# underdoc-wang/STC-GNN

Hardware: NVIDIA B200
Metric: train samples/s (fwd+bwd), SF-shape STC cell stack (higher is better)
Workload: dtype f32

## Files before the change

### include/stc_b200.h

```cpp
#ifndef STC_B200_H_
#define STC_B200_H_

#include <stddef.h>
#include <stdint.h>

#ifdef __cplusplus
extern "C" {
#endif

#define STC_ABI_VERSION 6

typedef enum {
  STC_OK = 0,
  STC_ERR_BAD_ARG = -1,
  STC_ERR_UNSUPPORTED = -2,
  STC_ERR_WORKSPACE = -3,
  STC_ERR_CUDA = -4,
  STC_ERR_ARCH = -5
} StcStatus;

enum { STC_ACT_NONE = 0, STC_ACT_RELU = 1 };
enum { STC_SUPPORT_DENSE = 0, STC_SUPPORT_CSR = 1 };

typedef struct {
  int32_t B;
  int32_t N;
  int32_t C;
  int32_t Din;
  int32_t h;
  int32_t Ks;
  int32_t Kc;
  int32_t act;
  int32_t has_bias;
} StcDims;

typedef struct {
  int32_t kind;
  int64_t nnz;
  const float* vals;
  const int32_t* rowptr;
  const int32_t* col;
  const float* t_vals;
  const int32_t* t_rowptr;
  const int32_t* t_col;
} StcSupport;

int stc_abi_version(void);
const char* stc_last_error(void);

size_t stc_cell_saved_bytes(const StcDims* d);
size_t stc_cell_bwd_scratch_bytes(const StcDims* d);

int stc_cell_fwd(const StcDims* d, const StcSupport* gs, const float* gc,
                 const float* xt, int64_t xt_batch_stride, const float* h_prev,
                 const float* Wg, const float* bg, const float* Wc, const float* bc,
                 float* h_out, void* saved, size_t saved_bytes, void* stream);

enum { STC_STAGE_GATES = 0, STC_STAGE_CANDI = 1 };
enum { STC_SAVED_U = 0, STC_SAVED_R, STC_SAVED_C, STC_SAVED_YR, STC_SAVED_YX, STC_SAVED_YH, STC_SAVED_Q,
       STC_SAVED_PG, STC_SAVED_PC, STC_SAVED_REGIONS };
int stc_cell_saved_layout(const StcDims* d, int64_t* offsets_floats, int32_t n_offsets);
int stc_cell_fwd_stage(const StcDims* d, int32_t stage, const float* gc,
                       const float* xt, int64_t xt_batch_stride, const float* h_prev,
                       const float* Wg, const float* bg, const float* Wc, const float* bc,
                       float* h_out, void* saved, size_t saved_bytes, void* stream);

int stc_cell_bwd(const StcDims* d, const StcSupport* gs, const float* gc,
                 const float* xt, int64_t xt_batch_stride, const float* h_prev,
                 const float* Wg, const float* Wc, const float* d_h_out,
                 float* d_xt, float* d_h_prev,
                 float* dWg, float* dbg, float* dWc, float* dbc, float* dGs, float* dGc,
                 int32_t accumulate_params, const void* saved, size_t saved_bytes,
                 void* scratch, size_t scratch_bytes, void* stream);

int stc_cell_fwd_x(const StcDims* d, const StcSupport* gs, const float* gc,
                   const float* xt, int64_t xt_batch_stride, const float* h_prev,
                   const float* Wg, const float* bg, const float* Wc, const float* bc,
                   float* h_out, void* saved, size_t saved_bytes, const float* yx_terms, void* stream);
int stc_cell_bwd_x(const StcDims* d, const StcSupport* gs, const float* gc,
                   const float* xt, int64_t xt_batch_stride, const float* h_prev,
                   const float* Wg, const float* Wc, const float* d_h_out,
                   float* d_xt, float* d_h_prev,
                   float* dWg, float* dbg, float* dWc, float* dbc, float* dGs, float* dGc,
                   int32_t accumulate_params, const void* saved, size_t saved_bytes,
                   void* scratch, size_t scratch_bytes, const float* yx_terms, float* dyx_terms_out, void* stream);
int stc_support_outer(int32_t N, int32_t B, int32_t width, const float* a, int64_t a_batch_stride, const float* b,
                      float coef, float* dGs, void* stream);
int stc_support_apply_edge_grad(const StcSupport* gs, int32_t N, int32_t B, int32_t width,
                                const float* x, int64_t x_batch_stride, const float* z, int64_t z_batch_stride,
                                float* y, float alpha, float beta, const float* a, int64_t a_batch_stride, float coef,
                                float* dvals, void* stream);
int stc_support_apply_rows_edge_grad(const StcSupport* gs, int32_t N, int32_t B, int32_t width,
                                     const float* x, int64_t x_batch_stride, const float* z, int64_t z_batch_stride,
                                     float* y, float alpha, float beta, const float* a, int64_t a_batch_stride,
                                     float coef, float* dvals, const int32_t* rows, int32_t n_rows, void* stream);

int stc_pair_scores_csr(const StcSupport* gs, int32_t N, int64_t width, const float* u, const float* v,
                        float* scores, void* stream);
int stc_pair_scores_csr_rows(const StcSupport* gs, int32_t N, int64_t width, int64_t ld, const float* u, const float* v,
                             float* scores, const int32_t* rows, int32_t n_rows, void* stream);
int stc_edge_softmax_fwd(const StcSupport* gs, int32_t N, const float* scores, float* p, void* stream);
int stc_edge_softmax_bwd(const StcSupport* gs, int32_t N, const float* scores, const float* p, const float* dp,
                         float* dscores, void* stream);

size_t stc_pair_topk_workspace_bytes(int32_t N, int64_t width, int32_t k);
int stc_pair_topk(int32_t N, int64_t width, const float* u, const float* v, int32_t k,
                  int32_t* cols, float* scores, void* ws, size_t ws_bytes, void* stream);

enum { STC_SCRATCH_DYR = 0, STC_SCRATCH_DYX, STC_SCRATCH_DYH, STC_SCRATCH_REGIONS };
int stc_cell_bwd_scratch_layout(const StcDims* d, int64_t* offsets_floats, int32_t n_offsets);
int stc_cell_bwd_stage(const StcDims* d, int32_t stage, const float* gc,
                       const float* xt, int64_t xt_batch_stride, const float* h_prev,
                       const float* Wg, const float* Wc, const float* d_h_out,
                       float* d_xt, float* d_h_prev,
                       float* dWg, float* dbg, float* dWc, float* dbc, float* dGc,
                       int32_t accumulate_params, const void* saved, size_t saved_bytes,
                       void* scratch, size_t scratch_bytes, void* stream);

int stc_support_apply(const StcSupport* gs, int32_t N, int32_t B, int32_t width, int32_t transpose,
                      const float* x, int64_t x_batch_stride, const float* z, int64_t z_batch_stride,
                      float* y, float alpha, float beta, void* stream);

int stc_support_apply_rows(const StcSupport* gs, int32_t N, int32_t B, int32_t width, int32_t transpose,
                           const float* x, int64_t x_batch_stride, const float* z, int64_t z_batch_stride,
                           float* y, float alpha, float beta, const int32_t* rows, int32_t n_rows, void* stream);

int stc_halo_pack(const float* x_ext, int64_t x_batch_stride, int32_t width, int32_t B, const int32_t* idx,
                  int32_t n_rows, float* send, void* stream);
int stc_halo_unpack(const float* recv, int32_t width, int32_t B, int32_t row0, int32_t n_rows, float* x_ext,
                    int64_t x_batch_stride, void* stream);

int stc_tf32x3_gemm(const float* a, const float* b, float* d, int32_t M, int32_t N, int32_t K, void* stream);

int stc_concurrency_set(int32_t mode);

int stc_last_launch_count(void);

int stc_timing_enable(int32_t on);
int stc_timing_collect(double* ms_by_kind, int64_t* launches_by_kind, double* alg_bytes_by_kind, int32_t n_kinds);
const char* stc_kernel_kind_name(int32_t kind);

int stc_debug_trace_set(void* dev_buf, int64_t n_slots);

#ifdef __cplusplus
}
#endif
#endif
```

### stc_gnn_b200/_lib.py

```python
import ctypes
import os
from ctypes import POINTER, Structure, c_char_p, c_float, c_int, c_int32, c_int64, c_size_t, c_void_p

HERE = os.path.dirname(os.path.abspath(__file__))
LIB_PATH = os.path.join(HERE, "libstc_b200.so")

ABI_VERSION = 6
ACT_NONE, ACT_RELU = 0, 1
SUPPORT_DENSE, SUPPORT_CSR = 0, 1

EXPORTED = (
    "stc_abi_version", "stc_last_error", "stc_cell_saved_bytes", "stc_cell_bwd_scratch_bytes",
    "stc_cell_fwd", "stc_cell_bwd", "stc_support_apply", "stc_last_launch_count",
    "stc_timing_enable", "stc_timing_collect", "stc_kernel_kind_name", "stc_tf32x3_gemm",
    "stc_cell_saved_layout", "stc_cell_fwd_stage", "stc_debug_trace_set",
    "stc_cell_bwd_scratch_layout", "stc_cell_bwd_stage",
    "stc_support_apply_rows", "stc_halo_pack", "stc_halo_unpack", "stc_concurrency_set",
    "stc_cell_fwd_x", "stc_cell_bwd_x", "stc_support_outer", "stc_support_apply_edge_grad",
    "stc_support_apply_rows_edge_grad", "stc_pair_scores_csr", "stc_edge_softmax_fwd", "stc_edge_softmax_bwd",
    "stc_pair_scores_csr_rows", "stc_pair_topk_workspace_bytes", "stc_pair_topk",
)
STAGE_GATES, STAGE_CANDI = 0, 1
SAVED_REGIONS = ("u", "r", "c", "Yr", "Yx", "Yh", "Q", "Pg", "Pc")
SCRATCH_REGIONS = ("dYr", "dYx", "dYh")


class StcDims(Structure):
    _fields_ = [(n, c_int32) for n in ("B", "N", "C", "Din", "h", "Ks", "Kc", "act", "has_bias")]


class StcSupport(Structure):
    _fields_ = [("kind", c_int32), ("nnz", c_int64), ("vals", c_void_p), ("rowptr", c_void_p), ("col", c_void_p),
                ("t_vals", c_void_p), ("t_rowptr", c_void_p), ("t_col", c_void_p)]


_lib = None


def load(build_if_missing: bool = True):
    global _lib
    if _lib is not None:
        return _lib
    if build_if_missing:
        from .build import build
        build()
    if not os.path.exists(LIB_PATH):
        raise RuntimeError(f"{LIB_PATH} is missing: run `python -m stc_gnn_b200.build` (no CPU fallback exists)")
    lib = ctypes.CDLL(LIB_PATH)
    lib.stc_abi_version.restype = c_int
    lib.stc_last_error.restype = c_char_p
    lib.stc_last_launch_count.restype = c_int
    lib.stc_cell_saved_bytes.restype = c_size_t
    lib.stc_cell_saved_bytes.argtypes = [POINTER(StcDims)]
    lib.stc_cell_bwd_scratch_bytes.restype = c_size_t
    lib.stc_cell_bwd_scratch_bytes.argtypes = [POINTER(StcDims)]
    lib.stc_cell_fwd.restype = c_int
    lib.stc_cell_fwd.argtypes = [POINTER(StcDims), POINTER(StcSupport), c_void_p, c_void_p, c_int64, c_void_p,
                                 c_void_p, c_void_p, c_void_p, c_void_p, c_void_p, c_void_p, c_size_t, c_void_p]
    lib.stc_cell_fwd_x.restype = c_int
    lib.stc_cell_fwd_x.argtypes = lib.stc_cell_fwd.argtypes[:-1] + [c_void_p, c_void_p]
    lib.stc_support_outer.restype = c_int
    lib.stc_support_outer.argtypes = [c_int32, c_int32, c_int32, c_void_p, c_int64, c_void_p, c_float, c_void_p, c_void_p]
    lib.stc_support_apply_edge_grad.restype = c_int
    lib.stc_support_apply_edge_grad.argtypes = [POINTER(StcSupport), c_int32, c_int32, c_int32, c_void_p, c_int64,
                                                c_void_p, c_int64, c_void_p, c_float, c_float, c_void_p, c_int64,
                                                c_float, c_void_p, c_void_p]
    lib.stc_support_apply_rows_edge_grad.restype = c_int
    lib.stc_support_apply_rows_edge_grad.argtypes = lib.stc_support_apply_edge_grad.argtypes[:-1] + [c_void_p, c_int32,
                                                                                                    c_void_p]
    lib.stc_pair_scores_csr.restype = c_int
    lib.stc_pair_scores_csr.argtypes = [POINTER(StcSupport), c_int32, c_int64, c_void_p, c_void_p, c_void_p, c_void_p]
    lib.stc_pair_scores_csr_rows.restype = c_int
    lib.stc_pair_scores_csr_rows.argtypes = [POINTER(StcSupport), c_int32, c_int64, c_int64, c_void_p, c_void_p,
                                             c_void_p, c_void_p, c_int32, c_void_p]
    lib.stc_pair_topk_workspace_bytes.restype = c_size_t
    lib.stc_pair_topk_workspace_bytes.argtypes = [c_int32, c_int64, c_int32]
    lib.stc_pair_topk.restype = c_int
    lib.stc_pair_topk.argtypes = [c_int32, c_int64, c_void_p, c_void_p, c_int32, c_void_p, c_void_p, c_void_p, c_size_t,
                                  c_void_p]
    lib.stc_edge_softmax_fwd.restype = c_int
    lib.stc_edge_softmax_fwd.argtypes = [POINTER(StcSupport), c_int32, c_void_p, c_void_p, c_void_p]
    lib.stc_edge_softmax_bwd.restype = c_int
    lib.stc_edge_softmax_bwd.argtypes = [POINTER(StcSupport), c_int32, c_void_p, c_void_p, c_void_p, c_void_p, c_void_p]
    lib.stc_cell_saved_layout.restype = c_int
    lib.stc_cell_saved_layout.argtypes = [POINTER(StcDims), POINTER(c_int64), c_int32]
    lib.stc_cell_fwd_stage.restype = c_int
    lib.stc_cell_fwd_stage.argtypes = [POINTER(StcDims), c_int32, c_void_p, c_void_p, c_int64, c_void_p, c_void_p,
                                       c_void_p, c_void_p, c_void_p, c_void_p, c_void_p, c_size_t, c_void_p]
    lib.stc_cell_bwd.restype = c_int
    lib.stc_cell_bwd.argtypes = [POINTER(StcDims), POINTER(StcSupport), c_void_p, c_void_p, c_int64, c_void_p,
                                 c_void_p, c_void_p, c_void_p, c_void_p, c_void_p, c_void_p, c_void_p, c_void_p,
                                 c_void_p, c_void_p, c_void_p, c_int32, c_void_p, c_size_t, c_void_p, c_size_t,
                                 c_void_p]
    lib.stc_cell_bwd_x.restype = c_int
    lib.stc_cell_bwd_x.argtypes = lib.stc_cell_bwd.argtypes[:-1] + [c_void_p, c_void_p, c_void_p]
    lib.stc_cell_bwd_scratch_layout.restype = c_int
    lib.stc_cell_bwd_scratch_layout.argtypes = [POINTER(StcDims), POINTER(c_int64), c_int32]
    lib.stc_cell_bwd_stage.restype = c_int
    lib.stc_cell_bwd_stage.argtypes = [POINTER(StcDims), c_int32, c_void_p, c_void_p, c_int64, c_void_p,
                                       c_void_p, c_void_p, c_void_p, c_void_p, c_void_p, c_void_p, c_void_p, c_void_p,
                                       c_void_p, c_void_p, c_int32, c_void_p, c_size_t, c_void_p, c_size_t, c_void_p]
    lib.stc_support_apply.restype = c_int
    lib.stc_support_apply.argtypes = [POINTER(StcSupport), c_int32, c_int32, c_int32, c_int32, c_void_p, c_int64,
                                      c_void_p, c_int64, c_void_p, c_float, c_float, c_void_p]
    lib.stc_support_apply_rows.restype = c_int
    lib.stc_support_apply_rows.argtypes = [POINTER(StcSupport), c_int32, c_int32, c_int32, c_int32, c_void_p, c_int64,
                                           c_void_p, c_int64, c_void_p, c_float, c_float, c_void_p, c_int32, c_void_p]
    lib.stc_halo_pack.restype = c_int
    lib.stc_halo_pack.argtypes = [c_void_p, c_int64, c_int32, c_int32, c_void_p, c_int32, c_void_p, c_void_p]
    lib.stc_halo_unpack.restype = c_int
    lib.stc_halo_unpack.argtypes = [c_void_p, c_int32, c_int32, c_int32, c_int32, c_void_p, c_int64, c_void_p]
    lib.stc_concurrency_set.restype = c_int
    lib.stc_concurrency_set.argtypes = [c_int32]
    lib.stc_tf32x3_gemm.restype = c_int
    lib.stc_tf32x3_gemm.argtypes = [c_void_p, c_void_p, c_void_p, c_int32, c_int32, c_int32, c_void_p]
    lib.stc_timing_enable.restype = c_int
    lib.stc_timing_enable.argtypes = [c_int32]
    lib.stc_timing_collect.restype = c_int
    lib.stc_timing_collect.argtypes = [POINTER(ctypes.c_double), POINTER(c_int64), POINTER(ctypes.c_double), c_int32]
    lib.stc_debug_trace_set.restype = c_int
    lib.stc_debug_trace_set.argtypes = [c_void_p, c_int64]
    lib.stc_kernel_kind_name.restype = c_char_p
    lib.stc_kernel_kind_name.argtypes = [c_int32]
    if lib.stc_abi_version() != ABI_VERSION:
        raise RuntimeError(f"libstc_b200.so ABI {lib.stc_abi_version()} != binding ABI {ABI_VERSION}: rebuild")
    _lib = lib
    return lib


def saved_layout(dims: StcDims) -> dict:
    lib = load()
    offs = (c_int64 * len(SAVED_REGIONS))()
    check(lib.stc_cell_saved_layout(dims, offs, len(SAVED_REGIONS)), "stc_cell_saved_layout")
    return {n: int(offs[i]) for i, n in enumerate(SAVED_REGIONS)}


def scratch_layout(dims: StcDims) -> dict:
    lib = load()
    offs = (c_int64 * len(SCRATCH_REGIONS))()
    check(lib.stc_cell_bwd_scratch_layout(dims, offs, len(SCRATCH_REGIONS)), "stc_cell_bwd_scratch_layout")
    return {n: int(offs[i]) for i, n in enumerate(SCRATCH_REGIONS)}


def check(status: int, what: str) -> None:
    if status != 0:
        msg = _lib.stc_last_error().decode("utf-8", "replace") if _lib is not None else ""
        raise RuntimeError(f"{what} failed (status {status}): {msg}")


def last_launch_count() -> int:
    return int(load().stc_last_launch_count())


LAUNCHES = 0


def note_launches() -> None:
    global LAUNCHES
    LAUNCHES += int(_lib.stc_last_launch_count())


def set_concurrency(mode: int) -> None:
    check(load().stc_concurrency_set(int(mode)), "stc_concurrency_set")


def timing_enable(on: bool) -> None:
    load().stc_timing_enable(1 if on else 0)


def timing_collect():
    lib = load()
    n = 32
    ms = (ctypes.c_double * n)()
    cnt = (c_int64 * n)()
    by = (ctypes.c_double * n)()
    kinds = lib.stc_timing_collect(ms, cnt, by, n)
    return {lib.stc_kernel_kind_name(k).decode(): (ms[k], int(cnt[k]), by[k]) for k in range(kinds) if cnt[k]}
```

### stc_gnn_b200/cell.py

```python
from __future__ import annotations

import os

import torch
from torch import nn

from . import _lib
from .support import CsrSupport, dense_struct

INPLACE_LEAF_GRADS = os.environ.get("STC_INPLACE_GRADS", "1") != "0"

_ACT_CODES = {None: _lib.ACT_NONE, nn.ReLU: _lib.ACT_RELU}
_ACT_NAMES = {_lib.ACT_NONE: None, _lib.ACT_RELU: "relu"}


def _activation_code(activation) -> int:
    if activation in _ACT_CODES:
        return _ACT_CODES[activation]
    if isinstance(activation, str):
        return {"none": _lib.ACT_NONE, "relu": _lib.ACT_RELU}[activation]
    raise NotImplementedError(f"activation {activation!r} is not implemented in the B200 cell (None or nn.ReLU)")


class GraphConvParams(nn.Module):

    def __init__(self, Ks: int, Kc: int, input_dim: int, hidden_dim: int, use_bias: bool = True):
        super().__init__()
        self.Ks, self.Kc, self.input_dim, self.hidden_dim, self.use_bias = Ks, Kc, input_dim, hidden_dim, use_bias
        self.W = nn.Parameter(torch.empty(input_dim * Ks * Kc, hidden_dim), requires_grad=True)
        nn.init.xavier_normal_(self.W)
        if use_bias:
            self.b = nn.Parameter(torch.empty(hidden_dim), requires_grad=True)
            nn.init.constant_(self.b, val=0.0)


def _dims(B, N, C, Din, h, Ks, Kc, act, has_bias) -> _lib.StcDims:
    return _lib.StcDims(B, N, C, Din, h, Ks, Kc, act, 1 if has_bias else 0)


_SIZES = {}


def _buffer_floats(lib, dims: _lib.StcDims, key):
    hit = _SIZES.get(key)
    if hit is None:
        if len(_SIZES) > 256:
            _SIZES.clear()
        hit = _SIZES[key] = (lib.stc_cell_saved_bytes(dims) // 4, lib.stc_cell_bwd_scratch_bytes(dims) // 4)
    return hit


def _ptr(t):
    return t.data_ptr() if t is not None else None


class _CellFunction(torch.autograd.Function):

    @staticmethod
    def forward(ctx, Gs, Gc, Xt, H, Wg, bg, Wc, bc, Yx, Ev, cfg):
        lib = _lib.load()
        Ks, Kc, act = cfg
        B, N, C, Din = Xt.shape
        h = H.shape[-1]
        for name, t in (("Gc", Gc), ("Xt", Xt), ("Ht_1", H), ("gates.W", Wg), ("candi.W", Wc)):
            if not t.is_cuda or t.dtype != torch.float32:
                raise RuntimeError(f"STC_Cell (B200): {name} must be a float32 CUDA tensor, got {t.dtype} on {t.device}; "
                                   "there is no CPU fallback")
        if H.shape != (B, N, C, h):
            raise RuntimeError(f"Ht_1 shape {tuple(H.shape)} does not match Xt {tuple(Xt.shape)}")
        rows = (Din + h) * Ks * Kc
        if Wg.shape != (rows, 2 * h) or Wc.shape != (rows, h) or Gc.shape != (C, C):
            raise RuntimeError(f"shape mismatch: gates.W {tuple(Wg.shape)} (want {(rows, 2 * h)}), candi.W "
                               f"{tuple(Wc.shape)} (want {(rows, h)}), Gc {tuple(Gc.shape)} (want {(C, C)})")
        for name, b_, n_ in (("gates.b", bg, 2 * h), ("candi.b", bc, h)):
            if b_ is not None and (b_.shape != (n_,) or not b_.is_cuda or b_.dtype != torch.float32):
                raise RuntimeError(f"{name} must be a float32 CUDA tensor of shape ({n_},)")
        if (bg is None) != (bc is None):
            raise RuntimeError("gates.b and candi.b must both be present or both absent")
        csr = isinstance(Gs, CsrSupport)
        if csr:
            if Gs.N != N:
                raise RuntimeError(f"CSR support has {Gs.N} nodes, Xt has {N}")
            if Ev is not None and Ev is not Gs.vals:
                raise RuntimeError("edge values passed to the cell must be the CsrSupport's own `vals`")
            if Gs.learnable:
                Gs.sync_t_vals()
            gs_struct = Gs.struct()
        else:
            if not Gs.is_cuda or Gs.dtype != torch.float32 or Gs.shape != (N, N):
                raise RuntimeError(f"Gs must be a float32 CUDA [N,N] tensor or a CsrSupport, got {tuple(Gs.shape)} {Gs.dtype}")
            gs_keep = Gs.contiguous()
            gs_struct = dense_struct(gs_keep)
        Gc_c, H_c, Wg_c, Wc_c = Gc.contiguous(), H.contiguous(), Wg.contiguous(), Wc.contiguous()
        bg_c = bg.contiguous() if bg is not None else None
        bc_c = bc.contiguous() if bc is not None else None
        Xt_c = Xt if (B == 0 or Xt[0].is_contiguous()) else Xt.contiguous()
        xbs = Xt_c.stride(0) if B > 1 else N * C * Din
        dims = _dims(B, N, C, Din, h, Ks, Kc, act, bg is not None)
        ctx.size_key = (B, N, C, Din, h, Ks, Kc, act, bg is not None)
        saved = torch.empty(_buffer_floats(lib, dims, ctx.size_key)[0], dtype=torch.float32, device=Xt.device)
        Hn = torch.empty((B, N, C, h), dtype=torch.float32, device=Xt.device)
        stream = torch.cuda.current_stream().cuda_stream
        Yx_c = None
        if Yx is not None and Ks > 1:
            if Yx.shape != (Ks - 1, B, N, C, Din) or not Yx.is_cuda or Yx.dtype != torch.float32:
                raise RuntimeError(f"hoisted Xt-side terms must be a float32 CUDA tensor of shape {(Ks - 1, B, N, C, Din)}, "
                                   f"got {tuple(Yx.shape)}")
            Yx_c = Yx.contiguous()
        if B == 0:
            status = 0
        elif Yx_c is not None:
            status = lib.stc_cell_fwd_x(dims, gs_struct, Gc_c.data_ptr(), Xt_c.data_ptr(), xbs, H_c.data_ptr(),
                                        Wg_c.data_ptr(), _ptr(bg_c), Wc_c.data_ptr(), _ptr(bc_c), Hn.data_ptr(),
                                        saved.data_ptr(), saved.numel() * 4, Yx_c.data_ptr(), stream)
        else:
            status = lib.stc_cell_fwd(dims, gs_struct, Gc_c.data_ptr(), Xt_c.data_ptr(), xbs, H_c.data_ptr(),
                                      Wg_c.data_ptr(), _ptr(bg_c), Wc_c.data_ptr(), _ptr(bc_c), Hn.data_ptr(),
                                      saved.data_ptr(), saved.numel() * 4, stream)
        _lib.check(status, "stc_cell_fwd")
        _lib.note_launches()
        ctx.hoisted = Yx_c is not None
        ctx.cfg, ctx.dims_tuple, ctx.xbs, ctx.csr = cfg, (B, N, C, Din, h), xbs, csr
        ctx.gs_obj = Gs if csr else None
        ctx.has_bias = bg is not None
        ctx.sinks = {}
        if INPLACE_LEAF_GRADS:
            for i, t in ((0, None if csr else Gs), (1, Gc), (4, Wg), (5, bg), (6, Wc), (7, bc), (9, Ev)):
                if t is not None and ctx.needs_input_grad[i] and t.is_leaf and t.is_contiguous():
                    ctx.sinks[i] = t
        ctx.has_ev = Ev is not None
        ctx.save_for_backward(*( [] if csr else [gs_keep] ), Gc_c, Xt_c, H_c, Wg_c, Wc_c, saved,
                              *([Yx_c] if Yx_c is not None else []), *([Ev] if Ev is not None else []))
        return Hn

    @staticmethod
    @torch.autograd.function.once_differentiable
    def backward(ctx, dHn):
        lib = _lib.load()
        Ks, Kc, act = ctx.cfg
        B, N, C, Din, h = ctx.dims_tuple
        sv = list(ctx.saved_tensors)
        if ctx.has_ev:
            sv.pop()
        Yx = sv.pop() if ctx.hoisted else None
        if ctx.csr:
            Gs = ctx.gs_obj
            Gc, Xt, H, Wg, Wc, saved = sv
            gs_struct = Gs.struct()
        else:
            Gs, Gc, Xt, H, Wg, Wc, saved = sv
            gs_struct = dense_struct(Gs)
        need = ctx.needs_input_grad
        dev = dHn.device
        dHn = dHn.contiguous()
        L, P = Din + h, Ks * Kc
        dims = _dims(B, N, C, Din, h, Ks, Kc, act, ctx.has_bias)
        new = lambda *shape: torch.empty(shape, dtype=torch.float32, device=dev)
        if ctx.hoisted and need[2]:
            raise RuntimeError("hoisted Xt-side terms: the gradient w.r.t. Xt is folded by the caller (stack.py hoists only "
                               "when the input sequence needs no gradient)")
        dXt = new(B, N, C, Din) if need[2] else None
        dH = new(B, N, C, h)
        dYx = torch.empty_like(Yx) if ctx.hoisted else None
        returned = [None] * 11

        def target(i, shape, wanted=True):
            if not wanted:
                return None
            leaf = ctx.sinks.get(i)
            if leaf is not None and need[i]:
                if leaf.grad is None:
                    leaf.grad = torch.zeros(shape, dtype=torch.float32, device=dev)
                if leaf.grad.is_contiguous() and leaf.grad.dtype == torch.float32 and leaf.grad.shape == torch.Size(shape):
                    return leaf.grad
            buf = torch.zeros(shape, dtype=torch.float32, device=dev)
            returned[i] = buf
            return buf

        dWg, dWc = target(4, (P * L, 2 * h)), target(6, (P * L, h))
        dbg, dbc = target(5, (2 * h,), ctx.has_bias), target(7, (h,), ctx.has_bias)
        dGs = target(9, (Gs.nnz,), need[9]) if ctx.csr else target(0, (N, N), need[0])
        dGc = target(1, (C, C), need[1])
        returned[2], returned[3], returned[8] = dXt, dH, dYx
        if B == 0:
            if dYx is not None:
                dYx.zero_()
            return tuple(returned)
        scratch = torch.empty(_buffer_floats(lib, dims, ctx.size_key)[1], dtype=torch.float32, device=dev)
        common = (dims, gs_struct, Gc.data_ptr(), Xt.data_ptr(), ctx.xbs, H.data_ptr(), Wg.data_ptr(),
                  Wc.data_ptr(), dHn.data_ptr(), _ptr(dXt), dH.data_ptr(), dWg.data_ptr(), _ptr(dbg),
                  dWc.data_ptr(), _ptr(dbc), _ptr(dGs), _ptr(dGc), 1, saved.data_ptr(),
                  saved.numel() * 4, scratch.data_ptr(), scratch.numel() * 4)
        stream = torch.cuda.current_stream().cuda_stream
        if ctx.hoisted:
            status = lib.stc_cell_bwd_x(*common, Yx.data_ptr(), dYx.data_ptr(), stream)
        else:
            status = lib.stc_cell_bwd(*common, stream)
        _lib.check(status, "stc_cell_bwd")
        _lib.note_launches()
        for i in (0, 1, 4, 5, 6, 7, 8, 9):
            if not need[i]:
                returned[i] = None
        return tuple(returned)


def stc_cell_forward(Gs, Gc, Xt, Ht_1, Wg, bg, Wc, bc, Ks: int, Kc: int, activation=None) -> torch.Tensor:
    return _CellFunction.apply(Gs, Gc, Xt, Ht_1, Wg, bg, Wc, bc, None, _edge_values(Gs),
                               (int(Ks), int(Kc), _activation_code(activation)))


def _edge_values(Gs):
    return Gs.vals if isinstance(Gs, CsrSupport) and Gs.learnable else None


class STC_Cell(nn.Module):

    def __init__(self, num_nodes: int, num_categories: int, Ks: int, Kc: int, input_dim: int, hidden_dim: int,
                 use_bias=True, activation=None):
        super().__init__()
        self.num_nodes = num_nodes
        self.num_categories = num_categories
        self.hidden_dim = hidden_dim
        self.input_dim = input_dim
        self.Ks, self.Kc = Ks, Kc
        self._act = _activation_code(activation)
        self.gates = GraphConvParams(Ks, Kc, input_dim + hidden_dim, hidden_dim * 2, use_bias)
        self.candi = GraphConvParams(Ks, Kc, input_dim + hidden_dim, hidden_dim, use_bias)

    def init_hidden(self, batch_size: int):
        weight = next(self.parameters()).data
        return weight.new_zeros(batch_size, self.num_nodes, self.num_categories, self.hidden_dim)

    def forward(self, Gs, Gc: torch.Tensor, Xt: torch.Tensor, Ht_1: torch.Tensor, _Yx: torch.Tensor = None):
        assert len(Xt.shape) == len(Ht_1.shape) == 4, 'STC-cell must take in 4D tensor as input [Xt, Ht-1]'
        if isinstance(Gs, torch.Tensor) and Gs.layout != torch.strided:
            Gs = _csr_cache(Gs)
        if hasattr(Gs, "fwd") and hasattr(Gs, "hop_ext"):
            from .halo import partitioned_cell_forward
            return partitioned_cell_forward(Gs, Gc, Xt, Ht_1, self.gates.W, getattr(self.gates, "b", None), self.candi.W,
                                            getattr(self.candi, "b", None), self.Ks, self.Kc, _ACT_NAMES[self._act],
                                            reduce_params=getattr(Gs, "reduce_per_cell", True))
        return _CellFunction.apply(Gs, Gc, Xt, Ht_1, self.gates.W, getattr(self.gates, "b", None), self.candi.W,
                                   getattr(self.candi, "b", None), _Yx, _edge_values(Gs), (self.Ks, self.Kc, self._act))


_CSR_CACHE = {}


def _csr_cache(G: torch.Tensor) -> CsrSupport:
    if G.requires_grad:
        raise RuntimeError("STC_Cell (B200): a torch sparse Gs is a constant support and gets no gradient; for learned "
                           "edge weights on a fixed pattern pass CsrSupport(rowptr, col, vals_requiring_grad, N) "
                           "(or a dense [N,N] tensor when the whole dGs is needed)")
    if G.layout == torch.sparse_csr:
        vals, idx = G.values(), G.col_indices()
    else:
        vals, idx = G._values(), G._indices()
    key = (vals.data_ptr(), vals._version, idx.data_ptr(), idx._version, int(vals.numel()), tuple(G.shape), G.layout,
           vals.dtype)
    hit = _CSR_CACHE.get(key)
    if hit is None:
        if len(_CSR_CACHE) > 8:
            _CSR_CACHE.clear()
        hit = _CSR_CACHE[key] = (CsrSupport.from_torch_sparse(G), G)
    return hit[0]
```

### stc_gnn_b200/csrc/stc_api.cu

```cuda
#include "stc_common.cuh"

#include <stdlib.h>
#include <string.h>

#include <atomic>
#include <mutex>
#include <vector>

namespace stc {

static thread_local char g_err[512] = "";
static thread_local int g_launches = 0;

void set_error(const char* fmt, ...) {
  va_list ap;
  va_start(ap, fmt);
  vsnprintf(g_err, sizeof(g_err), fmt, ap);
  va_end(ap);
}
void count_launch(int n) { g_launches += n; }
void reset_launch_count() { g_launches = 0; }

struct TimedLaunch {
  int kind;
// ... 238 lines not shown
  a.Hout = phase == 0 ? 2 * d.h : d.h;
  a.x0 = xt;
  a.x0_bs = xt_bs;
  a.yx = ws + w.Yx;
  a.W = W;
  a.Q = Q;
  a.opt = conv_opt_flags();
  const bool wide_bwd = !(a.opt & OPT_WIDE_DX_FFMA) && conv_big_bwd_shape_ok(a.C, a.Din, a.h, a.Ks, a.Kc, a.Hout);
  a.dpre_ld = (conv_tc_eligible(a) || wide_bwd) ? a.Kc * a.Hout : a.Hout;
  conv_trace_target(&a.trace, &a.trace_tiles);
  if (a.trace) a.trace += (size_t)phase * a.trace_tiles * TRACE_SLOTS;
  return a;
}

}

using namespace stc;

extern "C" {

int stc_timing_enable(int32_t on) {
  g_timing.store(on != 0);
  return STC_OK;
}

int stc_timing_collect(double* ms, int64_t* launches, double* bytes, int32_t n_kinds) {
  std::lock_guard<std::mutex> lk(g_tmu);
  for (auto& t : g_timed) {
    float m = 0.f;
    if (cudaEventSynchronize(t.e1) == cudaSuccess && cudaEventElapsedTime(&m, t.e0, t.e1) == cudaSuccess &&
        t.kind < n_kinds) {
      if (ms) ms[t.kind] += m;
      if (launches) launches[t.kind] += 1;
      if (bytes) bytes[t.kind] += t.bytes;
    }
    g_event_pool.push_back(t.e0);
    g_event_pool.push_back(t.e1);
  }
  g_timed.clear();
  return KK_COUNT;
}

const char* stc_kernel_kind_name(int32_t kind) {
  static const char* names[KK_COUNT] = {"support_dense", "support_csr", "support_outer", "cheby_small",
                                        "conv_fwd",      "conv_bwd_dx", "conv_bwd_dw", "tc_conv_fwd", "tc_conv_bwd_dx", "tc_conv_bwd_dw",
                                        "tc_support", "tc_gemm_test", "tc_outer", "tc_support_big", "support_csr_grad",
                                        "pair_scores_csr", "edge_softmax", "pair_topk"};
  return (kind >= 0 && kind < KK_COUNT) ? names[kind] : "?";
}

int stc_debug_trace_set(void* dev_buf, int64_t n_slots) {
  std::lock_guard<std::mutex> lk(g_tmu);
  g_trace_buf = (long long*)dev_buf;
  g_trace_tiles = dev_buf ? (int)(n_slots / (2 * TRACE_SLOTS)) : 0;
  return STC_OK;
}

int stc_concurrency_set(int32_t mode) {
  if (mode < -1 || mode > 1) {
    set_error("stc_concurrency_set: mode %d (use -1 = by problem size, 0 = one stream, 1 = always fork)", mode);
    return STC_ERR_BAD_ARG;
  }
  g_concurrency.store(mode, std::memory_order_relaxed);
  return STC_OK;
}

int stc_abi_version(void) { return STC_ABI_VERSION; }
const char* stc_last_error(void) { return g_err; }
int stc_last_launch_count(void) { return g_launches; }

size_t stc_cell_saved_bytes(const StcDims* d) {
  if (check_dims(d) != STC_OK) return 0;
  return make_layout(*d).saved_total * sizeof(float);
}
size_t stc_cell_bwd_scratch_bytes(const StcDims* d) {
  if (check_dims(d) != STC_OK) return 0;
  return make_layout(*d).scratch_total * sizeof(float);
}

int stc_support_apply(const StcSupport* gs, int32_t N, int32_t B, int32_t width, int32_t transpose,
                      const float* x, int64_t x_batch_stride, const float* z, int64_t z_batch_stride, float* y,
                      float alpha, float beta, void* stream) {
  reset_launch_count();
  if (!gs || !x || !y) {
    set_error("stc_support_apply: NULL argument");
    return STC_ERR_BAD_ARG;
  }
  STC_TRY(check_arch());
  return launch_support_apply(*gs, N, B, width, transpose != 0, x, x_batch_stride, z, z_batch_stride, y, alpha,
                              beta, nullptr, 0.f, (cudaStream_t)stream);
}

int stc_support_apply_rows(const StcSupport* gs, int32_t N, int32_t B, int32_t width, int32_t transpose, const float* x,
                           int64_t x_batch_stride, const float* z, int64_t z_batch_stride, float* y, float alpha,
                           float beta, const int32_t* rows, int32_t n_rows, void* stream) {
  reset_launch_count();
  if (!gs || !x || !y || !rows) {
    set_error("stc_support_apply_rows: NULL argument");
    return STC_ERR_BAD_ARG;
  }
  if (n_rows < 0 || n_rows > N) {
    set_error("stc_support_apply_rows: n_rows %d outside [0, N = %d]", n_rows, N);
    return STC_ERR_BAD_ARG;
  }
  STC_TRY(check_arch());
  return launch_support_apply(*gs, N, B, width, transpose != 0, x, x_batch_stride, z, z_batch_stride, y, alpha, beta,
                              nullptr, 0.f, (cudaStream_t)stream, rows, n_rows);
}

int stc_halo_pack(const float* x_ext, int64_t x_batch_stride, int32_t width, int32_t B, const int32_t* idx, int32_t n_rows,
                  float* send, void* stream) {
  reset_launch_count();
  if (n_rows > 0 && (!x_ext || !idx || !send)) {
    set_error("stc_halo_pack: NULL argument");
    return STC_ERR_BAD_ARG;
  }
  STC_TRY(check_arch());
  return launch_halo_rows(true, const_cast<float*>(x_ext), x_batch_stride, width, B, idx, 0, n_rows, send, (cudaStream_t)stream);
}

int stc_halo_unpack(const float* recv, int32_t width, int32_t B, int32_t row0, int32_t n_rows, float* x_ext,
                    int64_t x_batch_stride, void* stream) {
  reset_launch_count();
  if (n_rows > 0 && (!x_ext || !recv)) {
    set_error("stc_halo_unpack: NULL argument");
    return STC_ERR_BAD_ARG;
  }
  STC_TRY(check_arch());
  return launch_halo_rows(false, x_ext, x_batch_stride, width, B, nullptr, row0, n_rows, const_cast<float*>(recv), (cudaStream_t)stream);
}

int stc_tf32x3_gemm(const float* a, const float* b, float* d, int32_t M, int32_t N, int32_t K, void* stream) {
  reset_launch_count();
  if (!a || !b || !d) {
    set_error("stc_tf32x3_gemm: NULL argument");
    return STC_ERR_BAD_ARG;
  }
  STC_TRY(check_arch());
  return launch_tf32x3_gemm(a, b, d, M, N, K, (cudaStream_t)stream);
}

struct FwdCtx {
  const StcDims& d;
  const WsLayout& w;
  const StcSupport* gs;
  const float* gc;
  const float* xt;
  int64_t xt_bs;
  const float* h_prev;
  float* ws;
  cudaStream_t st;
  Lanes* lanes = nullptr;
  const float* yx_pre = nullptr;
};

static int fwd_terms_xh(const FwdCtx& f) {
  const StcDims& d = f.d;
  const WsLayout& w = f.w;
  float* ws = f.ws;
  const size_t Rh = w.R * d.h, Rx = w.R * d.Din;
  const int CD = d.C * d.Din, CH = d.C * d.h;
  const long long nbs_h = (long long)d.N * CH;
  cudaStream_t sx = f.st;
  if (f.lanes && f.lanes->active() && d.Ks > 1 && !f.yx_pre) {
    STC_TRY(f.lanes->fork(0));
    sx = f.lanes->stream(0);
  }
  for (int k = 1; k < d.Ks && !f.yx_pre; ++k) {
    const float alpha = k == 1 ? 1.f : 2.f, beta = k == 1 ? 0.f : -1.f;
    const float* xin = k == 1 ? f.xt : ws + w.Yx + (size_t)(k - 2) * Rx;
    const int64_t xin_bs = k == 1 ? f.xt_bs : (int64_t)d.N * CD;
    const float* xz = k == 1 ? nullptr : (k == 2 ? f.xt : ws + w.Yx + (size_t)(k - 3) * Rx);
    const int64_t xz_bs = k == 2 ? f.xt_bs : (int64_t)d.N * CD;
    STC_TRY(launch_support_apply(*f.gs, d.N, d.B, CD, true, xin, xin_bs, xz, xz_bs, ws + w.Yx + (size_t)(k - 1) * Rx,
                                 alpha, beta, nullptr, 0.f, sx));
  }
  for (int k = 1; k < d.Ks; ++k) {
    const float alpha = k == 1 ? 1.f : 2.f, beta = k == 1 ? 0.f : -1.f;
    const float* hin = k == 1 ? f.h_prev : ws + w.Yh + (size_t)(k - 2) * Rh;
    const float* hz = k == 1 ? nullptr : (k == 2 ? f.h_prev : ws + w.Yh + (size_t)(k - 3) * Rh);
    STC_TRY(launch_support_apply(*f.gs, d.N, d.B, CH, true, hin, nbs_h, hz, nbs_h, ws + w.Yh + (size_t)(k - 1) * Rh,
                                 alpha, beta, nullptr, 0.f, f.st));
  }
  if (f.lanes) STC_TRY(f.lanes->join(0));
  return STC_OK;
}

static int fwd_gates(const FwdCtx& f, const float* Wg, const float* bg) {
  const StcDims& d = f.d;
  const WsLayout& w = f.w;
  float* ws = f.ws;
  if (d.Kc > 1) STC_TRY(launch_cheby_small(f.gc, d.C, d.Kc, ws + w.Q, f.st));
  ConvArgs a = base_args(d, f.xt, f.xt_bs, Wg, ws + w.Q, ws, w, 0);
  if (f.yx_pre) a.yx = f.yx_pre;
  a.h0 = f.h_prev;
  a.yh = ws + w.Yh;
  a.bias = d.has_bias ? bg : nullptr;
  a.Hprev = f.h_prev;
  a.u = ws + w.u;
  a.r = ws + w.r;
  a.rH = ws + w.Yr;
  a.Psave = ws + w.Pg;
  a.Wimg = (w.Wimg_c > w.Wimg_g) ? ws + w.Wimg_g : nullptr;
  return launch_conv_fwd(a, f.st);
}

static int fwd_terms_rh(const FwdCtx& f) {
  const StcDims& d = f.d;
  const WsLayout& w = f.w;
  float* ws = f.ws;
  const size_t Rh = w.R * d.h;
  const int CH = d.C * d.h;
  const long long nbs_h = (long long)d.N * CH;
  for (int k = 1; k < d.Ks; ++k) {
    const float alpha = k == 1 ? 1.f : 2.f, beta = k == 1 ? 0.f : -1.f;
    const float* in = ws + w.Yr + (size_t)(k - 1) * Rh;
    const float* z = k == 1 ? nullptr : ws + w.Yr + (size_t)(k - 2) * Rh;
    STC_TRY(launch_support_apply(*f.gs, d.N, d.B, CH, true, in, nbs_h, z, nbs_h, ws + w.Yr + (size_t)k * Rh, alpha, beta,
                                 nullptr, 0.f, f.st));
  }
  return STC_OK;
}

static int fwd_candi(const FwdCtx& f, const float* Wc, const float* bc, float* h_out) {
  const StcDims& d = f.d;
  const WsLayout& w = f.w;
  float* ws = f.ws;
  const size_t Rh = w.R * d.h;
  ConvArgs a = base_args(d, f.xt, f.xt_bs, Wc, ws + w.Q, ws, w, 1);
  if (f.yx_pre) a.yx = f.yx_pre;
  a.h0 = ws + w.Yr;
  a.yh = ws + w.Yr + Rh;
  a.bias = d.has_bias ? bc : nullptr;
  a.Hprev = f.h_prev;
  a.u = ws + w.u;
  a.c = ws + w.c;
  a.Hnew = h_out;
  a.Psave = ws + w.Pc;
  a.Wimg = (w.saved_total > w.Wimg_c) ? ws + w.Wimg_c : nullptr;
  return launch_conv_fwd(a, f.st);
}

static int check_fwd_args(const StcDims* dp, const float* gc, const float* xt, const float* h_prev, const float* Wg,
                          const float* bg, const float* Wc, const float* bc, float* h_out, void* wsv, size_t ws_bytes,
                          const char* who) {
  STC_TRY(check_dims(dp));
  if (!gc || !xt || !h_prev || !Wg || !Wc || !h_out || !wsv) {
    set_error("%s: NULL argument", who);
    return STC_ERR_BAD_ARG;
  }
  if (dp->has_bias && (!bg || !bc)) {
    set_error("%s: has_bias set but bias pointer is NULL", who);
    return STC_ERR_BAD_ARG;
  }
  const WsLayout w = make_layout(*dp);
  if (ws_bytes < w.saved_total * sizeof(float)) {
    set_error("saved buffer too small: %zu < %zu bytes", ws_bytes, w.saved_total * sizeof(float));
    return STC_ERR_WORKSPACE;
  }
  return STC_OK;
}

static int cell_fwd_impl(const StcDims* dp, const StcSupport* gs, const float* gc, const float* xt,
                         int64_t xt_batch_stride, const float* h_prev, const float* Wg, const float* bg, const float* Wc,
                         const float* bc, float* h_out, void* wsv, size_t ws_bytes, const float* yx_terms, void* stream,
                         const char* who) {
  reset_launch_count();
  STC_TRY(check_fwd_args(dp, gc, xt, h_prev, Wg, bg, Wc, bc, h_out, wsv, ws_bytes, who));
  if (!gs) {
    set_error("%s: NULL support", who);
    return STC_ERR_BAD_ARG;
  }
  const StcDims& d = *dp;
  if (d.B == 0) return STC_OK;
  STC_TRY(check_arch());
  const WsLayout w = make_layout(d);
  Lanes lanes((cudaStream_t)stream, d);
  FwdCtx f{d, w, gs, gc, xt, xt_batch_stride, h_prev, (float*)wsv, (cudaStream_t)stream};
  f.lanes = &lanes;
  f.yx_pre = d.Ks > 1 ? yx_terms : nullptr;
  STC_TRY(fwd_terms_xh(f));
  STC_TRY(fwd_gates(f, Wg, bg));
  STC_TRY(fwd_terms_rh(f));
  STC_TRY(fwd_candi(f, Wc, bc, h_out));
  return STC_OK;
}

int stc_cell_fwd(const StcDims* dp, const StcSupport* gs, const float* gc, const float* xt,
                 int64_t xt_batch_stride, const float* h_prev, const float* Wg, const float* bg, const float* Wc,
                 const float* bc, float* h_out, void* wsv, size_t ws_bytes, void* stream) {
  return cell_fwd_impl(dp, gs, gc, xt, xt_batch_stride, h_prev, Wg, bg, Wc, bc, h_out, wsv, ws_bytes, nullptr, stream,
                       "stc_cell_fwd");
}

int stc_cell_fwd_x(const StcDims* dp, const StcSupport* gs, const float* gc, const float* xt,
                   int64_t xt_batch_stride, const float* h_prev, const float* Wg, const float* bg, const float* Wc,
                   const float* bc, float* h_out, void* wsv, size_t ws_bytes, const float* yx_terms, void* stream) {
  return cell_fwd_impl(dp, gs, gc, xt, xt_batch_stride, h_prev, Wg, bg, Wc, bc, h_out, wsv, ws_bytes, yx_terms, stream,
                       "stc_cell_fwd_x");
}

int stc_cell_saved_layout(const StcDims* dp, int64_t* offsets, int32_t n_offsets) {
  STC_TRY(check_dims(dp));
  if (!offsets || n_offsets < STC_SAVED_REGIONS) {
    set_error("stc_cell_saved_layout: need room for %d offsets", (int)STC_SAVED_REGIONS);
    return STC_ERR_BAD_ARG;
  }
  const WsLayout w = make_layout(*dp);
  const size_t v[STC_SAVED_REGIONS] = {w.u, w.r, w.c, w.Yr, w.Yx, w.Yh, w.Q, w.Pg, w.Pc};
  for (int i = 0; i < STC_SAVED_REGIONS; ++i) offsets[i] = (int64_t)v[i];
  return STC_OK;
}

int stc_cell_fwd_stage(const StcDims* dp, int32_t stage, const float* gc, const float* xt, int64_t xt_batch_stride,
                       const float* h_prev, const float* Wg, const float* bg, const float* Wc, const float* bc,
                       float* h_out, void* wsv, size_t ws_bytes, void* stream) {
  reset_launch_count();
  STC_TRY(check_fwd_args(dp, gc, xt, h_prev, Wg, bg, Wc, bc, h_out, wsv, ws_bytes, "stc_cell_fwd_stage"));
  if (stage != STC_STAGE_GATES && stage != STC_STAGE_CANDI) {
    set_error("stc_cell_fwd_stage: bad stage %d", stage);
    return STC_ERR_BAD_ARG;
  }
  const StcDims& d = *dp;
  if (d.B == 0) return STC_OK;
  STC_TRY(check_arch());
  const WsLayout w = make_layout(d);
  const FwdCtx f{d, w, nullptr, gc, xt, xt_batch_stride, h_prev, (float*)wsv, (cudaStream_t)stream};
  return stage == STC_STAGE_GATES ? fwd_gates(f, Wg, bg) : fwd_candi(f, Wc, bc, h_out);
}

static int adjoint_chain(const StcDims& d, const StcSupport& gs, int width, const float* y0, int64_t y0_bs,
                         const float* yk , float* ybar0, float* ybark ,
                         float* dGs, cudaStream_t st, Lanes* lanes = nullptr, int outer_lane = 1) {
  const size_t Rw = (size_t)d.B * d.N * width;
  const int64_t nbs = (int64_t)d.N * width;
  for (int k = d.Ks - 1; k >= 1; --k) {
    const float coef = k >= 2 ? 2.f : 1.f;
    float* yb_k = ybark + (size_t)(k - 1) * Rw;
    float* yb_km1 = k == 1 ? ybar0 : ybark + (size_t)(k - 2) * Rw;
    float* axpy = nullptr;
    if (k >= 2) axpy = k == 2 ? ybar0 : ybark + (size_t)(k - 3) * Rw;
    if (dGs && gs.kind == STC_SUPPORT_CSR) {
      const float* yprev = k == 1 ? y0 : yk + (size_t)(k - 2) * Rw;
      const int64_t yprev_bs = k == 1 ? y0_bs : nbs;
      STC_TRY(launch_support_csr_edge_grad(gs, d.N, d.B, width, yb_k, nbs, yb_km1, nbs, yb_km1, coef, 1.f, axpy, -1.f,
                                           yprev, yprev_bs, coef, dGs, st));
      continue;
    }
    if (dGs) {
      const float* yprev = k == 1 ? y0 : yk + (size_t)(k - 2) * Rw;
      const int64_t yprev_bs = k == 1 ? y0_bs : nbs;
      cudaStream_t so = st;
      if (lanes && lanes->active()) {
        STC_TRY(lanes->fork_from(st, outer_lane));
        so = lanes->stream(outer_lane);
      }
      STC_TRY(launch_support_outer(d.N, d.B, width, yprev, yprev_bs, yb_k, coef, dGs, so));
    }
    STC_TRY(launch_support_apply(gs, d.N, d.B, width, false, yb_k, nbs, yb_km1, nbs, yb_km1, coef, 1.f, axpy, -1.f,
                                 st));
  }
  return STC_OK;
}

struct BwdCtx {
  const StcDims& d;
  const WsLayout& w;
  const float* gc;
  const float* xt;
  int64_t xt_bs;
  const float* h_prev;
  const float* d_h_out;
  float* d_xt;
  float* d_h_prev;
  float* dGc;
  float* sv;
  float* sc;
  cudaStream_t st;
  Lanes* lanes = nullptr;
  const float* yx_pre = nullptr;
  float* dyx_out = nullptr;
  bool want_dGc() const { return dGc != nullptr && d.Kc > 1; }
  float* dYx0() const { return d_xt ? d_xt : sc + w.dYx0; }
};

static int check_bwd_args(const StcDims* dp, const float* gc, const float* xt, const float* h_prev, const float* Wg,
                          const float* Wc, const float* d_h_out, float* d_h_prev, float* dWg, float* dbg, float* dWc,
                          float* dbc, const void* savedv, size_t saved_bytes, void* scratchv, size_t scratch_bytes,
                          const char* who) {
  STC_TRY(check_dims(dp));
  const StcDims& d = *dp;
  if (!gc || !xt || !h_prev || !Wg || !Wc || !d_h_out || !d_h_prev || !dWg || !dWc || !savedv || !scratchv) {
    set_error("%s: NULL argument", who);
    return STC_ERR_BAD_ARG;
  }
  if (d.has_bias && (!dbg || !dbc)) {
    set_error("%s: has_bias set but a bias-gradient pointer is NULL", who);
    return STC_ERR_BAD_ARG;
  }
  const WsLayout w = make_layout(d);
  if (saved_bytes < w.saved_total * sizeof(float) || scratch_bytes < w.scratch_total * sizeof(float)) {
    set_error("buffers too small: saved %zu (need %zu), scratch %zu (need %zu) bytes", saved_bytes,
              w.saved_total * sizeof(float), scratch_bytes, w.scratch_total * sizeof(float));
    return STC_ERR_WORKSPACE;
  }
  return STC_OK;
}

static int bwd_begin(const BwdCtx& b, float* dWg, float* dbg, float* dWc, float* dbc, float* dGs, size_t dGs_floats,
                     int accumulate_params) {
  const StcDims& d = b.d;
  const int L = d.Din + d.h, P = d.Ks * d.Kc;
  if (!accumulate_params) {
    STC_CUDA_OK(cudaMemsetAsync(dWg, 0, sizeof(float) * P * L * 2 * d.h, b.st));
    STC_CUDA_OK(cudaMemsetAsync(dWc, 0, sizeof(float) * P * L * d.h, b.st));
    if (d.has_bias) {
      STC_CUDA_OK(cudaMemsetAsync(dbg, 0, sizeof(float) * 2 * d.h, b.st));
      STC_CUDA_OK(cudaMemsetAsync(dbc, 0, sizeof(float) * d.h, b.st));
    }
    if (dGs && dGs_floats) STC_CUDA_OK(cudaMemsetAsync(dGs, 0, sizeof(float) * dGs_floats, b.st));
    if (b.dGc) STC_CUDA_OK(cudaMemsetAsync(b.dGc, 0, sizeof(float) * d.C * d.C, b.st));
  }
  if (d.B > 0 && b.want_dGc()) STC_CUDA_OK(cudaMemsetAsync(b.sc + b.w.dQ, 0, sizeof(float) * d.Kc * d.C * d.C, b.st));
  return STC_OK;
}

static int launch_dw_beside(const BwdCtx& b, const ConvArgs& a) {
  if (b.lanes && b.lanes->active()) {
    STC_TRY(b.lanes->fork(0));
    return launch_conv_bwd_dw(a, b.lanes->stream(0));
  }
  return launch_conv_bwd_dw(a, b.st);
}

static int bwd_candi(const BwdCtx& b, const float* Wc, float* dWc, float* dbc) {
  const StcDims& d = b.d;
  const WsLayout& w = b.w;
  const size_t Rh = w.R * d.h;
  ConvArgs a = base_args(d, b.xt, b.xt_bs, Wc, b.sv + w.Q, b.sv, w, 1);
  if (b.yx_pre) a.yx = b.yx_pre;
  a.h0 = b.sv + w.Yr;
  a.yh = b.sv + w.Yr + Rh;
  a.Hprev = b.h_prev;
  a.u = b.sv + w.u;
  a.c = b.sv + w.c;
  a.dHn = b.d_h_out;
  a.dpre = b.sc + w.dpre;
  a.dbias = d.has_bias ? dbc : nullptr;
  a.dYx0 = b.dYx0();
  a.dYx = b.dyx_out ? b.dyx_out : b.sc + w.dYx;
  a.accum_x = 0;
  a.dYh0 = b.sc + w.dYr;
  a.dYh = b.sc + w.dYr + Rh;
  a.dQ = b.want_dGc() ? b.sc + w.dQ : nullptr;
  a.dW = dWc;
  a.Psave = b.sv + w.Pc;
  a.Wimg = (w.saved_total > w.Wimg_c && w.scratch_total > w.Wimg_dx) ? b.sc + w.Wimg_dx : nullptr;
  STC_TRY(launch_conv_bwd_dx(a, b.st));
  return launch_dw_beside(b, a);
}

static int bwd_gates(const BwdCtx& b, const float* Wg, float* dWg, float* dbg) {
  const StcDims& d = b.d;
  const WsLayout& w = b.w;
  ConvArgs a = base_args(d, b.xt, b.xt_bs, Wg, b.sv + w.Q, b.sv, w, 0);
  if (b.yx_pre) a.yx = b.yx_pre;
  a.h0 = b.h_prev;
  a.yh = b.sv + w.Yh;
  a.Hprev = b.h_prev;
  a.u = b.sv + w.u;
  a.r = b.sv + w.r;
  a.c = b.sv + w.c;
  a.dHn = b.d_h_out;
  a.drH = b.sc + w.dYr;
  a.dpre = b.sc + w.dpre;
  a.dbias = d.has_bias ? dbg : nullptr;
  a.dYx0 = b.dYx0();
  a.dYx = b.dyx_out ? b.dyx_out : b.sc + w.dYx;
  a.accum_x = 1;
  a.dYh0 = b.d_h_prev;
  a.dYh = b.sc + w.dYh;
  a.dQ = b.want_dGc() ? b.sc + w.dQ : nullptr;
  a.dW = dWg;
  a.Psave = b.sv + w.Pg;
  a.Wimg = (w.Wimg_c > w.Wimg_g && w.scratch_total > w.Wimg_dx) ? b.sc + w.Wimg_dx : nullptr;
  if (b.lanes) STC_TRY(b.lanes->join(0));
  STC_TRY(launch_conv_bwd_dx(a, b.st));
  STC_TRY(launch_dw_beside(b, a));
  if (b.want_dGc()) STC_TRY(launch_cheby_small_bwd(b.gc, b.sv + w.Q, b.sc + w.dQ, d.C, d.Kc, b.dGc, b.st));
  return STC_OK;
}

static int cell_bwd_impl(const StcDims* dp, const StcSupport* gs, const float* gc, const float* xt,
                         int64_t xt_batch_stride, const float* h_prev, const float* Wg, const float* Wc,
                         const float* d_h_out, float* d_xt, float* d_h_prev, float* dWg, float* dbg, float* dWc, float* dbc,
                         float* dGs, float* dGc, int32_t accumulate_params, const void* savedv, size_t saved_bytes,
                         void* scratchv, size_t scratch_bytes, const float* yx_terms, float* dyx_terms_out, void* stream,
                         const char* who) {
  reset_launch_count();
  STC_TRY(check_bwd_args(dp, gc, xt, h_prev, Wg, Wc, d_h_out, d_h_prev, dWg, dbg, dWc, dbc, savedv, saved_bytes, scratchv,
                         scratch_bytes, who));
  const StcDims& d = *dp;
  if (!gs) {
    set_error("%s: NULL argument", who);
    return STC_ERR_BAD_ARG;
  }
  if (dGs && gs->kind == STC_SUPPORT_CSR && (!gs->rowptr || !gs->col || !gs->vals || gs->nnz < 0)) {
    set_error("%s: the edge-value gradient of a CSR support needs its rowptr/col/vals and nnz", who);
    return STC_ERR_BAD_ARG;
  }
  if (d.Ks > 1 && ((yx_terms != nullptr) != (dyx_terms_out != nullptr))) {
    set_error("%s: yx_terms and dyx_terms_out go together (the caller that supplied the Xt-side terms folds their adjoints)", who);
    return STC_ERR_BAD_ARG;
  }
  const WsLayout w = make_layout(d);
  STC_TRY(check_arch());
  cudaStream_t st = (cudaStream_t)stream;
  Lanes lanes(st, d);
  BwdCtx b{d, w, gc, xt, xt_batch_stride, h_prev, d_h_out, d_xt, d_h_prev, dGc,
           const_cast<float*>((const float*)savedv), (float*)scratchv, st};
  b.lanes = &lanes;
  const bool hoisted = d.Ks > 1 && yx_terms != nullptr;
  if (hoisted) {
    b.yx_pre = yx_terms;
    b.dyx_out = dyx_terms_out;
  }
  const size_t dGs_floats = gs->kind == STC_SUPPORT_CSR ? (size_t)gs->nnz : (size_t)d.N * d.N;
  STC_TRY(bwd_begin(b, dWg, dbg, dWc, dbc, dGs, dGs_floats, accumulate_params));
  if (d.B == 0) return STC_OK;
  const size_t Rh = w.R * d.h;
  const int CD = d.C * d.Din, CH = d.C * d.h;

  STC_TRY(bwd_candi(b, Wc, dWc, dbc));
  STC_TRY(adjoint_chain(d, *gs, CH, b.sv + w.Yr, (int64_t)d.N * CH, b.sv + w.Yr + Rh, b.sc + w.dYr, b.sc + w.dYr + Rh,
                        dGs, st, &lanes, 1));
  STC_TRY(bwd_gates(b, Wg, dWg, dbg));
  if (!hoisted) {
    cudaStream_t sx = st;
    if (lanes.active() && d.Ks > 1) {
      STC_TRY(lanes.fork(2));
      sx = lanes.stream(2);
    }
    STC_TRY(adjoint_chain(d, *gs, CD, xt, xt_batch_stride, b.sv + w.Yx, b.dYx0(), b.sc + w.dYx, dGs, sx, &lanes, 1));
  }
  STC_TRY(adjoint_chain(d, *gs, CH, h_prev, (int64_t)d.N * CH, b.sv + w.Yh, d_h_prev, b.sc + w.dYh, dGs, st, &lanes, 1));
  return lanes.join_all();
}

int stc_cell_bwd(const StcDims* dp, const StcSupport* gs, const float* gc, const float* xt,
                 int64_t xt_batch_stride, const float* h_prev, const float* Wg, const float* Wc,
                 const float* d_h_out, float* d_xt, float* d_h_prev, float* dWg, float* dbg, float* dWc, float* dbc,
                 float* dGs, float* dGc, int32_t accumulate_params, const void* savedv, size_t saved_bytes,
                 void* scratchv, size_t scratch_bytes, void* stream) {
  return cell_bwd_impl(dp, gs, gc, xt, xt_batch_stride, h_prev, Wg, Wc, d_h_out, d_xt, d_h_prev, dWg, dbg, dWc, dbc, dGs, dGc,
                       accumulate_params, savedv, saved_bytes, scratchv, scratch_bytes, nullptr, nullptr, stream,
                       "stc_cell_bwd");
}

int stc_cell_bwd_x(const StcDims* dp, const StcSupport* gs, const float* gc, const float* xt,
                   int64_t xt_batch_stride, const float* h_prev, const float* Wg, const float* Wc,
                   const float* d_h_out, float* d_xt, float* d_h_prev, float* dWg, float* dbg, float* dWc, float* dbc,
                   float* dGs, float* dGc, int32_t accumulate_params, const void* savedv, size_t saved_bytes,
                   void* scratchv, size_t scratch_bytes, const float* yx_terms, float* dyx_terms_out, void* stream) {
  return cell_bwd_impl(dp, gs, gc, xt, xt_batch_stride, h_prev, Wg, Wc, d_h_out, d_xt, d_h_prev, dWg, dbg, dWc, dbc, dGs, dGc,
                       accumulate_params, savedv, saved_bytes, scratchv, scratch_bytes, yx_terms, dyx_terms_out, stream,
                       "stc_cell_bwd_x");
}

int stc_support_outer(int32_t N, int32_t B, int32_t width, const float* a, int64_t a_batch_stride, const float* b,
                      float coef, float* dGs, void* stream) {
  reset_launch_count();
  if (!a || !b || !dGs) {
    set_error("stc_support_outer: NULL argument");
    return STC_ERR_BAD_ARG;
  }
  STC_TRY(check_arch());
  return launch_support_outer(N, B, width, a, a_batch_stride, b, coef, dGs, (cudaStream_t)stream);
}

int stc_support_apply_edge_grad(const StcSupport* gs, int32_t N, int32_t B, int32_t width, const float* x,
                                int64_t x_batch_stride, const float* z, int64_t z_batch_stride, float* y, float alpha,
                                float beta, const float* a, int64_t a_batch_stride, float coef, float* dvals,
                                void* stream) {
  reset_launch_count();
  if (!gs || !x || !y || !a || !dvals) {
    set_error("stc_support_apply_edge_grad: NULL argument");
    return STC_ERR_BAD_ARG;
  }
  if (gs->kind != STC_SUPPORT_CSR) {
    set_error("stc_support_apply_edge_grad: CSR supports only (a dense support's gradient is stc_support_outer)");
    return STC_ERR_UNSUPPORTED;
  }
  STC_TRY(check_arch());
  return launch_support_csr_edge_grad(*gs, N, B, width, x, x_batch_stride, z, z_batch_stride, y, alpha, beta, nullptr,
                                      0.f, a, a_batch_stride, coef, dvals, (cudaStream_t)stream);
}

int stc_support_apply_rows_edge_grad(const StcSupport* gs, int32_t N, int32_t B, int32_t width, const float* x,
                                     int64_t x_batch_stride, const float* z, int64_t z_batch_stride, float* y,
                                     float alpha, float beta, const float* a, int64_t a_batch_stride, float coef,
                                     float* dvals, const int32_t* rows, int32_t n_rows, void* stream) {
  reset_launch_count();
  if (!gs || !x || !y || !a || !dvals || !rows) {
    set_error("stc_support_apply_rows_edge_grad: NULL argument");
    return STC_ERR_BAD_ARG;
  }
  if (gs->kind != STC_SUPPORT_CSR) {
    set_error("stc_support_apply_rows_edge_grad: CSR supports only");
    return STC_ERR_UNSUPPORTED;
  }
  if (n_rows < 0 || n_rows > N) {
    set_error("stc_support_apply_rows_edge_grad: n_rows %d outside [0, N = %d]", n_rows, N);
    return STC_ERR_BAD_ARG;
  }
  STC_TRY(check_arch());
  return launch_support_csr_edge_grad(*gs, N, B, width, x, x_batch_stride, z, z_batch_stride, y, alpha, beta, nullptr,
                                      0.f, a, a_batch_stride, coef, dvals, (cudaStream_t)stream, rows, n_rows);
}

static int check_pattern(const StcSupport* gs, int32_t N, const char* who) {
  if (!gs) {
    set_error("%s: NULL pattern", who);
    return STC_ERR_BAD_ARG;
  }
  if (gs->kind != STC_SUPPORT_CSR) {
    set_error("%s: the pattern must be a CSR support (kind %d)", who, gs->kind);
    return STC_ERR_UNSUPPORTED;
  }
  if (!gs->rowptr || !gs->col || gs->nnz < 0) {
    set_error("%s: the pattern needs rowptr / col and nnz >= 0", who);
    return STC_ERR_BAD_ARG;
  }
  if (N <= 0) {
    set_error("%s: N = %d must be positive", who, N);
    return STC_ERR_BAD_ARG;
  }
  return STC_OK;
}

int stc_pair_scores_csr(const StcSupport* gs, int32_t N, int64_t width, const float* u, const float* v, float* scores,
                        void* stream) {
  reset_launch_count();
  STC_TRY(check_pattern(gs, N, "stc_pair_scores_csr"));
  if (!u || !v || !scores) {
    set_error("stc_pair_scores_csr: NULL argument");
    return STC_ERR_BAD_ARG;
  }
  if (width <= 0) {
    set_error("stc_pair_scores_csr: width = %lld must be positive", (long long)width);
    return STC_ERR_BAD_ARG;
  }
  STC_TRY(check_arch());
  return launch_pair_scores_csr(gs->rowptr, gs->col, gs->nnz, N, width, u, v, scores, (cudaStream_t)stream);
}

int stc_pair_scores_csr_rows(const StcSupport* gs, int32_t N, int64_t width, int64_t ld, const float* u, const float* v,
                             float* scores, const int32_t* rows, int32_t n_rows, void* stream) {
  reset_launch_count();
  STC_TRY(check_pattern(gs, N, "stc_pair_scores_csr_rows"));
  if (!u || !v || !scores || !rows) {
    set_error("stc_pair_scores_csr_rows: NULL argument");
    return STC_ERR_BAD_ARG;
  }
  if (width <= 0) {
    set_error("stc_pair_scores_csr_rows: width = %lld must be positive", (long long)width);
    return STC_ERR_BAD_ARG;
  }
  if (ld < width) {
    set_error("stc_pair_scores_csr_rows: row stride ld = %lld is smaller than width = %lld", (long long)ld,
              (long long)width);
    return STC_ERR_BAD_ARG;
  }
  if (n_rows < 0 || n_rows > N) {
    set_error("stc_pair_scores_csr_rows: n_rows %d outside [0, N = %d]", n_rows, N);
    return STC_ERR_BAD_ARG;
  }
  STC_TRY(check_arch());
  return launch_pair_scores_csr_rows(gs->rowptr, gs->col, gs->nnz, N, width, ld, u, v, scores, rows, n_rows,
                                     (cudaStream_t)stream);
}

int stc_edge_softmax_fwd(const StcSupport* gs, int32_t N, const float* scores, float* p, void* stream) {
  reset_launch_count();
  STC_TRY(check_pattern(gs, N, "stc_edge_softmax_fwd"));
  if (!scores || !p) {
    set_error("stc_edge_softmax_fwd: NULL argument");
    return STC_ERR_BAD_ARG;
  }
  STC_TRY(check_arch());
  return launch_edge_softmax(false, gs->rowptr, gs->nnz, N, scores, nullptr, nullptr, p, (cudaStream_t)stream);
}

int stc_edge_softmax_bwd(const StcSupport* gs, int32_t N, const float* scores, const float* p, const float* dp,
                         float* dscores, void* stream) {
  reset_launch_count();
  STC_TRY(check_pattern(gs, N, "stc_edge_softmax_bwd"));
  if (!scores || !p || !dp || !dscores) {
    set_error("stc_edge_softmax_bwd: NULL argument");
    return STC_ERR_BAD_ARG;
  }
  STC_TRY(check_arch());
  return launch_edge_softmax(true, gs->rowptr, gs->nnz, N, scores, p, dp, dscores, (cudaStream_t)stream);
}

static int check_topk_shape(int32_t N, int64_t width, int32_t k, const char* who) {
  if (N <= 0 || width <= 0 || width % 4 != 0 || width > (1 << 28)) {
    set_error("%s: N = %d must be positive and width = %lld a positive multiple of 4 (at most 2^28)", who, N,
              (long long)width);
    return STC_ERR_BAD_ARG;
  }
  if (k > 32) {
    set_error("%s: k = %d: at most 32 columns a row are kept on chip", who, k);
    return STC_ERR_UNSUPPORTED;
  }
  if (k < 1 || k > N) {
    set_error("%s: k = %d outside [1, N = %d]", who, k, N);
    return STC_ERR_BAD_ARG;
  }
  return STC_OK;
// ... 72 lines not shown
```

### stc_gnn_b200/csrc/stc_common.cuh

```cuda
#pragma once
#include <cuda_runtime.h>
#include <stdint.h>
#include <stdio.h>
#include <stdarg.h>

#include "../../include/stc_b200.h"

namespace stc {

void set_error(const char* fmt, ...);
void count_launch(int n = 1);
void reset_launch_count();

#define STC_CUDA_OK(expr)                                                                   \
  do {                                                                                      \
    cudaError_t _e = (expr);                                                                \
    if (_e != cudaSuccess) {                                                                \
      stc::set_error("%s failed: %s (%s:%d)", #expr, cudaGetErrorString(_e), __FILE__, __LINE__); \
      return STC_ERR_CUDA;                                                                  \
    }                                                                                       \
  } while (0)

#define STC_LAUNCH_OK(name)                                                                 \
  do {                                                                                      \
    cudaError_t _e = cudaGetLastError();                                                    \
    if (_e != cudaSuccess) {                                                                \
      stc::set_error("launch of %s failed: %s (%s:%d)", name, cudaGetErrorString(_e), __FILE__, __LINE__); \
      return STC_ERR_CUDA;                                                                  \
    }                                                                                       \
    stc::count_launch();                                                                    \
  } while (0)

#define STC_TRY(expr)            \
  do {                           \
    int _s = (expr);             \
    if (_s != STC_OK) return _s; \
  } while (0)

enum KernelKind {
  KK_SUPPORT_DENSE = 0, KK_SUPPORT_CSR, KK_SUPPORT_OUTER, KK_CHEBY_SMALL, KK_CONV_FWD, KK_CONV_BWD_DX,
  KK_CONV_BWD_DW, KK_TC_CONV_FWD, KK_TC_CONV_BWD_DX, KK_TC_CONV_BWD_DW, KK_TC_SUPPORT, KK_TC_GEMM_TEST, KK_TC_OUTER, KK_TC_SUPPORT_BIG,
  KK_SUPPORT_CSR_GRAD, KK_PAIR_SCORES_CSR, KK_EDGE_SOFTMAX, KK_PAIR_TOPK, KK_COUNT
};
struct ScopedKernelTimer {
  ScopedKernelTimer(int kind, cudaStream_t st, double alg_bytes);
  ~ScopedKernelTimer();
  cudaEvent_t e0, e1;
  int kind;
  double bytes;
  cudaStream_t st;
};

static inline size_t round_up(size_t x, size_t m) { return (x + m - 1) / m * m; }
static inline int ceil_div(long long a, long long b) { return (int)((a + b - 1) / b); }

struct FastDiv {
  uint32_t d, M, s;
};
static inline FastDiv make_fastdiv(uint32_t d) {
  FastDiv f;
  f.d = d ? d : 1;
  f.s = 0;
  while ((2u << f.s) <= f.d && f.s < 31) ++f.s;
  f.M = (uint32_t)(((((uint64_t)1) << (32 + f.s)) - 1) / f.d);
  return f;
}
#ifdef __CUDACC__
__device__ __forceinline__ uint32_t fast_div(uint32_t n, const FastDiv f) {
  if (f.d == 1) return n;
  uint32_t q = __umulhi(n, f.M) >> f.s;
  if (n - q * f.d >= f.d) ++q;
  return q;
}
#endif

int device_sm_count();
int check_arch();

struct WsLayout {
  size_t R;
  size_t u, r, c, Yr, Yx, Yh, Q, Pg, Pc, Wimg_g, Wimg_c, saved_total;
  size_t dpre, dYx0, dYx, dYh, dYr, dQ, Wimg_dx, scratch_total;
};
WsLayout make_layout(const StcDims& d);

int launch_support_apply(const StcSupport& gs, int N, int B, int width, bool transpose, const float* x,
                         int64_t x_bs, const float* z, int64_t z_bs, float* y, float alpha, float beta,
                         float* axpy_out, float axpy_coef, cudaStream_t st, const int32_t* row_list = nullptr,
                         int n_list = 0);
int launch_halo_rows(bool pack, float* x_ext, long long x_bs, int W, int B, const int32_t* idx, int row0, int n_rows,
                     float* buf, cudaStream_t st);

int try_launch_support_tc(const float* G, int N, int B, int width, bool transpose, const float* x, int64_t x_bs,
                          const float* z, int64_t z_bs, float* y, float alpha, float beta, cudaStream_t st,
                          bool* handled);
int try_launch_support_tc_big(const float* G, int N, int B, int width, bool transpose, const float* x, int64_t x_bs,
                              const float* z, int64_t z_bs, float* y, float alpha, float beta, cudaStream_t st,
                              bool* handled);
int try_launch_outer_tc(int N, int B, int width, const float* a, int64_t a_bs, const float* bmat, float coef, float* dG,
                        cudaStream_t st, bool* handled);

int launch_support_csr_edge_grad(const StcSupport& gs, int N, int B, int width, const float* x, int64_t x_bs,
                                 const float* z, int64_t z_bs, float* y, float alpha, float beta, float* axpy_out,
                                 float axpy_coef, const float* a, int64_t a_bs, float coef, float* dvals,
                                 cudaStream_t st, const int32_t* row_list = nullptr, int n_list = 0);

int launch_support_outer(int N, int B, int width, const float* a, int64_t a_bs, const float* bmat, float coef,
                         float* dG, cudaStream_t st);

int launch_pair_scores_csr(const int32_t* rowptr, const int32_t* col, long long nnz, int N, long long width,
                           const float* u, const float* v, float* scores, cudaStream_t st);
int launch_pair_scores_csr_rows(const int32_t* rowptr, const int32_t* col, long long nnz, int N, long long width,
                                long long ld, const float* u, const float* v, float* scores, const int32_t* rows,
                                int n_rows, cudaStream_t st);
int launch_edge_softmax(bool bwd, const int32_t* rowptr, long long nnz, int N, const float* s, const float* p,
                        const float* dp, float* out, cudaStream_t st);
size_t pair_topk_ws_bytes(int N, int k);
int launch_pair_topk(int N, int width, const float* u, const float* v, int k, int32_t* cols, float* scores, void* ws,
                     cudaStream_t st);

int launch_cheby_small(const float* G, int C, int K, float* Q, cudaStream_t st);
int launch_cheby_small_bwd(const float* G, const float* Q, float* dQ, int C, int K, float* dG, cudaStream_t st);

struct ConvArgs {
  int B, N, C, Din, h, Ks, Kc, Hout, act, phase;
  const float* x0;
  long long x0_bs;
  const float* yx;
  const float* h0;
  const float* yh;
  const float* W;
  const float* bias;
  const float* Q;
  const float* Hprev;
  float* u;
  float* r;
  float* rH;
  float* c;
  float* Hnew;
  float* Psave;
  float* Wimg;
  const float* dHn;
  const float* drH;
  float* dpre;
  int dpre_ld;
  float* dbias;
  float* dYx0;
  float* dYx;
  int accum_x;
  float* dYh0;
  float* dYh;
  float* dQ;
  float* dW;
  int opt;
  long long* trace;
  int trace_tiles;
};
enum { OPT_L2_PREFETCH = 1, OPT_GENERIC_EPILOGUE = 4 ,
       OPT_SMEM_A = 8 ,
       OPT_WIDE_DX_FFMA = 32  };
constexpr int TRACE_SLOTS = 16;
int conv_opt_flags();
void conv_trace_target(long long** buf, int* tiles);
int launch_tf32x3_gemm(const float* A, const float* Bm, float* D, int M, int N, int K, cudaStream_t st);
int launch_conv_fwd(const ConvArgs& a, cudaStream_t st);
bool conv_big_shape_ok(int C, int Din, int h, int Ks, int Kc, int Hout);
size_t conv_big_img_floats(int C, int Din, int h, int Ks, int Kc, int Hout);
int try_launch_conv_fwd_big(const ConvArgs& a, cudaStream_t st, bool* handled);
size_t conv_big_dx_img_floats(int C, int Din, int h, int Ks, int Kc, int Hout);
int try_launch_conv_bwd_dx_big(const ConvArgs& a, cudaStream_t st, bool* handled);
bool conv_big_bwd_shape_ok(int C, int Din, int h, int Ks, int Kc, int Hout);
int try_launch_conv_bwd_dw_big(const ConvArgs& a, cudaStream_t st, bool* handled);
bool conv_tc_eligible(const ConvArgs& a);
bool conv_tc_dw_shape_ok(const ConvArgs& a);
int launch_conv_bwd_dx(const ConvArgs& a, cudaStream_t st);
int launch_conv_bwd_dw(const ConvArgs& a, cudaStream_t st);

}
```

### stc_gnn_b200/csrc/stc_conv.cu

```cuda
#include "stc_conv_common.cuh"

namespace stc {

template <int NI>
__device__ __forceinline__ void tile_gemm(float (&acc)[NI][4][4], const float* __restrict__ A, int lda,
                                          const float* __restrict__ Bm, int ldb, int K, int RG, int CG) {
  const int items = RG * CG;
#pragma unroll
  for (int i = 0; i < NI; ++i) {
    const int it = threadIdx.x + i * CV_THREADS;
    if (it >= items) break;
    const int rg = it / CG, cg = it - rg * CG;
    const float* ap = A + rg * 4 * lda;
    const float* bp = Bm + cg * 4;
#pragma unroll 4
    for (int k = 0; k < K; ++k) {
      float a0 = ap[k], a1 = ap[lda + k], a2 = ap[2 * lda + k], a3 = ap[3 * lda + k];
      float4 b = *reinterpret_cast<const float4*>(bp + k * ldb);
      acc[i][0][0] = fmaf(a0, b.x, acc[i][0][0]); acc[i][0][1] = fmaf(a0, b.y, acc[i][0][1]);
      acc[i][0][2] = fmaf(a0, b.z, acc[i][0][2]); acc[i][0][3] = fmaf(a0, b.w, acc[i][0][3]);
      acc[i][1][0] = fmaf(a1, b.x, acc[i][1][0]); acc[i][1][1] = fmaf(a1, b.y, acc[i][1][1]);
      acc[i][1][2] = fmaf(a1, b.z, acc[i][1][2]); acc[i][1][3] = fmaf(a1, b.w, acc[i][1][3]);
      acc[i][2][0] = fmaf(a2, b.x, acc[i][2][0]); acc[i][2][1] = fmaf(a2, b.y, acc[i][2][1]);
      acc[i][2][2] = fmaf(a2, b.z, acc[i][2][2]); acc[i][2][3] = fmaf(a2, b.w, acc[i][2][3]);
// ... 118 lines not shown
    }
    target = (t.npt / 2) * a.C;
    if (target < a.C) target = a.C;
  }
}


int launch_conv_fwd(const ConvArgs& a, cudaStream_t st) {
  bool handled = false;
  STC_TRY(try_launch_conv_fwd_tc(a, st, &handled));
  if (handled) return STC_OK;
  STC_TRY(try_launch_conv_fwd_big(a, st, &handled));
  if (handled) return STC_OK;
  ConvTile t; size_t smem; int ni;
  STC_TRY(pick_rows_fwd(a, &t, &smem, &ni));
  long long total_nodes = (long long)a.B * a.N;
  int grid = ceil_div(total_nodes, t.npt);
  const double R = (double)total_nodes * a.C;
  ScopedKernelTimer _t(KK_CONV_FWD, st,
                       4.0 * R * (a.Ks * t.L + (a.phase == 0 ? 3 * a.h : 4 * a.h)) + 4.0 * a.Ks * a.Kc * t.L * a.Hout);
  switch (ni) {
    case 1: STC_TRY(set_smem(conv_fwd_kernel<1>, smem)); conv_fwd_kernel<1><<<grid, CV_THREADS, smem, st>>>(a, t); break;
    case 2: STC_TRY(set_smem(conv_fwd_kernel<2>, smem)); conv_fwd_kernel<2><<<grid, CV_THREADS, smem, st>>>(a, t); break;
    default: STC_TRY(set_smem(conv_fwd_kernel<4>, smem)); conv_fwd_kernel<4><<<grid, CV_THREADS, smem, st>>>(a, t); break;
  }
  STC_LAUNCH_OK("conv_fwd_kernel");
  return STC_OK;
}

template <int NI>
__global__ void __launch_bounds__(CV_THREADS)
conv_bwd_dx_kernel(const ConvArgs a, const ConvTile t, const int DP) {
  extern __shared__ __align__(16) float smem[];
  const int C = a.C, L = t.L, LP = t.LP, LP4 = t.LP4, Hout = a.Hout, h = a.h, Din = a.Din;
  const bool mixed = a.Kc > 1;
  const bool want_dQ = mixed && a.dQ != nullptr;
  float* Ds = smem;
  float* WsT = Ds + (size_t)t.rowsP * DP;
  float* DY = WsT + (size_t)Hout * LP4;
  float* DF = DY + (size_t)t.rowsP * LP;
  float* Fin = DF + (mixed ? (size_t)t.rowsP * LP : 0);
  float* Qs = Fin + (want_dQ ? (size_t)t.rowsP * LP : 0);

  const long long total_nodes = (long long)a.B * a.N;
  const long long g0 = (long long)blockIdx.x * t.npt;
  const int nodes_valid = (int)min((long long)t.npt, total_nodes - g0);
  const int rows_valid = nodes_valid * C;
  const long long row0 = g0 * C;
  const long long R = total_nodes * C;
  const FeatSrc fs = feat_src(a);
  const int RG = t.rowsP / 4, CGL = LP4 / 4;

  for (int i = threadIdx.x; i < (a.Kc - 1) * C * C; i += blockDim.x) Qs[i] = a.Q[C * C + i];

  for (int idx = threadIdx.x; idx < t.rowsP * h; idx += blockDim.x) {
    const int row = idx / h, j = idx - row * h;
    const long long o = (row0 + row) * h + j;
    if (row < rows_valid) {
      const float dhn = a.dHn[o], uu = a.u[o], cc = a.c[o];
      if (a.phase == 1) {
        float g = dhn * uu * (1.f - cc * cc);
        if (a.act == STC_ACT_RELU && !(cc > 0.f)) g = 0.f;
        Ds[row * DP + j] = g;
        a.dpre[(row0 + row) * a.dpre_ld + j] = g;
      } else {
        const float hp = a.Hprev[o], rr = a.r[o], drh = a.drH[o];
        float gu = dhn * (cc - hp) * uu * (1.f - uu);
        float gr = drh * hp * rr * (1.f - rr);
        if (a.act == STC_ACT_RELU) {
          if (!(uu > 0.5f)) gu = 0.f;
          if (!(rr > 0.5f)) gr = 0.f;
        }
        Ds[row * DP + j] = gu;
        Ds[row * DP + h + j] = gr;
        a.dpre[(row0 + row) * a.dpre_ld + j] = gu;
        a.dpre[(row0 + row) * a.dpre_ld + h + j] = gr;
        a.dYh0[o] = dhn * (1.f - uu) + drh * rr;
      }
    } else {
      Ds[row * DP + j] = 0.f;
      if (a.phase == 0) Ds[row * DP + h + j] = 0.f;
    }
  }
  __syncthreads();
  if (a.dbias) {
    for (int j = threadIdx.x; j < Hout; j += blockDim.x) {
      float s = 0.f;
      for (int row = 0; row < rows_valid; ++row) s += Ds[row * DP + j];
      atomicAdd(&a.dbias[j], s);
    }
  }

  for (int k = 0; k < a.Ks; ++k) {
    __syncthreads();
    for (int idx = threadIdx.x; idx < t.rowsP * LP; idx += blockDim.x) DY[idx] = 0.f;
    if (want_dQ) load_feat_tile(fs, k, g0, nodes_valid, t.rowsP, Fin, LP);
    for (int c = 0; c < a.Kc; ++c) {
      __syncthreads();
      const float* Wblk = a.W + (size_t)(k * a.Kc + c) * L * Hout;
      for (int idx = threadIdx.x; idx < Hout * LP4; idx += blockDim.x) {
        int j = idx / LP4, l = idx - j * LP4;
        WsT[idx] = (l < L) ? Wblk[l * Hout + j] : 0.f;
      }
      __syncthreads();
      float acc[NI][4][4];
#pragma unroll
      for (int i = 0; i < NI; ++i)
#pragma unroll
        for (int x = 0; x < 4; ++x)
#pragma unroll
          for (int y = 0; y < 4; ++y) acc[i][x][y] = 0.f;
      tile_gemm<NI>(acc, Ds, DP, WsT, LP4, Hout, RG, CGL);
      float* dst = (c == 0) ? DY : DF;
      const int items = RG * CGL;
#pragma unroll
      for (int i = 0; i < NI; ++i) {
        const int it = threadIdx.x + i * CV_THREADS;
        if (it >= items) break;
        const int rg = it / CGL, lg = it - rg * CGL;
#pragma unroll
        for (int x = 0; x < 4; ++x)
#pragma unroll
          for (int y = 0; y < 4; ++y) {
            const int l = lg * 4 + y;
            if (l < L) {
              float* p = dst + (rg * 4 + x) * LP + l;
              if (c == 0) *p += acc[i][x][y]; else *p = acc[i][x][y];
            }
          }
      }
      if (c > 0) {
        __syncthreads();
        const float* Qc = Qs + (size_t)(c - 1) * C * C;
        unmix_add_tile(DF, DY, Qc, rows_valid, C, L, LP);
        if (want_dQ) {
          for (int pr = threadIdx.x; pr < C * C; pr += blockDim.x) {
            const int cp = pr / C, d = pr - cp * C;
            float s = 0.f;
            for (int node = 0; node < nodes_valid; ++node) {
              const float* y = Fin + (node * C + cp) * LP;
              const float* f = DF + (node * C + d) * LP;
              for (int l = 0; l < L; ++l) s = fmaf(y[l], f[l], s);
            }
            atomicAdd(&a.dQ[(size_t)c * C * C + pr], s);
          }
        }
      }
    }
    __syncthreads();
    {
      float* dx = (k == 0) ? a.dYx0 : a.dYx + (size_t)(k - 1) * R * Din;
      if (dx) {
        dx += row0 * Din;
        for (int idx = threadIdx.x; idx < rows_valid * Din; idx += blockDim.x) {
          int row = idx / Din, l = idx - row * Din;
          float v = DY[row * LP + l];
          dx[idx] = a.accum_x ? dx[idx] + v : v;
        }
      }
      float* dh = (k == 0) ? a.dYh0 : a.dYh + (size_t)(k - 1) * R * h;
      dh += row0 * h;
      const bool add_direct = (k == 0 && a.phase == 0);
      for (int idx = threadIdx.x; idx < rows_valid * h; idx += blockDim.x) {
        int row = idx / h, l = idx - row * h;
        float v = DY[row * LP + Din + l];
        dh[idx] = add_direct ? dh[idx] + v : v;
      }
    }
  }
}

static size_t conv_dx_smem(const ConvArgs& a, const ConvTile& t, int DP) {
  const bool mixed = a.Kc > 1;
  const bool want_dQ = mixed && a.dQ != nullptr;
  size_t f = (size_t)t.rowsP * DP + (size_t)a.Hout * t.LP4 + (size_t)t.rowsP * t.LP * (1 + (mixed ? 1 : 0) + (want_dQ ? 1 : 0)) +
             (size_t)(mixed ? (a.Kc - 1) : 0) * a.C * a.C;
  return f * sizeof(float);
}

int launch_conv_bwd_dx(const ConvArgs& a, cudaStream_t st) {
  {
    bool handled = false;
    STC_TRY(try_launch_conv_bwd_dx_tc(a, st, &handled));
    if (handled) return STC_OK;
    STC_TRY(try_launch_conv_bwd_dx_big(a, st, &handled));
    if (handled) return STC_OK;
  }
  const int L = a.Din + a.h;
  const int CGL = ((L + 3) & ~3) / 4;
  const int HoutP = (a.Hout + 3) & ~3;
  const int DP = HoutP | 1;
  int target = 4 * CV_THREADS * 2 / CGL;
  if (target > 128) target = 128;
  if (target < 4) target = 4;
  ConvTile t; size_t smem; int ni;
  for (;;) {
    t = make_tile(a, target);
    smem = conv_dx_smem(a, t, DP);
    ni = ceil_div((t.rowsP / 4) * CGL, CV_THREADS);
    if (smem <= 200 * 1024 && ni <= CV_MAX_NI) break;
    if (t.npt == 1) {
      set_error("conv backward tile does not fit: C=%d Din=%d h=%d Hout=%d needs %zu B smem, %d items/thread", a.C,
                a.Din, a.h, a.Hout, smem, ni);
      return STC_ERR_UNSUPPORTED;
    }
    target = (t.npt / 2) * a.C;
    if (target < a.C) target = a.C;
  }
  long long total_nodes = (long long)a.B * a.N;
  int grid = ceil_div(total_nodes, t.npt);
  const double R = (double)total_nodes * a.C;
  ScopedKernelTimer _t(KK_CONV_BWD_DX, st,
                       4.0 * R * ((a.phase == 0 ? 7 * a.h + a.Ks * a.Din : 3 * a.h) + a.Hout + a.Ks * L +
                                  ((a.dQ && a.Kc > 1) ? a.Ks * L : 0)) + 4.0 * a.Ks * a.Kc * L * a.Hout);
  switch (ni) {
    case 1: STC_TRY(set_smem(conv_bwd_dx_kernel<1>, smem)); conv_bwd_dx_kernel<1><<<grid, CV_THREADS, smem, st>>>(a, t, DP); break;
    case 2: STC_TRY(set_smem(conv_bwd_dx_kernel<2>, smem)); conv_bwd_dx_kernel<2><<<grid, CV_THREADS, smem, st>>>(a, t, DP); break;
    default: STC_TRY(set_smem(conv_bwd_dx_kernel<4>, smem)); conv_bwd_dx_kernel<4><<<grid, CV_THREADS, smem, st>>>(a, t, DP); break;
  }
  STC_LAUNCH_OK("conv_bwd_dx_kernel");
  return STC_OK;
}

constexpr int DW_SLAB = 64;

template <int NI>
__global__ void __launch_bounds__(CV_THREADS)
conv_bwd_dw_kernel(const ConvArgs a, const ConvTile t, const int tiles_per_cta) {
  extern __shared__ __align__(16) float smem[];
  const int C = a.C, L = t.L, LP4 = t.LP4, Hout = a.Hout;
  const int blk = blockIdx.y, k = blk / a.Kc, c = blk - k * a.Kc;
  const int col0 = blockIdx.z * DW_SLAB;
  const int ncol = min(DW_SLAB, Hout - col0);
  const int SP = (ncol + 3) & ~3;
  float* Fin = smem;
  float* Fmx = Fin + (size_t)t.rowsP * LP4;
  float* Dsm = Fmx + (c > 0 ? (size_t)t.rowsP * LP4 : 0);
  float* Qs = Dsm + (size_t)t.rowsP * DW_SLAB;
  const FeatSrc fs = feat_src(a);
  const long long total_nodes = (long long)a.B * a.N;
  const long long ntiles = (total_nodes + t.npt - 1) / t.npt;

  if (c > 0)
    for (int i = threadIdx.x; i < C * C; i += blockDim.x) Qs[i] = a.Q[(size_t)c * C * C + i];

  const int LG = LP4 / 4, CG = SP / 4, IT = LG * CG;
  int G = 1, g = 0, item0 = threadIdx.x;
  bool active = true;
  if (IT < CV_THREADS) {
    G = CV_THREADS / IT;
    g = threadIdx.x / IT;
    item0 = threadIdx.x - g * IT;
    active = g < G;
  }
  float acc[NI][4][4];
#pragma unroll
  for (int i = 0; i < NI; ++i)
#pragma unroll
    for (int x = 0; x < 4; ++x)
#pragma unroll
      for (int y = 0; y < 4; ++y) acc[i][x][y] = 0.f;

  for (int idx = threadIdx.x; idx < t.rowsP * LP4 * (c > 0 ? 2 : 1); idx += blockDim.x) Fin[idx] = 0.f;

  const long long tile_lo = (long long)blockIdx.x * tiles_per_cta;
  const long long tile_hi = min(ntiles, tile_lo + tiles_per_cta);
  for (long long tile = tile_lo; tile < tile_hi; ++tile) {
    const long long g0 = tile * t.npt;
    const int nodes_valid = (int)min((long long)t.npt, total_nodes - g0);
    const int rows_valid = nodes_valid * C;
    const long long row0 = g0 * C;
    __syncthreads();
    load_feat_tile(fs, k, g0, nodes_valid, rows_valid, Fin, LP4);
    for (int idx = threadIdx.x; idx < rows_valid * SP; idx += blockDim.x) {
      int row = idx / SP, j = idx - row * SP;
      Dsm[row * SP + j] = (j < ncol) ? a.dpre[(row0 + row) * a.dpre_ld + col0 + j] : 0.f;
    }
    __syncthreads();
    const float* F = Fin;
    if (c > 0) {
      mix_tile(Fin, Fmx, Qs, rows_valid, C, L, LP4);
      F = Fmx;
      __syncthreads();
    }
    if (active) {
#pragma unroll
      for (int i = 0; i < NI; ++i) {
        const int it = item0 + i * CV_THREADS;
        if (it >= IT) break;
        const int lg = it / CG, cg = it - lg * CG;
        for (int row = g; row < rows_valid; row += G) {
          float4 f = *reinterpret_cast<const float4*>(F + row * LP4 + lg * 4);
          float4 d = *reinterpret_cast<const float4*>(Dsm + row * SP + cg * 4);
          acc[i][0][0] = fmaf(f.x, d.x, acc[i][0][0]); acc[i][0][1] = fmaf(f.x, d.y, acc[i][0][1]);
          acc[i][0][2] = fmaf(f.x, d.z, acc[i][0][2]); acc[i][0][3] = fmaf(f.x, d.w, acc[i][0][3]);
          acc[i][1][0] = fmaf(f.y, d.x, acc[i][1][0]); acc[i][1][1] = fmaf(f.y, d.y, acc[i][1][1]);
          acc[i][1][2] = fmaf(f.y, d.z, acc[i][1][2]); acc[i][1][3] = fmaf(f.y, d.w, acc[i][1][3]);
          acc[i][2][0] = fmaf(f.z, d.x, acc[i][2][0]); acc[i][2][1] = fmaf(f.z, d.y, acc[i][2][1]);
          acc[i][2][2] = fmaf(f.z, d.z, acc[i][2][2]); acc[i][2][3] = fmaf(f.z, d.w, acc[i][2][3]);
          acc[i][3][0] = fmaf(f.w, d.x, acc[i][3][0]); acc[i][3][1] = fmaf(f.w, d.y, acc[i][3][1]);
          acc[i][3][2] = fmaf(f.w, d.z, acc[i][3][2]); acc[i][3][3] = fmaf(f.w, d.w, acc[i][3][3]);
        }
      }
    }
  }
  if (active) {
    float* dWblk = a.dW + (size_t)blk * L * Hout;
#pragma unroll
    for (int i = 0; i < NI; ++i) {
      const int it = item0 + i * CV_THREADS;
      if (it >= IT) break;
      const int lg = it / CG, cg = it - lg * CG;
#pragma unroll
      for (int x = 0; x < 4; ++x) {
        const int l = lg * 4 + x;
        if (l >= L) continue;
#pragma unroll
        for (int y = 0; y < 4; ++y) {
          const int j = cg * 4 + y;
// ... 60 lines not shown
```

### stc_gnn_b200/csrc/stc_conv_tc_big.cu

```cuda
#include "stc_conv_common.cuh"
#include "stc_tc.cuh"

#include <stdlib.h>
#include <string.h>

namespace stc {

using namespace tc;

constexpr int BG_STAGES = 3;
constexpr int BG_THREADS = 512;
constexpr int BG_FWD_THREADS = BG_THREADS + 32;
constexpr int BG_ACOL = 384;

struct BigPlan {
  int npt, Dp, KBL;
  int nchk;
  int nch;
  int ntiles;
  int PS;
  int x_vec;
  uint32_t stage_bytes;
  uint32_t off_b, off_pm, off_q, off_bias, off_bar, smem_bytes;
  int land;
// ... 555 lines not shown
      for (int t_ = 0; t_ < my_tiles; ++t_) {
        for (int k = 0; k < a.Ks; ++k, ++terms) {
          for (int kc = 0; kc < p.nkc; ++kc, ++g) {
            const int buf = (int)(g & 1u), st = (int)(g % (uint32_t)p.stages);
            if (kc == 0 && terms > 0) mbar_wait(acc_empty, (terms - 1u) & 1u);
            mbar_wait(&a_full[buf], (g >> 1) & 1u);
            mbar_wait(&b_full[st], (g / (uint32_t)p.stages) & 1u);
            fence_after_sync();
            const uint32_t a_hi0 = tmem_base + (uint32_t)(BG_ACOL + 64 * buf);
            const uint64_t dBh = make_smem_desc_sw128(smem_u32(Bring + (size_t)st * p.stage_bytes));
            const uint64_t dBl = dBh + (uint64_t)(((uint32_t)Nb * ATOM_ROW_BYTES) >> 4);
#pragma unroll
            for (int ks = 0; ks < 4; ++ks) {
              const uint64_t ko = (uint64_t)(ks * 2);
              const uint32_t ah = a_hi0 + (uint32_t)(ks * 8), al = ah + 32u;
              const uint32_t d_main = tmem_base + (uint32_t)((ks & 1) * Nb);
              mma_tf32_atmem(d_small, al, dBh + ko, idesc, (kc > 0 || ks > 0) ? 1u : 0u);
              mma_tf32_atmem(d_main, ah, dBh + ko, idesc, (kc > 0 || ks >= 2) ? 1u : 0u);
              mma_tf32_atmem(d_small, ah, dBl + ko, idesc, 1u);
            }
            mma_commit(&a_free[buf]);
            mma_commit(&b_free[st]);
            if (kc == p.nkc - 1) mma_commit(acc_full);
            const uint32_t t = g + (uint32_t)(p.stages - 1);
            if (t < total_chunks) {
              const uint32_t ts = t % (uint32_t)p.stages, tu = t / (uint32_t)p.stages;
              if (tu >= 1u) mbar_wait(&b_free[ts], (tu - 1u) & 1u);
              mbar_arrive_expect_tx(&b_full[ts], p.stage_bytes);
              bulk_g2s(Bring + (size_t)ts * p.stage_bytes, img_of(t), p.stage_bytes, &b_full[ts]);
            }
          }
        }
      }
    }
    __syncwarp();
  } else {
  uint32_t g = 0;
  uint32_t acc_phase = 0;
  for (int tile = blockIdx.x; tile < p.ntiles; tile += gridDim.x) {
    const long long g0 = (long long)tile * p.npt;
    const int nodes_valid = (int)min((long long)p.npt, total_nodes - g0);
    const int rows_valid = nodes_valid * C;
    const long long row0 = g0 * C;
    const bool valid = erow < rows_valid;
    const long long gr = row0 + erow;
    const int cpr = h >> 2;
    for (int it = tid; it < 128 * cpr; it += BG_THREADS) {
      const int row = it / cpr, j = (it - row * cpr) << 2;
      float4 g0v = make_float4(0.f, 0.f, 0.f, 0.f), g1v = g0v;
      if (row < rows_valid) {
        const long long o = (row0 + row) * h + j;
        const float4 dhn = *reinterpret_cast<const float4*>(a.dHn + o);
        const float4 uu = *reinterpret_cast<const float4*>(a.u + o);
        const float4 cc = *reinterpret_cast<const float4*>(a.c + o);
        if (a.phase == 1) {
          g0v = make_float4(dhn.x * uu.x * (1.f - cc.x * cc.x), dhn.y * uu.y * (1.f - cc.y * cc.y),
                            dhn.z * uu.z * (1.f - cc.z * cc.z), dhn.w * uu.w * (1.f - cc.w * cc.w));
          if (a.act == STC_ACT_RELU) {
            if (!(cc.x > 0.f)) g0v.x = 0.f;
            if (!(cc.y > 0.f)) g0v.y = 0.f;
            if (!(cc.z > 0.f)) g0v.z = 0.f;
            if (!(cc.w > 0.f)) g0v.w = 0.f;
          }
          *reinterpret_cast<float4*>(a.dpre + (row0 + row) * a.dpre_ld + j) = g0v;
        } else {
          const float4 hp = *reinterpret_cast<const float4*>(a.Hprev + o);
          const float4 rr = *reinterpret_cast<const float4*>(a.r + o);
          const float4 drh = *reinterpret_cast<const float4*>(a.drH + o);
          g0v = make_float4(dhn.x * (cc.x - hp.x) * uu.x * (1.f - uu.x), dhn.y * (cc.y - hp.y) * uu.y * (1.f - uu.y),
                            dhn.z * (cc.z - hp.z) * uu.z * (1.f - uu.z), dhn.w * (cc.w - hp.w) * uu.w * (1.f - uu.w));
          g1v = make_float4(drh.x * hp.x * rr.x * (1.f - rr.x), drh.y * hp.y * rr.y * (1.f - rr.y),
                            drh.z * hp.z * rr.z * (1.f - rr.z), drh.w * hp.w * rr.w * (1.f - rr.w));
          if (a.act == STC_ACT_RELU) {
            if (!(uu.x > 0.5f)) g0v.x = 0.f;
            if (!(uu.y > 0.5f)) g0v.y = 0.f;
            if (!(uu.z > 0.5f)) g0v.z = 0.f;
            if (!(uu.w > 0.5f)) g0v.w = 0.f;
            if (!(rr.x > 0.5f)) g1v.x = 0.f;
            if (!(rr.y > 0.5f)) g1v.y = 0.f;
            if (!(rr.z > 0.5f)) g1v.z = 0.f;
            if (!(rr.w > 0.5f)) g1v.w = 0.f;
          }
          *reinterpret_cast<float4*>(a.dpre + (row0 + row) * a.dpre_ld + j) = g0v;
          *reinterpret_cast<float4*>(a.dpre + (row0 + row) * a.dpre_ld + h + j) = g1v;
          *reinterpret_cast<float4*>(a.dYh0 + o) =
              make_float4(dhn.x * (1.f - uu.x) + drh.x * rr.x, dhn.y * (1.f - uu.y) + drh.y * rr.y,
                          dhn.z * (1.f - uu.z) + drh.z * rr.z, dhn.w * (1.f - uu.w) + drh.w * rr.w);
        }
      }
      *reinterpret_cast<float4*>(Dsm + row * DP + j) = g0v;
      if (a.phase == 0) *reinterpret_cast<float4*>(Dsm + row * DP + h + j) = g1v;
    }
    bg_producer_sync();
    if (a.dbias && tid < Hout) {
      float sacc = 0.f;
      for (int row = 0; row < rows_valid; ++row) sacc += Dsm[row * DP + tid];
      db_acc += sacc;
    }
    if (want_dQ && (C & 7) == 0) {
      const int nblk = C >> 3;
      for (int item = tid; item < C * nblk; item += BG_THREADS) {
        const int cp = item / nblk, dblk = item - cp * nblk;
        float sacc[8];
#pragma unroll
        for (int j = 0; j < 8; ++j) sacc[j] = 0.f;
        for (int node = 0; node < nodes_valid; ++node) {
          const float* pp = a.Psave + (row0 + node * C + cp) * (long long)Hout;
          const float* dd = Dsm + (node * C + dblk) * DP;
          for (int o = 0; o < Hout; o += 4) {
            const float4 x = *reinterpret_cast<const float4*>(pp + o);
#pragma unroll
            for (int j = 0; j < 8; ++j) {
              const float4 y = *reinterpret_cast<const float4*>(dd + (size_t)(j * nblk) * DP + o);
              sacc[j] = fmaf(x.x, y.x, sacc[j]); sacc[j] = fmaf(x.y, y.y, sacc[j]);
              sacc[j] = fmaf(x.z, y.z, sacc[j]); sacc[j] = fmaf(x.w, y.w, sacc[j]);
            }
          }
        }
#pragma unroll
        for (int j = 0; j < 8; ++j) dQacc[cp * C + dblk + j * nblk] += sacc[j];
      }
    } else if (want_dQ) {
      for (int pr = tid; pr < C * C; pr += BG_THREADS) {
        const int cp = pr / C, d = pr - cp * C;
        float sacc = 0.f;
        for (int node = 0; node < nodes_valid; ++node) {
          const float* pp = a.Psave + (row0 + node * C + cp) * (long long)Hout;
          const float* dd = Dsm + (node * C + d) * DP;
          for (int o = 0; o < Hout; o += 4) {
            const float4 x = *reinterpret_cast<const float4*>(pp + o);
            const float4 y = *reinterpret_cast<const float4*>(dd + o);
            sacc = fmaf(x.x, y.x, sacc); sacc = fmaf(x.y, y.y, sacc); sacc = fmaf(x.z, y.z, sacc); sacc = fmaf(x.w, y.w, sacc);
          }
        }
        dQacc[pr] += sacc;
      }
    }
    auto reload_ok = [&](int k_, int kc_) {
      return k_ > 0 && kc_ < p.nkc && (32 * kc_ + 8 * qtr) >= Hout && valid && a.dpre_ld >= 2 * Hout;
    };
    float4 nx0 = make_float4(0.f, 0.f, 0.f, 0.f), nx1 = nx0;
    for (int k = 0; k < a.Ks; ++k) {
      float4 prev[4][2];
#pragma unroll
      for (int gi = 0; gi < 4; ++gi) {
        prev[gi][0] = prev[gi][1] = make_float4(0.f, 0.f, 0.f, 0.f);
        const int c0 = 8 * qtr + 32 * gi;
        if (c0 < Nb && valid) {
          if (c0 < h) {
            if (k == 0 && a.phase == 0) {
              const float4* src = reinterpret_cast<const float4*>(a.dYh0 + gr * h + c0);
              prev[gi][0] = src[0];
              prev[gi][1] = src[1];
            }
          } else {
            const int xi = c0 - h;
            if (xi < Din && xvec && a.accum_x) {
              const float* src = (k == 0 ? a.dYx0 : a.dYx + (size_t)(k - 1) * R * Din) + gr * Din + xi;
              prev[gi][0] = *reinterpret_cast<const float4*>(src);
              if (xi + 4 < Din) prev[gi][1] = *reinterpret_cast<const float4*>(src + 4);
            }
          }
        }
      }
      if (reload_ok(k, 0)) {
        const float4* dp = reinterpret_cast<const float4*>(a.dpre + gr * a.dpre_ld + 8 * qtr);
        nx0 = dp[0];
        nx1 = dp[1];
      }
      for (int kc = 0; kc < p.nkc; ++kc, ++g) {
        const int kk0 = 32 * kc + 8 * qtr;
        float av[8];
        if (kk0 < Hout) {
          const float4 x0 = *reinterpret_cast<const float4*>(Dsm + erow * DP + kk0);
          const float4 x1 = *reinterpret_cast<const float4*>(Dsm + erow * DP + kk0 + 4);
          av[0] = x0.x; av[1] = x0.y; av[2] = x0.z; av[3] = x0.w; av[4] = x1.x; av[5] = x1.y; av[6] = x1.z; av[7] = x1.w;
        } else if (k > 0 && valid && a.dpre_ld >= 2 * Hout) {
          av[0] = nx0.x; av[1] = nx0.y; av[2] = nx0.z; av[3] = nx0.w; av[4] = nx1.x; av[5] = nx1.y; av[6] = nx1.z; av[7] = nx1.w;
        } else {
          const float* spm = Dsm + (enode * C) * DP + (kk0 - Hout);
#pragma unroll
          for (int i = 0; i < 8; ++i) av[i] = 0.f;
          if (valid) {
#pragma unroll 4
            for (int d = 0; d < C; ++d) {
              const float w = qrow[d];
              const float4 x0 = *reinterpret_cast<const float4*>(spm + d * DP);
              const float4 x1 = *reinterpret_cast<const float4*>(spm + d * DP + 4);
              av[0] = fmaf(w, x0.x, av[0]); av[1] = fmaf(w, x0.y, av[1]); av[2] = fmaf(w, x0.z, av[2]); av[3] = fmaf(w, x0.w, av[3]);
              av[4] = fmaf(w, x1.x, av[4]); av[5] = fmaf(w, x1.y, av[5]); av[6] = fmaf(w, x1.z, av[6]); av[7] = fmaf(w, x1.w, av[7]);
            }
          }
        }
        if (reload_ok(k, kc + 1)) {
          const float4* dp = reinterpret_cast<const float4*>(a.dpre + gr * a.dpre_ld + kk0 + 32);
          nx0 = dp[0];
          nx1 = dp[1];
        }
        if (k == 0 && kk0 >= Hout && valid && a.dpre_ld >= 2 * Hout) {
          float4* dp = reinterpret_cast<float4*>(a.dpre + gr * a.dpre_ld + kk0);
          dp[0] = make_float4(av[0], av[1], av[2], av[3]);
          dp[1] = make_float4(av[4], av[5], av[6], av[7]);
        }
        const int buf = (int)(g & 1u);
        const uint32_t ua = g >> 1;
        if (ua >= 1u) {
          mbar_wait(&a_free[buf], (ua - 1u) & 1u);
          fence_after_sync();
        }
        {
          const uint32_t tA = tl + (uint32_t)(BG_ACOL + 64 * buf + 8 * qtr);
          float hi[8], lo[8];
#pragma unroll
          for (int i = 0; i < 8; ++i) split_tf32(av[i], hi[i], lo[i]);
          tmem_st8(tA, hi);
          tmem_st8(tA + 32u, lo);
        }
        tmem_st_wait();
        fence_before_sync();
        __syncwarp();
        if (lane == 0) mbar_arrive(&a_full[buf]);
      }
      mbar_wait(acc_full, acc_phase);
      acc_phase ^= 1u;
      fence_after_sync();
#pragma unroll
      for (int gi = 0; gi < 4; ++gi) {
        const int c0 = 8 * qtr + 32 * gi;
        if (c0 >= Nb) break;
        float v[8];
        {
          uint32_t t0[8], t1[8], t2[8];
          tmem_ld8_async(tl + (uint32_t)(2 * Nb + c0), t2);
          tmem_ld8_async(tl + (uint32_t)c0, t0);
          tmem_ld8_async(tl + (uint32_t)(Nb + c0), t1);
          tmem_ld_wait();
          tmem_ld_pin8(t0); tmem_ld_pin8(t1); tmem_ld_pin8(t2);
#pragma unroll
          for (int i = 0; i < 8; ++i) v[i] = (__uint_as_float(t2[i]) + __uint_as_float(t0[i])) + __uint_as_float(t1[i]);
        }
        if (!valid) continue;
        const float4 p0 = prev[gi][0], p1 = prev[gi][1];
        if (c0 < h) {
          float* dst = (k == 0 ? a.dYh0 : a.dYh + (size_t)(k - 1) * R * h) + gr * h + c0;
          reinterpret_cast<float4*>(dst)[0] = make_float4(v[0] + p0.x, v[1] + p0.y, v[2] + p0.z, v[3] + p0.w);
          reinterpret_cast<float4*>(dst)[1] = make_float4(v[4] + p1.x, v[5] + p1.y, v[6] + p1.z, v[7] + p1.w);
        } else {
          const int xi = c0 - h;
          if (xi >= Din) continue;
          float* dst = (k == 0 ? a.dYx0 : a.dYx + (size_t)(k - 1) * R * Din) + gr * Din + xi;
          if (xvec) {
            reinterpret_cast<float4*>(dst)[0] = make_float4(v[0] + p0.x, v[1] + p0.y, v[2] + p0.z, v[3] + p0.w);
            if (xi + 4 < Din) reinterpret_cast<float4*>(dst)[1] = make_float4(v[4] + p1.x, v[5] + p1.y, v[6] + p1.z, v[7] + p1.w);
          } else {
#pragma unroll
            for (int i = 0; i < 8; ++i)
              if (xi + i < Din) dst[i] = a.accum_x ? dst[i] + v[i] : v[i];
          }
        }
      }
      fence_before_sync();
      __syncwarp();
      if (lane == 0) mbar_arrive(acc_empty);
      bg_producer_sync();
    }
  }
  if (a.dbias && tid < Hout) atomicAdd(&a.dbias[tid], db_acc);
  if (want_dQ)
    for (int i = tid; i < C * C; i += BG_THREADS) atomicAdd(&a.dQ[C * C + i], dQacc[i]);
  }
  __syncthreads();
  if (warp == 0) tmem_dealloc(tmem_base, 512u);
}

static bool big_dx_shape_ok(const ConvArgs& a) {
  if (!conv_big_shape_ok(a.C, a.Din, a.h, a.Ks, a.Kc, a.Hout)) return false;
  const int KBLp = (a.h + ((a.Din + 7) & ~7) + 15) & ~15;
  if (KBLp > 128) return false;
  const size_t smem = (size_t)2 * 2 * KBLp * ATOM_ROW_BYTES + (size_t)(128 + a.C) * (a.Hout + 4) * sizeof(float) +
                      2 * (size_t)a.C * a.C * sizeof(float) + 2048;
  return smem <= 220 * 1024;
}

size_t conv_big_dx_img_floats(int C, int Din, int h, int Ks, int Kc, int Hout) {
  ConvArgs a;
  memset(&a, 0, sizeof(a));
  a.C = C; a.Din = Din; a.h = h; a.Ks = Ks; a.Kc = Kc; a.Hout = Hout;
  if (!big_dx_shape_ok(a)) return 0;
  const int KBLp = (h + ((Din + 7) & ~7) + 15) & ~15;
  return (size_t)Ks * (2 * Hout / 32) * 2 * KBLp * (ATOM_ROW_BYTES / sizeof(float));
}

int try_launch_conv_bwd_dx_big(const ConvArgs& a, cudaStream_t st, bool* handled) {
  *handled = false;
  if (a.Wimg == nullptr || !big_dx_shape_ok(a) || (a.opt & OPT_WIDE_DX_FFMA)) return STC_OK;
  if (!aligned16g(a.dHn) || !aligned16g(a.u) || !aligned16g(a.c) || !aligned16g(a.Hprev) || !aligned16g(a.dpre) ||
      !aligned16g(a.dYh0) || !aligned16g(a.dYh) || !aligned16g(a.Psave) || (a.dpre_ld % 4) != 0 ||
      (a.phase == 0 && (!aligned16g(a.r) || !aligned16g(a.drH))) || ((reinterpret_cast<uintptr_t>(a.Wimg) & 127) != 0)) {
    set_error("tcgen05 wide-state backward needs 16-byte aligned gradient / workspace tensors");
    return STC_ERR_BAD_ARG;
  }
  BigDxPlan p;
  p.npt = 128 / a.C;
  p.Dp = (a.Din + 7) & ~7;
  p.KBL = a.h + p.Dp;
  p.KBLp = (p.KBL + 15) & ~15;
  p.nkc = 2 * a.Hout / 32;
  p.DP = a.Hout + 4;
  p.x_vec = (a.Din % 4 == 0) && aligned16g(a.dYx0) && aligned16g(a.dYx);
  const long long total_nodes = (long long)a.B * a.N;
  p.ntiles = ceil_div(total_nodes, p.npt);
  p.stage_bytes = (uint32_t)(2 * p.KBLp * ATOM_ROW_BYTES);
  const size_t rest = round_up((size_t)(128 + a.C) * p.DP * sizeof(float), 16) +
                      2 * round_up((size_t)a.C * a.C * sizeof(float), 16) + 8 * (2 * BG_STAGES + 3) + 16;
  p.stages = ((size_t)BG_STAGES * p.stage_bytes + rest <= 226 * 1024) ? BG_STAGES : 2;
  size_t o = 0;
  p.off_b = (uint32_t)o; o += (size_t)p.stages * p.stage_bytes;
  p.off_ds = (uint32_t)o; o += round_up((size_t)(128 + a.C) * p.DP * sizeof(float), 16);
  p.off_q = (uint32_t)o; o += round_up((size_t)a.C * a.C * sizeof(float), 16);
  p.off_qacc = (uint32_t)o; o += round_up((size_t)a.C * a.C * sizeof(float), 16);
  p.off_bar = (uint32_t)o; o += 8 * (2 * BG_STAGES + 6) + 16;
  p.smem_bytes = (uint32_t)o;
  if (p.smem_bytes > 226 * 1024) return STC_OK;
  {
    const long long items = (long long)a.Ks * p.nkc * p.KBLp * 8;
    tc_big_dx_prep_kernel<<<(int)min((items + 255) / 256, (long long)1024), 256, 0, st>>>(
        a.W, reinterpret_cast<uint8_t*>(a.Wimg), a.Din, a.h, a.Ks, a.Kc, a.Hout, p.KBL, p.KBLp, p.nkc);
    STC_LAUNCH_OK("tc_big_dx_prep_kernel");
  }
  STC_TRY(set_smem(tc_conv_bwd_dx_big_kernel, p.smem_bytes));
  int grid = device_sm_count();
  if (grid > p.ntiles) grid = p.ntiles;
  const int L = a.Din + a.h;
  const double R = (double)total_nodes * a.C;
  ScopedKernelTimer _t(KK_TC_CONV_BWD_DX, st,
                       4.0 * R * ((a.phase == 0 ? 6 * a.h + a.Ks * a.Din : 3 * a.h) + a.Hout + a.Ks * L +
                                  (a.dQ ? a.Hout : 0)) + 4.0 * a.Ks * a.Kc * L * a.Hout);
  tc_conv_bwd_dx_big_kernel<<<grid, BG_FWD_THREADS, p.smem_bytes, st>>>(a, p, reinterpret_cast<const uint8_t*>(a.Wimg));
  STC_LAUNCH_OK("tc_conv_bwd_dx_big_kernel");
  *handled = true;
  return STC_OK;
}

constexpr int BG_DW_CR = 32;
constexpr int BG_DW_DRAIN = 4;

struct BigDwPlan {
  int Dp, KBL, N1, NH;
  int nsplit;
  long long rows_per;
  int x_vec;
  uint32_t img_bytes;
  uint32_t off_img, off_bar, smem_bytes;
};

__global__ void __launch_bounds__(BG_THREADS, 1)
tc_conv_bwd_dw_big_kernel(const ConvArgs a, const BigDwPlan p) {
  extern __shared__ __align__(1024) uint8_t smem[];
  if ((smem_u32(smem) & 1023u) != 0u) __trap();
  const int tid = threadIdx.x, warp = tid >> 5, lane = tid & 31;
  const int C = a.C, h = a.h, Din = a.Din, Hout = a.Hout, L = a.Din + a.h;
  constexpr uint32_t IMG1 = 4u * BG_DW_CR * ATOM_ROW_BYTES;
  uint8_t* img = smem + p.off_img;
  uint64_t* img_free = reinterpret_cast<uint64_t*>(smem + p.off_bar);
  uint64_t* acc_full = img_free + 2;
  uint32_t* tmem_slot = reinterpret_cast<uint32_t*>(acc_full + 1);
  if (tid == 0) {
    mbar_init(&img_free[0], 1);
    mbar_init(&img_free[1], 1);
    mbar_init(acc_full, 1);
    mbar_fence_init();
  }
  if (warp == 0) tmem_alloc(tmem_slot, 512u);
  fence_before_sync();
  __syncthreads();
  fence_after_sync();
  const int warp_u = uniform_warp_index();
  const uint32_t tmem_base = uniform_u32(*tmem_slot);
  const uint32_t idesc = make_idesc_tf32_mn(128, 128);
  const uint32_t d_small = tmem_base + 256u;
  const long long total_nodes = (long long)a.B * a.N;
  const long long R = total_nodes * C;

  const int T = a.Ks * p.NH;
  const int tile = (int)blockIdx.x % T, split = (int)blockIdx.x / T;
  const int k = tile / p.NH, nh = tile - k * p.NH;
  const long long rbeg = (long long)split * p.rows_per;
  const long long rend = min(R, rbeg + p.rows_per);
  const int nchunks = rbeg < rend ? (int)((rend - rbeg + BG_DW_CR - 1) / BG_DW_CR) : 0;

  const int cq = tid & 31, r0 = tid >> 5;
  const int m0 = 4 * cq;
  const uint32_t soff0 = (uint32_t)(m0 >> 5) * (BG_DW_CR * ATOM_ROW_BYTES);
  int apart = 2;
  int aoff = 0;
  if (m0 < h) { apart = 0; aoff = m0; }
  else if (m0 - h < Din) { apart = 1; aoff = m0 - h; }
  const int anvalid = apart == 1 ? min(4, Din - aoff) : 4;
  const bool avec = apart == 0 || (apart == 1 && p.x_vec && anvalid == 4);
  const int bn = nh * 128 + m0;
  const bool blive = bn < p.N1;
  const float* hsrc = (k == 0 ? a.h0 : a.yh + (size_t)(k - 1) * R * h);
  const float* xsrc = (k == 0 ? a.x0 : a.yx + (size_t)(k - 1) * R * Din);

  auto fetch = [&](int ch, float4 (&fa)[2], float4 (&fb)[2]) {
#pragma unroll
    for (int i = 0; i < 2; ++i) {
      const long long row = rbeg + (long long)ch * BG_DW_CR + r0 + 16 * i;
      fa[i] = fb[i] = make_float4(0.f, 0.f, 0.f, 0.f);
      if (row >= rend) continue;
      if (apart == 0) {
        fa[i] = *reinterpret_cast<const float4*>(hsrc + row * h + aoff);
      } else if (apart == 1) {
        const float* xs;
        if (k == 0) {
          const long long rows_per_sample = (long long)a.N * C;
          const long long b = row / rows_per_sample;
          xs = xsrc + b * a.x0_bs + (row - b * rows_per_sample) * Din + aoff;
        } else {
          xs = xsrc + row * Din + aoff;
        }
        if (avec) {
          fa[i] = *reinterpret_cast<const float4*>(xs);
        } else {
          fa[i].x = xs[0];
          if (anvalid > 1) fa[i].y = xs[1];
          if (anvalid > 2) fa[i].z = xs[2];
          if (anvalid > 3) fa[i].w = xs[3];
        }
      }
      if (blive) fb[i] = *reinterpret_cast<const float4*>(a.dpre + row * a.dpre_ld + bn);
    }
  };

  const int sp = warp & 3, qtr = warp >> 2;
  const int mrow = sp * 32 + lane;
  const uint32_t tl = tmem_base + ((uint32_t)(sp * 32) << 16);
  float acc[4][8];
#pragma unroll
  for (int i = 0; i < 4; ++i)
#pragma unroll
    for (int j = 0; j < 8; ++j) acc[i][j] = 0.f;
  uint32_t acc_phase = 0;
  auto drain = [&]() {
    mbar_wait(acc_full, acc_phase);
    acc_phase ^= 1u;
    fence_after_sync();
#pragma unroll
    for (int i = 0; i < 4; ++i) {
      uint32_t t0[8], t1[8], t2[8];
      const uint32_t c0 = (uint32_t)(32 * qtr + 8 * i);
      tmem_ld8_async(tl + 256u + c0, t2);
      tmem_ld8_async(tl + c0, t0);
      tmem_ld8_async(tl + 128u + c0, t1);
      tmem_ld_wait();
      tmem_ld_pin8(t0); tmem_ld_pin8(t1); tmem_ld_pin8(t2);
#pragma unroll
      for (int j = 0; j < 8; ++j)
        acc[i][j] += (__uint_as_float(t2[j]) + __uint_as_float(t0[j])) + __uint_as_float(t1[j]);
    }
    fence_before_sync();
    __syncthreads();
// ... 118 lines not shown
```

### stc_gnn_b200/csrc/stc_conv_tc_bwd.cu

```cuda
#include "stc_conv_common.cuh"
#include "stc_tc.cuh"

namespace stc {

using namespace tc;

constexpr int DX_APM = 3;

struct TcDxPlan {
  int npt, Dp, KBL;
  int N1;
  int Npad;
  int Kdd;
  int KA;
  int nmain;
  int tmem_cols, ntiles;
  int DP;
  int PW;
  int x_vec;
  uint32_t off_a, off_b, off_ds, off_dh, off_ps, off_q, off_acc, off_bar, smem_bytes;
};

struct DxIn {
  float4 dhn, uu, cc, hp, rr, drh;
};
__device__ __forceinline__ void dx_load(const ConvArgs& a, long long o, DxIn& in) {
  in.dhn = *reinterpret_cast<const float4*>(a.dHn + o);
  in.uu = *reinterpret_cast<const float4*>(a.u + o);
  in.cc = *reinterpret_cast<const float4*>(a.c + o);
  if (a.phase == 0) {
    in.hp = *reinterpret_cast<const float4*>(a.Hprev + o);
    in.rr = *reinterpret_cast<const float4*>(a.r + o);
    in.drh = *reinterpret_cast<const float4*>(a.drH + o);
  }
}
__device__ __forceinline__ void dx_adjoint(const ConvArgs& a, const DxIn& in, float4& g0v, float4& g1v, float4& dir) {
  const float4 dhn = in.dhn, uu = in.uu, cc = in.cc;
  if (a.phase == 1) {
    g0v = make_float4(dhn.x * uu.x * (1.f - cc.x * cc.x), dhn.y * uu.y * (1.f - cc.y * cc.y),
                      dhn.z * uu.z * (1.f - cc.z * cc.z), dhn.w * uu.w * (1.f - cc.w * cc.w));
    if (a.act == STC_ACT_RELU) {
      if (!(cc.x > 0.f)) g0v.x = 0.f;
      if (!(cc.y > 0.f)) g0v.y = 0.f;
      if (!(cc.z > 0.f)) g0v.z = 0.f;
      if (!(cc.w > 0.f)) g0v.w = 0.f;
    }
  } else {
    const float4 hp = in.hp, rr = in.rr, drh = in.drh;
    g0v = make_float4(dhn.x * (cc.x - hp.x) * uu.x * (1.f - uu.x), dhn.y * (cc.y - hp.y) * uu.y * (1.f - uu.y),
                      dhn.z * (cc.z - hp.z) * uu.z * (1.f - uu.z), dhn.w * (cc.w - hp.w) * uu.w * (1.f - uu.w));
    g1v = make_float4(drh.x * hp.x * rr.x * (1.f - rr.x), drh.y * hp.y * rr.y * (1.f - rr.y),
                      drh.z * hp.z * rr.z * (1.f - rr.z), drh.w * hp.w * rr.w * (1.f - rr.w));
    if (a.act == STC_ACT_RELU) {
      if (!(uu.x > 0.5f)) g0v.x = 0.f;
      if (!(uu.y > 0.5f)) g0v.y = 0.f;
      if (!(uu.z > 0.5f)) g0v.z = 0.f;
      if (!(uu.w > 0.5f)) g0v.w = 0.f;
      if (!(rr.x > 0.5f)) g1v.x = 0.f;
      if (!(rr.y > 0.5f)) g1v.y = 0.f;
      if (!(rr.z > 0.5f)) g1v.z = 0.f;
      if (!(rr.w > 0.5f)) g1v.w = 0.f;
    }
    dir = make_float4(dhn.x * (1.f - uu.x) + drh.x * rr.x, dhn.y * (1.f - uu.y) + drh.y * rr.y,
                      dhn.z * (1.f - uu.z) + drh.z * rr.z, dhn.w * (1.f - uu.w) + drh.w * rr.w);
  }
}

__device__ __forceinline__ void dx_prefetch_tile(const ConvArgs& a, const TcDxPlan& p, int tile, bool want_dQ) {
  const long long total_nodes = (long long)a.B * a.N;
  const long long g0 = (long long)tile * p.npt;
  const int nv = (int)min((long long)p.npt, total_nodes - g0);
  const long long row0 = g0 * a.C;
  const uint32_t hb = (uint32_t)(nv * a.C * a.h * 4);
  l2_prefetch(a.dHn + row0 * a.h, hb);
  l2_prefetch(a.u + row0 * a.h, hb);
  l2_prefetch(a.c + row0 * a.h, hb);
  if (a.phase == 0) {
    l2_prefetch(a.Hprev + row0 * a.h, hb);
    l2_prefetch(a.r + row0 * a.h, hb);
    l2_prefetch(a.drH + row0 * a.h, hb);
  }
  if (want_dQ) l2_prefetch(a.Psave + row0 * p.PW, (uint32_t)(nv * a.C * p.PW * 4));
  if (a.accum_x && p.x_vec) {
    const uint32_t xb = (uint32_t)(nv * a.C * a.Din * 4);
    const long long R = total_nodes * a.C;
    if (a.dYx0) l2_prefetch(a.dYx0 + row0 * a.Din, xb);
    if (a.dYx)
      for (int k = 1; k < a.Ks; ++k) l2_prefetch(a.dYx + (size_t)(k - 1) * R * a.Din + row0 * a.Din, xb);
  }
}

template <bool FAST, bool AT>
__global__ void __launch_bounds__(CV_THREADS, 2)
tc_conv_bwd_dx_kernel(const ConvArgs a, const TcDxPlan p) {
  extern __shared__ __align__(1024) uint8_t smem[];
  if ((smem_u32(smem) & 1023u) != 0u) __trap();
  const int tid = threadIdx.x, warp = tid >> 5, lane = tid & 31;
  const int C = a.C, L = a.Din + a.h, h = a.h, Din = a.Din, Hout = a.Hout, DP = p.DP;
  const bool want_dQ = a.dQ != nullptr && a.Kc > 1;
  const uint32_t atomA = 128 * ATOM_ROW_BYTES;
  const uint32_t atomB = (uint32_t)p.Npad * ATOM_ROW_BYTES;
  uint8_t* A_hi = smem + p.off_a;
  uint8_t* A_lo = A_hi + atomA;
  uint8_t* B_hi = smem + p.off_b;
  uint8_t* B_lo = B_hi + (AT ? (size_t)atomB : (size_t)p.KA * atomB);
  const size_t bstride = AT ? 2 * (size_t)atomB : (size_t)atomB;
  float* Dsm = reinterpret_cast<float*>(smem + p.off_ds);
  float* Dh = reinterpret_cast<float*>(smem + p.off_dh);
  float* Psm = reinterpret_cast<float*>(smem + p.off_ps);
  float* Qs = reinterpret_cast<float*>(smem + p.off_q);
  float* dQacc = reinterpret_cast<float*>(smem + p.off_acc);
  uint64_t* mma_bar = reinterpret_cast<uint64_t*>(smem + p.off_bar);
  uint64_t* load_bar = mma_bar + 1;
  uint32_t* tmem_slot = reinterpret_cast<uint32_t*>(mma_bar + 2);

  if (tid == 0) {
    mbar_init(mma_bar, 1);
    mbar_init(load_bar, 1);
    mbar_fence_init();
  }
  if (warp == 0) tmem_alloc(tmem_slot, (uint32_t)p.tmem_cols);
  for (int i = tid; i < (a.Kc - 1) * C * C; i += CV_THREADS) {
    Qs[i] = a.Q[C * C + i];
    dQacc[i] = 0.f;
  }
  for (int ja = 0; ja < p.KA; ++ja) {
    uint8_t* bh = B_hi + (size_t)ja * bstride;
    uint8_t* bl = B_lo + (size_t)ja * bstride;
    for (int it = tid; it < p.Npad * 8; it += CV_THREADS) {
      const int n = it >> 3, qq = it & 7;
      const int k = n / p.KBL, kb = n - k * p.KBL;
      const int l = kb < h ? Din + kb : (kb - h < Din ? kb - h : -1);
      float v[4];
#pragma unroll
      for (int i = 0; i < 4; ++i) {
        const int kk = ja * ATOM_K + qq * 4 + i;
        const int c = kk / Hout, o = kk - c * Hout;
        v[i] = (n < p.N1 && l >= 0 && kk < p.Kdd) ? a.W[((size_t)(k * a.Kc + c) * L + l) * Hout + o] : 0.f;
      }
      store_split4(bh, bl, atom_chunk_offset(n, qq), make_float4(v[0], v[1], v[2], v[3]));
    }
  }
  fence_async_smem();
  fence_before_sync();
  __syncthreads();
  fence_after_sync();
  const int warp_u = uniform_warp_index();
  const uint32_t tmem_base = uniform_u32(*tmem_slot);
  const uint32_t idesc = make_idesc_tf32(128, p.Npad), idesc2 = make_idesc_tf32(128, 2 * p.Npad);
  const uint32_t d_small = tmem_base + (uint32_t)(p.nmain * p.Npad);
  const uint64_t dA_hi = make_smem_desc_sw128(smem_u32(A_hi)), dA_lo = make_smem_desc_sw128(smem_u32(A_lo));
  const uint64_t dB_hi = make_smem_desc_sw128(smem_u32(B_hi)), dB_lo = make_smem_desc_sw128(smem_u32(B_lo));
  const long long total_nodes = (long long)a.B * a.N;
  const long long R = total_nodes * C;

  const int q = tid & 7, r0 = tid >> 3;
  uint32_t aoff[4];
  int rnode[4], rcat[4];
#pragma unroll
  for (int i = 0; i < 4; ++i) {
    aoff[i] = atom_chunk_offset(r0 + 32 * i, q);
    rnode[i] = (r0 + 32 * i) / C;
    rcat[i] = (r0 + 32 * i) - rnode[i] * C;
  }
  const int lane_base = (warp & 3) * 32, half = warp >> 2;
  const int erow = lane_base + lane;
  const uint32_t tl = tmem_base + ((uint32_t)lane_base << 16);
  const bool db_fast = a.dbias != nullptr && (CV_THREADS % (h >> 2)) == 0;
  float4 dbs0 = make_float4(0.f, 0.f, 0.f, 0.f), dbs1 = dbs0;
  float db_acc = 0.f;
  const int db_groups = CV_THREADS / Hout, db_col = tid % Hout, db_grp = tid / Hout;
  constexpr int DQ_C = 5;
  const int dq_chunks = Hout >> 2;
  const bool dq_fast = want_dQ && a.Kc == 2 && C <= DQ_C && p.npt * dq_chunks <= CV_THREADS;
  const int dq_node = tid / dq_chunks, dq_oc = (tid - dq_node * dq_chunks) << 2;
  float dq[DQ_C * DQ_C];
#pragma unroll
  for (int i = 0; i < DQ_C * DQ_C; ++i) dq[i] = 0.f;
  uint32_t mma_phase = 0, load_phase = 0;
  bool mma_pending = false;
  const bool tracing = a.trace != nullptr && blockIdx.x == 0 && tid == 0;
  int trace_it = 0;

  for (int tile = blockIdx.x; tile < p.ntiles; tile += gridDim.x) {
    const long long g0 = (long long)tile * p.npt;
    const int nodes_valid = (int)min((long long)p.npt, total_nodes - g0);
    const int rows_valid = nodes_valid * C;
    const long long row0 = g0 * C;
    if (warp_u == 1 && elect_one_sync()) {
      if (want_dQ) {
        const uint32_t bytes = (uint32_t)(rows_valid * p.PW * 4);
        mbar_arrive_expect_tx(load_bar, bytes);
        bulk_g2s(Psm, a.Psave + row0 * p.PW, bytes, load_bar);
      }
      if ((a.opt & OPT_L2_PREFETCH) && tile + (int)gridDim.x < p.ntiles) dx_prefetch_tile(a, p, tile + gridDim.x, want_dQ);
    }
    STC_TRACE(0);
    const int cpr = h >> 2;
    auto emit_item = [&](int row, int j, const float4& g0v, const float4& g1v, const float4& dir, bool live) {
      if (live) {
        *reinterpret_cast<float4*>(a.dpre + (row0 + row) * p.Kdd + j) = g0v;
        if (a.phase == 0) *reinterpret_cast<float4*>(a.dpre + (row0 + row) * p.Kdd + h + j) = g1v;
      }
      if (db_fast) {
        dbs0.x += g0v.x; dbs0.y += g0v.y; dbs0.z += g0v.z; dbs0.w += g0v.w;
        dbs1.x += g1v.x; dbs1.y += g1v.y; dbs1.z += g1v.z; dbs1.w += g1v.w;
      }
      *reinterpret_cast<float4*>(Dsm + row * DP + j) = g0v;
      if (a.phase == 0) {
        *reinterpret_cast<float4*>(Dsm + row * DP + h + j) = g1v;
        *reinterpret_cast<float4*>(Dh + row * h + j) = dir;
      }
    };
    for (int it = tid; it < 128 * cpr; it += CV_THREADS) {
      const int row = it / cpr, j = (it - row * cpr) << 2;
      float4 g0v = make_float4(0.f, 0.f, 0.f, 0.f), g1v = g0v, dir = g0v;
      const bool live = row < rows_valid;
      if (live) {
        DxIn in;
        dx_load(a, (row0 + row) * h + j, in);
        dx_adjoint(a, in, g0v, g1v, dir);
      }
      emit_item(row, j, g0v, g1v, dir, live);
    }
    __syncthreads();
    STC_TRACE(1);
    if (a.dbias && !db_fast && tid < db_groups * Hout) {
      float s = 0.f;
      for (int row = db_grp; row < rows_valid; row += db_groups) s += Dsm[row * DP + db_col];
      db_acc += s;
    }
    if constexpr (AT) {
      const int cw = Hout >> 1;
      const int cbase = cw * half;
      const int enode = erow / C, ecat = erow - enode * C;
      const float* qrow = Qs + ecat * C;
      const uint32_t tA = tl + (uint32_t)(2 * p.Npad);
      const bool two = cw == 16;
      float dm[16];
#pragma unroll
      for (int i = 0; i < 16; ++i) dm[i] = 0.f;
      {
        const float* sp = Dsm + (enode * C) * DP + cbase;
#pragma unroll 5
        for (int d = 0; d < C; ++d) {
          const float w = qrow[d];
          const float4 x0 = *reinterpret_cast<const float4*>(sp + d * DP);
          const float4 x1 = *reinterpret_cast<const float4*>(sp + d * DP + 4);
          dm[0] = fmaf(w, x0.x, dm[0]); dm[1] = fmaf(w, x0.y, dm[1]); dm[2] = fmaf(w, x0.z, dm[2]); dm[3] = fmaf(w, x0.w, dm[3]);
          dm[4] = fmaf(w, x1.x, dm[4]); dm[5] = fmaf(w, x1.y, dm[5]); dm[6] = fmaf(w, x1.z, dm[6]); dm[7] = fmaf(w, x1.w, dm[7]);
          if (two) {
            const float4 x2 = *reinterpret_cast<const float4*>(sp + d * DP + 8);
            const float4 x3 = *reinterpret_cast<const float4*>(sp + d * DP + 12);
            dm[8] = fmaf(w, x2.x, dm[8]); dm[9] = fmaf(w, x2.y, dm[9]); dm[10] = fmaf(w, x2.z, dm[10]); dm[11] = fmaf(w, x2.w, dm[11]);
            dm[12] = fmaf(w, x3.x, dm[12]); dm[13] = fmaf(w, x3.y, dm[13]); dm[14] = fmaf(w, x3.z, dm[14]); dm[15] = fmaf(w, x3.w, dm[15]);
          }
        }
      }
      if (erow < rows_valid) {
        float* dp = a.dpre + (row0 + erow) * p.Kdd + Hout + cbase;
        *reinterpret_cast<float4*>(dp) = make_float4(dm[0], dm[1], dm[2], dm[3]);
        *reinterpret_cast<float4*>(dp + 4) = make_float4(dm[4], dm[5], dm[6], dm[7]);
        if (two) {
          *reinterpret_cast<float4*>(dp + 8) = make_float4(dm[8], dm[9], dm[10], dm[11]);
          *reinterpret_cast<float4*>(dp + 12) = make_float4(dm[12], dm[13], dm[14], dm[15]);
        }
      }
#pragma unroll
      for (int part = 0; part < 2; ++part) {
        if (part * 8 < cw) {
          const int col = cbase + part * 8;
          float hi[8], lo[8];
          {
            const float4 x0 = *reinterpret_cast<const float4*>(Dsm + erow * DP + col);
            const float4 x1 = *reinterpret_cast<const float4*>(Dsm + erow * DP + col + 4);
            split_tf32(x0.x, hi[0], lo[0]); split_tf32(x0.y, hi[1], lo[1]); split_tf32(x0.z, hi[2], lo[2]); split_tf32(x0.w, hi[3], lo[3]);
            split_tf32(x1.x, hi[4], lo[4]); split_tf32(x1.y, hi[5], lo[5]); split_tf32(x1.z, hi[6], lo[6]); split_tf32(x1.w, hi[7], lo[7]);
          }
          tmem_st8(tA + (uint32_t)col, hi);
          tmem_st8(tA + 64u + (uint32_t)col, lo);
#pragma unroll
          for (int i = 0; i < 8; ++i) split_tf32(dm[part * 8 + i], hi[i], lo[i]);
          tmem_st8(tA + (uint32_t)(Hout + col), hi);
          tmem_st8(tA + 64u + (uint32_t)(Hout + col), lo);
        }
      }
      tmem_st_wait();
      STC_TRACE(12);
      fence_before_sync();
      STC_TRACE(13);
      __syncthreads();
      STC_TRACE(2);
      if (warp_u == 0 && elect_one_sync()) {
        fence_after_sync();
        const uint32_t a0 = tmem_base + (uint32_t)(2 * p.Npad);
        uint32_t acc = 0u;
        const int nks = p.Kdd >> 3;
        for (int ks = 0; ks < nks; ++ks) {
          const uint64_t bo = (uint64_t)((((uint32_t)(ks >> 2)) * 2u * atomB) >> 4) + (uint64_t)((ks & 3) * 2);
          const uint32_t ah = a0 + (uint32_t)(ks * 8), al = ah + 64u;
          mma_tf32_atmem(tmem_base, ah, dB_hi + bo, idesc2, acc);
          mma_tf32_atmem(d_small, al, dB_hi + bo, idesc, 1u);
          acc = 1u;
        }
        STC_TRACE(8);
        STC_TRACE(10);
        mma_commit(mma_bar);
        STC_TRACE(9);
        STC_TRACE(11);
      }
      mma_pending = true;
    } else {
      bool acc_small = false;
      for (int ja = 0; ja < p.KA; ++ja) {
        const int kk = ja * ATOM_K + q * 4;
        const int c = kk / Hout, o0 = kk - c * Hout;
        float4 vv[4];
  #pragma unroll
        for (int i = 0; i < 4; ++i) {
          float4 v = make_float4(0.f, 0.f, 0.f, 0.f);
          if (kk < p.Kdd) {
            if (c == 0) {
              v = *reinterpret_cast<const float4*>(Dsm + (r0 + 32 * i) * DP + o0);
            } else {
              const float* Qc = Qs + (size_t)(c - 1) * C * C + rcat[i] * C;
              const float* sp = Dsm + rnode[i] * C * DP + o0;
              for (int d = 0; d < C; ++d) {
                const float w = Qc[d];
                const float4 x = *reinterpret_cast<const float4*>(sp + d * DP);
                v.x = fmaf(w, x.x, v.x); v.y = fmaf(w, x.y, v.y); v.z = fmaf(w, x.z, v.z); v.w = fmaf(w, x.w, v.w);
              }
              if (r0 + 32 * i < rows_valid)
                *reinterpret_cast<float4*>(a.dpre + (row0 + r0 + 32 * i) * p.Kdd + kk) = v;
            }
          }
          vv[i] = v;
        }
        if (mma_pending) {
          mbar_wait(mma_bar, mma_phase);
          mma_phase ^= 1u;
          mma_pending = false;
        }
  #pragma unroll
        for (int i = 0; i < 4; ++i) store_split4(A_hi, A_lo, aoff[i], vv[i]);
        if (ja == 0) STC_TRACE(12);
        fence_async_smem();
        if (ja == 0) STC_TRACE(13);
        __syncthreads();
        if (ja == 0) STC_TRACE(2);
        if (warp_u == 0 && elect_one_sync()) {
          fence_after_sync();
          const int kleft = p.Kdd - ja * ATOM_K;
          const int ksteps = kleft >= ATOM_K ? 4 : (kleft + 7) / 8;
          const uint64_t bo = (uint64_t)(((uint32_t)ja * atomB) >> 4);
          const uint32_t d_main = tmem_base + (uint32_t)((ja / DX_APM) * p.Npad);
          uint32_t acc_main = (ja % DX_APM) != 0 ? 1u : 0u;
  #pragma unroll 4
          for (int ks = 0; ks < ksteps; ++ks) {
            const uint64_t ko = (uint64_t)(ks * 2);
            mma_tf32(d_small, dA_lo + ko, dB_hi + bo + ko, idesc, acc_small ? 1u : 0u);
            mma_tf32(d_small, dA_hi + ko, dB_lo + bo + ko, idesc, 1u);
            mma_tf32(d_main, dA_hi + ko, dB_hi + bo + ko, idesc, acc_main);
            acc_main = 1u;
            acc_small = true;
          }
          if (ja == 0) STC_TRACE(8);
          if (ja == p.KA - 1) STC_TRACE(10);
          mma_commit(mma_bar);
          if (ja == 0) STC_TRACE(9);
          if (ja == p.KA - 1) STC_TRACE(11);
        }
        acc_small = true;
        mma_pending = true;
      }
    }
    STC_TRACE(3);
    float4 xprev[4];
#pragma unroll
    for (int i = 0; i < 4; ++i) xprev[i] = make_float4(0.f, 0.f, 0.f, 0.f);
    if constexpr (FAST) {
      if (a.accum_x && p.x_vec && erow < rows_valid) {
        const float* dbase_pf = (half == 0 ? a.dYx0 : a.dYx);
        if (dbase_pf != nullptr) {
          const float* src = dbase_pf + (row0 + erow) * Din;
#pragma unroll
          for (int i = 0; i < 4; ++i)
            if (4 * i < Din) xprev[i] = *reinterpret_cast<const float4*>(src + 4 * i);
        }
      }
    }
    if (want_dQ) {
      mbar_wait(load_bar, load_phase);
      load_phase ^= 1u;
      const int npairs = (a.Kc - 1) * C * C;
      const int groups = CV_THREADS / npairs;
      if (dq_fast) {
        if (dq_node < nodes_valid) {
          float4 pv[DQ_C], dv[DQ_C];
#pragma unroll
          for (int i = 0; i < DQ_C; ++i) {
            const int ci = i < C ? i : 0;
            pv[i] = *reinterpret_cast<const float4*>(Psm + (dq_node * C + ci) * p.PW + dq_oc);
            dv[i] = *reinterpret_cast<const float4*>(Dsm + (dq_node * C + ci) * DP + dq_oc);
          }
#pragma unroll
          for (int cp = 0; cp < DQ_C; ++cp)
#pragma unroll
            for (int d = 0; d < DQ_C; ++d) {
              float s = dq[cp * DQ_C + d];
              s = fmaf(pv[cp].x, dv[d].x, s); s = fmaf(pv[cp].y, dv[d].y, s);
              s = fmaf(pv[cp].z, dv[d].z, s); s = fmaf(pv[cp].w, dv[d].w, s);
              dq[cp * DQ_C + d] = s;
            }
        }
      } else if (groups >= 1) {
        const int pr = tid % npairs, grp = tid / npairs;
        if (grp < groups) {
          const int c = pr / (C * C), rem = pr - c * C * C, cp = rem / C, d = rem - cp * C;
          float s = 0.f;
          for (int node = grp; node < nodes_valid; node += groups) {
            const float* pp = Psm + (node * C + cp) * p.PW + c * Hout;
            const float* dd = Dsm + (node * C + d) * DP;
            for (int o = 0; o < Hout; o += 4) {
              const float4 x = *reinterpret_cast<const float4*>(pp + o);
              const float4 y = *reinterpret_cast<const float4*>(dd + o);
              s = fmaf(x.x, y.x, s); s = fmaf(x.y, y.y, s); s = fmaf(x.z, y.z, s); s = fmaf(x.w, y.w, s);
            }
          }
          atomicAdd(&dQacc[pr], s);
        }
      } else {
        for (int pr = tid; pr < npairs; pr += CV_THREADS) {
          const int c = pr / (C * C), rem = pr - c * C * C, cp = rem / C, d = rem - cp * C;
          float s = 0.f;
          for (int node = 0; node < nodes_valid; ++node) {
            const float* pp = Psm + (node * C + cp) * p.PW + c * Hout;
            const float* dd = Dsm + (node * C + d) * DP;
            for (int o = 0; o < Hout; ++o) s = fmaf(pp[o], dd[o], s);
          }
          dQacc[pr] += s;
        }
      }
    }
    STC_TRACE(4);
    mbar_wait(mma_bar, mma_phase);
    mma_phase ^= 1u;
    mma_pending = false;
    fence_after_sync();
    STC_TRACE(5);
    const bool valid = erow < rows_valid;
    const long long gr = row0 + erow;
    if constexpr (FAST) {
      const int k = half;
      const uint32_t nb = (uint32_t)(k * p.KBL);
      {
        uint32_t sm[16], mn[16];
        tmem_ld16_async(tl + (uint32_t)p.Npad + nb, sm);
        tmem_ld16_async(tl + nb, mn);
        tmem_ld_wait();
        tmem_ld_pin16(sm); tmem_ld_pin16(mn);
        if (valid) {
          float v[16];
#pragma unroll
          for (int i = 0; i < 16; ++i) v[i] = __uint_as_float(sm[i]) + __uint_as_float(mn[i]);
          if (k == 0 && a.phase == 0) {
#pragma unroll
            for (int i = 0; i < 16; i += 4) {
              const float4 d = *reinterpret_cast<const float4*>(Dh + erow * 16 + i);
              v[i] += d.x; v[i + 1] += d.y; v[i + 2] += d.z; v[i + 3] += d.w;
            }
          }
          float* dst = (k == 0 ? a.dYh0 : a.dYh) + gr * 16;
#pragma unroll
          for (int i = 0; i < 16; i += 4) *reinterpret_cast<float4*>(dst + i) = make_float4(v[i], v[i + 1], v[i + 2], v[i + 3]);
        }
      }
      float* dbase = (k == 0 ? a.dYx0 : a.dYx);
      {
        uint32_t sm[16], mn[16];
        if (p.Dp == 16) {
          tmem_ld16_async(tl + (uint32_t)p.Npad + nb + 16u, sm);
          tmem_ld16_async(tl + nb + 16u, mn);
          tmem_ld_wait();
          tmem_ld_pin16(sm); tmem_ld_pin16(mn);
        } else {
          uint32_t s8[8], m8[8];
          tmem_ld8_async(tl + (uint32_t)p.Npad + nb + 16u, s8);
          tmem_ld8_async(tl + nb + 16u, m8);
          tmem_ld_wait();
          tmem_ld_pin8(s8); tmem_ld_pin8(m8);
#pragma unroll
          for (int i = 0; i < 8; ++i) { sm[i] = s8[i]; mn[i] = m8[i]; sm[i + 8] = 0u; mn[i + 8] = 0u; }
        }
        if (valid && dbase != nullptr) {
          float* dst = dbase + gr * Din;
          if (p.x_vec) {
            float4 o[4];
#pragma unroll
            for (int i = 0; i < 4; ++i)
              o[i] = make_float4(__uint_as_float(sm[4 * i]) + __uint_as_float(mn[4 * i]),
                                 __uint_as_float(sm[4 * i + 1]) + __uint_as_float(mn[4 * i + 1]),
                                 __uint_as_float(sm[4 * i + 2]) + __uint_as_float(mn[4 * i + 2]),
                                 __uint_as_float(sm[4 * i + 3]) + __uint_as_float(mn[4 * i + 3]));
            if (a.accum_x) {
#pragma unroll
              for (int i = 0; i < 4; ++i)
                if (4 * i < Din) { o[i].x += xprev[i].x; o[i].y += xprev[i].y; o[i].z += xprev[i].z; o[i].w += xprev[i].w; }
            }
#pragma unroll
            for (int i = 0; i < 4; ++i)
              if (4 * i < Din) *reinterpret_cast<float4*>(dst + 4 * i) = o[i];
          } else {
#pragma unroll
            for (int i = 0; i < 16; ++i)
              if (i < Din) {
                const float vi = __uint_as_float(sm[i]) + __uint_as_float(mn[i]);
                dst[i] = a.accum_x ? dst[i] + vi : vi;
              }
          }
        }
      }
    } else {
      int k = 0, kb = half * 8;
      for (int n0 = half * 8; n0 < p.Npad; n0 += 16, kb += 16) {
        float v[8];
        if (p.nmain == 1) {
          uint32_t t0[8], t1[8];
          tmem_ld8_async(tl + (uint32_t)(p.Npad + n0), t1);
          tmem_ld8_async(tl + (uint32_t)n0, t0);
          tmem_ld_wait();
          tmem_ld_pin8(t0); tmem_ld_pin8(t1);
#pragma unroll
          for (int i = 0; i < 8; ++i) v[i] = __uint_as_float(t1[i]) + __uint_as_float(t0[i]);
        } else {
          float t[8];
          tmem_ld8(tl + (uint32_t)(p.nmain * p.Npad + n0), v);
          for (int m = 0; m < p.nmain; ++m) {
            tmem_ld8(tl + (uint32_t)(m * p.Npad + n0), t);
#pragma unroll
            for (int i = 0; i < 8; ++i) v[i] += t[i];
          }
        }
        while (kb >= p.KBL) { kb -= p.KBL; ++k; }
        if (!valid || n0 >= p.N1) continue;
        if (kb < h) {
          float* dst = (k == 0 ? a.dYh0 : a.dYh + (size_t)(k - 1) * R * h) + gr * h + kb;
          if (k == 0 && a.phase == 0) {
            const float* dp = Dh + erow * h + kb;
#pragma unroll
            for (int i = 0; i < 8; ++i) v[i] += dp[i];
          }
          reinterpret_cast<float4*>(dst)[0] = make_float4(v[0], v[1], v[2], v[3]);
          reinterpret_cast<float4*>(dst)[1] = make_float4(v[4], v[5], v[6], v[7]);
        } else {
          const int xi = kb - h;
          float* dbase = (k == 0 ? a.dYx0 : a.dYx + (size_t)(k - 1) * R * Din);
          if (dbase == nullptr) continue;
          float* dst = dbase + gr * Din + xi;
          if (p.x_vec && xi + 8 <= Din) {
            float4 o0 = make_float4(v[0], v[1], v[2], v[3]), o1 = make_float4(v[4], v[5], v[6], v[7]);
            if (a.accum_x) {
              const float4 p0 = reinterpret_cast<const float4*>(dst)[0], p1 = reinterpret_cast<const float4*>(dst)[1];
              o0.x += p0.x; o0.y += p0.y; o0.z += p0.z; o0.w += p0.w;
              o1.x += p1.x; o1.y += p1.y; o1.z += p1.z; o1.w += p1.w;
            }
            reinterpret_cast<float4*>(dst)[0] = o0;
            reinterpret_cast<float4*>(dst)[1] = o1;
          } else {
#pragma unroll
            for (int i = 0; i < 8; ++i)
              if (xi + i < Din) dst[i] = a.accum_x ? dst[i] + v[i] : v[i];
          }
        }
      }
    }
    STC_TRACE(6);
    fence_before_sync();
    fence_async_smem();
    __syncthreads();
    STC_TRACE(7);
    ++trace_it;
  }
  if (a.dbias && !db_fast && tid < db_groups * Hout) atomicAdd(&a.dbias[db_col], db_acc);
  __syncthreads();
  if (db_fast) {
    for (int i = tid; i < Hout; i += CV_THREADS) Dsm[i] = 0.f;
    __syncthreads();
    const int cprw = h >> 2;
    float v[8] = {dbs0.x, dbs0.y, dbs0.z, dbs0.w, dbs1.x, dbs1.y, dbs1.z, dbs1.w};
    for (int off = cprw; off < 32; off <<= 1) {
#pragma unroll
      for (int i = 0; i < 8; ++i) v[i] += __shfl_xor_sync(0xffffffffu, v[i], off);
    }
    if (lane < cprw || cprw >= 32) {
      const int j = (tid % cprw) << 2;
      atomicAdd(&Dsm[j + 0], v[0]); atomicAdd(&Dsm[j + 1], v[1]); atomicAdd(&Dsm[j + 2], v[2]); atomicAdd(&Dsm[j + 3], v[3]);
      if (a.phase == 0) {
        atomicAdd(&Dsm[h + j + 0], v[4]); atomicAdd(&Dsm[h + j + 1], v[5]);
        atomicAdd(&Dsm[h + j + 2], v[6]); atomicAdd(&Dsm[h + j + 3], v[7]);
      }
    }
    __syncthreads();
    for (int i = tid; i < Hout; i += CV_THREADS) atomicAdd(&a.dbias[i], Dsm[i]);
  }
  if (dq_fast) {
#pragma unroll
    for (int cp = 0; cp < DQ_C; ++cp)
#pragma unroll
      for (int d = 0; d < DQ_C; ++d) {
        float s = dq[cp * DQ_C + d];
#pragma unroll
        for (int off = 16; off >= 1; off >>= 1) s += __shfl_xor_sync(0xffffffffu, s, off);
        if (lane == 0 && cp < C && d < C) atomicAdd(&dQacc[cp * C + d], s);
      }
  }
  __syncthreads();
  if (want_dQ)
    for (int i = tid; i < (a.Kc - 1) * C * C; i += CV_THREADS) atomicAdd(&a.dQ[C * C + i], dQacc[i]);
  if (warp == 0) tmem_dealloc(tmem_base, (uint32_t)p.tmem_cols);
}

static bool aligned16b(const void* p) { return (reinterpret_cast<uintptr_t>(p) & 15) == 0; }

int try_launch_conv_bwd_dx_tc(const ConvArgs& a, cudaStream_t st, bool* handled) {
  *handled = false;
  if (!conv_tc_eligible(a)) return STC_OK;
  if (!aligned16b(a.dHn) || !aligned16b(a.u) || !aligned16b(a.c) || !aligned16b(a.Hprev) || !aligned16b(a.dpre) ||
      !aligned16b(a.dYh0) || !aligned16b(a.dYh) || !aligned16b(a.Psave) || (a.phase == 0 && (!aligned16b(a.r) || !aligned16b(a.drH)))) {
    set_error("tcgen05 backward needs 16-byte aligned gradient / workspace tensors");
    return STC_ERR_BAD_ARG;
  }
  const int L = a.Din + a.h;
  TcDxPlan p;
  p.npt = 128 / a.C;
  p.Dp = (a.Din + 7) & ~7;
  p.KBL = a.h + p.Dp;
  p.N1 = a.Ks * p.KBL;
  p.Npad = (p.N1 + 15) & ~15;
  p.Kdd = a.Kc * a.Hout;
  p.KA = (p.Kdd + ATOM_K - 1) / ATOM_K;
  p.nmain = (p.KA + DX_APM - 1) / DX_APM;
  p.tmem_cols = 32;
  while (p.tmem_cols < (p.nmain + 1) * p.Npad) p.tmem_cols *= 2;
  p.DP = a.Hout + 4;
  p.PW = (a.Kc - 1) * a.Hout;
  p.x_vec = (a.Din % 4 == 0) && aligned16b(a.dYx0) && aligned16b(a.dYx);
  const long long total_nodes = (long long)a.B * a.N;
  p.ntiles = ceil_div(total_nodes, p.npt);
  const size_t atomB = (size_t)p.Npad * ATOM_ROW_BYTES;
  size_t o = 0;
  p.off_a = (uint32_t)o; o += 2 * 128 * ATOM_ROW_BYTES;
  p.off_b = (uint32_t)o; o += 2 * (size_t)p.KA * atomB;
  p.off_ds = (uint32_t)o; o += (size_t)128 * p.DP * sizeof(float);
  p.off_dh = (uint32_t)o; o += (size_t)128 * a.h * sizeof(float);
  p.off_ps = (uint32_t)o; o += round_up((size_t)128 * p.PW * sizeof(float), 16);
  p.off_q = (uint32_t)o; o += round_up((size_t)(a.Kc > 1 ? a.Kc - 1 : 0) * a.C * a.C * sizeof(float), 16);
  p.off_acc = (uint32_t)o; o += round_up((size_t)(a.Kc > 1 ? a.Kc - 1 : 0) * a.C * a.C * sizeof(float), 16);
  p.off_bar = (uint32_t)o; o += 32;
  p.smem_bytes = (uint32_t)o;
  if (p.smem_bytes > 200 * 1024) {
    set_error("tcgen05 backward tile does not fit (%u B) although the forward ran on the tensor-core path", p.smem_bytes);
    return STC_ERR_UNSUPPORTED;
  }
  const bool fast = a.Ks == 2 && a.h == 16 && a.Din <= 16 && p.nmain == 1 && !(a.opt & OPT_GENERIC_EPILOGUE);
  const bool at = fast && a.Kc == 2 && p.Kdd <= 64 && (a.Hout == 16 || a.Hout == 32) && !(a.opt & OPT_SMEM_A);
  auto kern = at ? tc_conv_bwd_dx_kernel<true, true>
                 : (fast ? tc_conv_bwd_dx_kernel<true, false> : tc_conv_bwd_dx_kernel<false, false>);
  if (at) p.tmem_cols = 256;
  STC_TRY(set_smem(kern, p.smem_bytes));
  int ctas_per_sm = (int)((228 * 1024) / (p.smem_bytes + 1024));
  if (ctas_per_sm < 1) ctas_per_sm = 1;
  if (ctas_per_sm > 2) ctas_per_sm = 2;
  if (ctas_per_sm * p.tmem_cols > 512) ctas_per_sm = 512 / p.tmem_cols;
  int grid = device_sm_count() * ctas_per_sm;
  if (grid > p.ntiles) grid = p.ntiles;
  const double R = (double)total_nodes * a.C;
  ScopedKernelTimer _t(KK_TC_CONV_BWD_DX, st,
                       4.0 * R * ((a.phase == 0 ? 6 * a.h + a.Ks * a.Din : 3 * a.h) + a.Hout + a.Ks * L +
                                  ((a.dQ && a.Kc > 1) ? p.PW : 0)) + 4.0 * a.Ks * a.Kc * L * a.Hout);
  kern<<<grid, CV_THREADS, p.smem_bytes, st>>>(a, p);
  STC_LAUNCH_OK("tc_conv_bwd_dx_kernel");
  *handled = true;
  return STC_OK;
}

}
```

### stc_gnn_b200/stack.py

```python
from __future__ import annotations

import torch
from torch import nn

from . import _lib
from .cell import STC_Cell
from .support import dense_struct, support_apply


class _XSideTerms(torch.autograd.Function):

    @staticmethod
    def forward(ctx, Gs, X_seq):
        B, T, N, C, Din = X_seq.shape
        W = T * C * Din
        Wp = (W + 3) & ~3
        Xp = X_seq.new_zeros(B, N, Wp) if Wp != W else X_seq.new_empty(B, N, Wp)
        Xp[:, :, :W] = X_seq.permute(0, 2, 1, 3, 4).reshape(B, N, W)
        Gs_c = Gs.detach().contiguous()
        Y1p = support_apply(Gs_c, Xp, transpose=True)
        outs = tuple(Y1p[:, :, t * C * Din:(t + 1) * C * Din].reshape(1, B, N, C, Din).contiguous() for t in range(T))
        ctx.save_for_backward(Gs_c, Xp)
        ctx.shape = (B, T, N, C, Din, W, Wp)
        return outs

    @staticmethod
    @torch.autograd.function.once_differentiable
    def backward(ctx, *dY):
        Gs, Xp = ctx.saved_tensors
        B, T, N, C, Din, W, Wp = ctx.shape
        if not ctx.needs_input_grad[0]:
            return None, None
        dYp = Xp.new_zeros(B, N, Wp) if Wp != W else Xp.new_empty(B, N, Wp)
        for t, g in enumerate(dY):
            piece = dYp[:, :, t * C * Din:(t + 1) * C * Din]
            if g is None:
                piece.zero_()
            else:
                piece.copy_(g.reshape(B, N, C * Din))
        dGs = torch.zeros(N, N, dtype=torch.float32, device=Xp.device)
        lib = _lib.load()
        _lib.check(lib.stc_support_outer(N, B, Wp, Xp.data_ptr(), N * Wp, dYp.data_ptr(), 1.0, dGs.data_ptr(),
                                         torch.cuda.current_stream().cuda_stream), "stc_support_outer")
        _lib.note_launches()
        return dGs, None


def _hoistable(Gs, X_seq: torch.Tensor, cell: STC_Cell) -> bool:
    if not isinstance(Gs, torch.Tensor) or Gs.layout != torch.strided or not Gs.is_cuda or Gs.dtype != torch.float32:
        return False
    B, T, N, C, Din = X_seq.shape
    narrow = (C * Din) % 4 != 0 or C * Din < 32
    return (cell.Ks == 2 and narrow and T >= 2 and B > 0 and N <= 128 and not X_seq.requires_grad and X_seq.is_cuda
            and X_seq.dtype == torch.float32)


class RecurrentStack(nn.Module):
    def __init__(self, num_nodes: int, num_categories: int, Ks: int, Kc: int, input_dim: int, hidden_dim: int,
                 num_layers: int, out_horizon: int, use_bias=True, activation=None):
        super().__init__()
        self.num_layers, self.out_horizon, self.hidden_dim = num_layers, out_horizon, hidden_dim
        self.encoder = nn.ModuleList(
            STC_Cell(num_nodes, num_categories, Ks, Kc, input_dim if i == 0 else hidden_dim, hidden_dim,
                     use_bias=use_bias, activation=activation) for i in range(num_layers))
        self.decoder = nn.ModuleList(
            STC_Cell(num_nodes, num_categories, Ks, Kc, hidden_dim, hidden_dim, use_bias=use_bias,
                     activation=activation) for _ in range(num_layers))

    def forward(self, Gs, Gc: torch.Tensor, X_seq: torch.Tensor) -> torch.Tensor:
        assert X_seq.dim() == 5, "X_seq must be [B,T,N,C,Din]"
        B, T = X_seq.shape[0], X_seq.shape[1]
        seq = [X_seq[:, t] for t in range(T)]
        last = []
        for li, cell in enumerate(self.encoder):
            Ht = cell.init_hidden(B)
            outs = []
            yx = _XSideTerms.apply(Gs, X_seq) if (li == 0 and _hoistable(Gs, X_seq, cell)) else None
            for t in range(T):
                Ht = cell(Gs=Gs, Gc=Gc, Xt=seq[t], Ht_1=Ht, _Yx=None if yx is None else yx[t])
                outs.append(Ht)
            seq = outs
            last.append(Ht)
        if self.out_horizon == 0:
            return torch.stack(seq, dim=1)
        states, x, outs = last, last[-1], []
        for _ in range(self.out_horizon):
            new_states, inp = [], x
            for l, cell in enumerate(self.decoder):
                inp = cell(Gs=Gs, Gc=Gc, Xt=inp, Ht_1=states[l])
                new_states.append(inp)
            states, x = new_states, new_states[-1]
            outs.append(x)
        return torch.stack(outs, dim=1)
```

Before: 60700.

## Share graph-propagated state terms between consumer cells across the recurrent stack

Each hidden state is read by two cells: as input by the next layer and as the previous state by the next timestep. Both cells used to compute their own Chebyshev support terms (Gs·H) for that state. A static sharing plan now lets the first reader export its computed terms as extra autograd outputs, and the second reader takes them as precomputed Yx/Yh. The backward kernels gain fold pointers so the consumer's term gradients are added into the producer's gradient in place. The initial zero hidden state skips the graph multiply entirely. The cost is more plumbing: extra autograd outputs, a wider ABI, and forward ordering that relies on the plan's producer-before-consumer schedule.

After: 64490, median of 6. 6.3% higher.

```diff
diff --git a/include/stc_b200.h b/include/stc_b200.h
--- a/include/stc_b200.h
+++ b/include/stc_b200.h
@@ -8,7 +8,7 @@
 extern "C" {
 #endif
 
-#define STC_ABI_VERSION 6
+#define STC_ABI_VERSION 7
 
 typedef enum {
   STC_OK = 0,
@@ -76,14 +76,17 @@
 int stc_cell_fwd_x(const StcDims* d, const StcSupport* gs, const float* gc,
                    const float* xt, int64_t xt_batch_stride, const float* h_prev,
                    const float* Wg, const float* bg, const float* Wc, const float* bc,
-                   float* h_out, void* saved, size_t saved_bytes, const float* yx_terms, void* stream);
+                   float* h_out, void* saved, size_t saved_bytes, const float* yx_terms, const float* yh_terms,
+                   void* stream);
 int stc_cell_bwd_x(const StcDims* d, const StcSupport* gs, const float* gc,
                    const float* xt, int64_t xt_batch_stride, const float* h_prev,
                    const float* Wg, const float* Wc, const float* d_h_out,
                    float* d_xt, float* d_h_prev,
                    float* dWg, float* dbg, float* dWc, float* dbc, float* dGs, float* dGc,
                    int32_t accumulate_params, const void* saved, size_t saved_bytes,
-                   void* scratch, size_t scratch_bytes, const float* yx_terms, float* dyx_terms_out, void* stream);
+                   void* scratch, size_t scratch_bytes, const float* yx_terms, float* dyx_terms_out,
+                   const float* dyx_fold, const float* yh_terms, float* dyh_terms_out, const float* dyh_fold,
+                   void* stream);
 int stc_support_outer(int32_t N, int32_t B, int32_t width, const float* a, int64_t a_batch_stride, const float* b,
                       float coef, float* dGs, void* stream);
 int stc_support_apply_edge_grad(const StcSupport* gs, int32_t N, int32_t B, int32_t width,
diff --git a/stc_gnn_b200/_lib.py b/stc_gnn_b200/_lib.py
--- a/stc_gnn_b200/_lib.py
+++ b/stc_gnn_b200/_lib.py
@@ -5,7 +5,7 @@
 HERE = os.path.dirname(os.path.abspath(__file__))
 LIB_PATH = os.path.join(HERE, "libstc_b200.so")
 
-ABI_VERSION = 6
+ABI_VERSION = 7
 ACT_NONE, ACT_RELU = 0, 1
 SUPPORT_DENSE, SUPPORT_CSR = 0, 1
 
@@ -58,7 +58,7 @@
     lib.stc_cell_fwd.argtypes = [POINTER(StcDims), POINTER(StcSupport), c_void_p, c_void_p, c_int64, c_void_p,
                                  c_void_p, c_void_p, c_void_p, c_void_p, c_void_p, c_void_p, c_size_t, c_void_p]
     lib.stc_cell_fwd_x.restype = c_int
-    lib.stc_cell_fwd_x.argtypes = lib.stc_cell_fwd.argtypes[:-1] + [c_void_p, c_void_p]
+    lib.stc_cell_fwd_x.argtypes = lib.stc_cell_fwd.argtypes[:-1] + [c_void_p, c_void_p, c_void_p]
     lib.stc_support_outer.restype = c_int
     lib.stc_support_outer.argtypes = [c_int32, c_int32, c_int32, c_void_p, c_int64, c_void_p, c_float, c_void_p, c_void_p]
     lib.stc_support_apply_edge_grad.restype = c_int
@@ -93,7 +93,7 @@
                                  c_void_p, c_void_p, c_void_p, c_int32, c_void_p, c_size_t, c_void_p, c_size_t,
                                  c_void_p]
     lib.stc_cell_bwd_x.restype = c_int
-    lib.stc_cell_bwd_x.argtypes = lib.stc_cell_bwd.argtypes[:-1] + [c_void_p, c_void_p, c_void_p]
+    lib.stc_cell_bwd_x.argtypes = lib.stc_cell_bwd.argtypes[:-1] + [c_void_p] * 7
     lib.stc_cell_bwd_scratch_layout.restype = c_int
     lib.stc_cell_bwd_scratch_layout.argtypes = [POINTER(StcDims), POINTER(c_int64), c_int32]
     lib.stc_cell_bwd_stage.restype = c_int
diff --git a/stc_gnn_b200/cell.py b/stc_gnn_b200/cell.py
--- a/stc_gnn_b200/cell.py
+++ b/stc_gnn_b200/cell.py
@@ -54,10 +54,25 @@
     return t.data_ptr() if t is not None else None
 
 
+_SAVED_OFFSETS = {}
+
+
+def _terms_view(saved, dims, key, side, shape):
+    offs = _SAVED_OFFSETS.get(key)
+    if offs is None:
+        if len(_SAVED_OFFSETS) > 256:
+            _SAVED_OFFSETS.clear()
+        offs = _SAVED_OFFSETS[key] = _lib.saved_layout(dims)
+    n = 1
+    for s_ in shape:
+        n *= s_
+    return saved[offs["Yx" if side == "x" else "Yh"]:][:n].view(shape)
+
+
 class _CellFunction(torch.autograd.Function):
 
     @staticmethod
-    def forward(ctx, Gs, Gc, Xt, H, Wg, bg, Wc, bc, Yx, Ev, cfg):
+    def forward(ctx, Gs, Gc, Xt, H, Wg, bg, Wc, bc, Yx, Ev, cfg, Yh=None, share=None):
         lib = _lib.load()
         Ks, Kc, act = cfg
         B, N, C, Din = Xt.shape
@@ -101,25 +116,33 @@
         saved = torch.empty(_buffer_floats(lib, dims, ctx.size_key)[0], dtype=torch.float32, device=Xt.device)
         Hn = torch.empty((B, N, C, h), dtype=torch.float32, device=Xt.device)
         stream = torch.cuda.current_stream().cuda_stream
-        Yx_c = None
-        if Yx is not None and Ks > 1:
-            if Yx.shape != (Ks - 1, B, N, C, Din) or not Yx.is_cuda or Yx.dtype != torch.float32:
-                raise RuntimeError(f"hoisted Xt-side terms must be a float32 CUDA tensor of shape {(Ks - 1, B, N, C, Din)}, "
-                                   f"got {tuple(Yx.shape)}")
-            Yx_c = Yx.contiguous()
+        give, yx_shared = share if share is not None else ((), False)
+
+        def supplied(Y, w, what):
+            if Y is None or Ks <= 1:
+                return None
+            if Y.shape != (Ks - 1, B, N, C, w) or not Y.is_cuda or Y.dtype != torch.float32:
+                raise RuntimeError(f"supplied {what} terms must be a float32 CUDA tensor of shape {(Ks - 1, B, N, C, w)}, "
+                                   f"got {tuple(Y.shape)}")
+            return Y.contiguous()
+
+        Yx_c, Yh_c = supplied(Yx, Din, "Xt-side"), supplied(Yh, h, "H-side")
+        for side in give:
+            if side not in ("x", "h") or Ks <= 1 or (Yx_c if side == "x" else Yh_c) is not None:
+                raise RuntimeError(f"a cell can only give terms of a side it computes itself (give={give!r}, Ks={Ks})")
         if B == 0:
             status = 0
-        elif Yx_c is not None:
+        elif Yx_c is not None or Yh_c is not None:
             status = lib.stc_cell_fwd_x(dims, gs_struct, Gc_c.data_ptr(), Xt_c.data_ptr(), xbs, H_c.data_ptr(),
                                         Wg_c.data_ptr(), _ptr(bg_c), Wc_c.data_ptr(), _ptr(bc_c), Hn.data_ptr(),
-                                        saved.data_ptr(), saved.numel() * 4, Yx_c.data_ptr(), stream)
+                                        saved.data_ptr(), saved.numel() * 4, _ptr(Yx_c), _ptr(Yh_c), stream)
         else:
             status = lib.stc_cell_fwd(dims, gs_struct, Gc_c.data_ptr(), Xt_c.data_ptr(), xbs, H_c.data_ptr(),
                                       Wg_c.data_ptr(), _ptr(bg_c), Wc_c.data_ptr(), _ptr(bc_c), Hn.data_ptr(),
                                       saved.data_ptr(), saved.numel() * 4, stream)
         _lib.check(status, "stc_cell_fwd")
         _lib.note_launches()
-        ctx.hoisted = Yx_c is not None
+        ctx.hoisted, ctx.h_given, ctx.yx_shared, ctx.give = Yx_c is not None, Yh_c is not None, bool(yx_shared), tuple(give)
         ctx.cfg, ctx.dims_tuple, ctx.xbs, ctx.csr = cfg, (B, N, C, Din, h), xbs, csr
         ctx.gs_obj = Gs if csr else None
         ctx.has_bias = bg is not None
@@ -130,18 +153,24 @@
                     ctx.sinks[i] = t
         ctx.has_ev = Ev is not None
         ctx.save_for_backward(*( [] if csr else [gs_keep] ), Gc_c, Xt_c, H_c, Wg_c, Wc_c, saved,
-                              *([Yx_c] if Yx_c is not None else []), *([Ev] if Ev is not None else []))
-        return Hn
+                              *([Yx_c] if Yx_c is not None else []), *([Yh_c] if Yh_c is not None else []),
+                              *([Ev] if Ev is not None else []))
+        if not give:
+            return Hn
+        ctx.set_materialize_grads(False)
+        return (Hn,) + tuple(_terms_view(saved, dims, ctx.size_key, side, (Ks - 1, B, N, C, Din if side == "x" else h))
+                             for side in give)
 
     @staticmethod
     @torch.autograd.function.once_differentiable
-    def backward(ctx, dHn):
+    def backward(ctx, dHn, *dGiven):
         lib = _lib.load()
         Ks, Kc, act = ctx.cfg
         B, N, C, Din, h = ctx.dims_tuple
         sv = list(ctx.saved_tensors)
         if ctx.has_ev:
             sv.pop()
+        Yh = sv.pop() if ctx.h_given else None
         Yx = sv.pop() if ctx.hoisted else None
         if ctx.csr:
             Gs = ctx.gs_obj
@@ -150,19 +179,22 @@
         else:
             Gs, Gc, Xt, H, Wg, Wc, saved = sv
             gs_struct = dense_struct(Gs)
-        need = ctx.needs_input_grad
-        dev = dHn.device
-        dHn = dHn.contiguous()
+        n_in = len(ctx.needs_input_grad)
+        need = tuple(ctx.needs_input_grad) + (False,) * (13 - n_in)
+        dev = H.device
+        dHn = dHn.contiguous() if dHn is not None else torch.zeros(B, N, C, h, dtype=torch.float32, device=dev)
         L, P = Din + h, Ks * Kc
         dims = _dims(B, N, C, Din, h, Ks, Kc, act, ctx.has_bias)
         new = lambda *shape: torch.empty(shape, dtype=torch.float32, device=dev)
-        if ctx.hoisted and need[2]:
+        if ctx.hoisted and need[2] and not ctx.yx_shared:
             raise RuntimeError("hoisted Xt-side terms: the gradient w.r.t. Xt is folded by the caller (stack.py hoists only "
                                "when the input sequence needs no gradient)")
         dXt = new(B, N, C, Din) if need[2] else None
         dH = new(B, N, C, h)
-        dYx = torch.empty_like(Yx) if ctx.hoisted else None
-        returned = [None] * 11
+        dYx = torch.empty_like(Yx) if ctx.hoisted and need[8] else None
+        dYh = torch.empty_like(Yh) if ctx.h_given and need[11] else None
+        fold = {side: g.contiguous() for side, g in zip(ctx.give, dGiven) if g is not None and B > 0}
+        returned = [None] * 13
 
         def target(i, shape, wanted=True):
             if not wanted:
@@ -181,27 +213,29 @@
         dbg, dbc = target(5, (2 * h,), ctx.has_bias), target(7, (h,), ctx.has_bias)
         dGs = target(9, (Gs.nnz,), need[9]) if ctx.csr else target(0, (N, N), need[0])
         dGc = target(1, (C, C), need[1])
-        returned[2], returned[3], returned[8] = dXt, dH, dYx
+        returned[2], returned[3], returned[8], returned[11] = dXt, dH, dYx, dYh
         if B == 0:
-            if dYx is not None:
-                dYx.zero_()
-            return tuple(returned)
+            for t in (dYx, dYh):
+                if t is not None:
+                    t.zero_()
+            return tuple(returned[:n_in])
         scratch = torch.empty(_buffer_floats(lib, dims, ctx.size_key)[1], dtype=torch.float32, device=dev)
         common = (dims, gs_struct, Gc.data_ptr(), Xt.data_ptr(), ctx.xbs, H.data_ptr(), Wg.data_ptr(),
                   Wc.data_ptr(), dHn.data_ptr(), _ptr(dXt), dH.data_ptr(), dWg.data_ptr(), _ptr(dbg),
                   dWc.data_ptr(), _ptr(dbc), _ptr(dGs), _ptr(dGc), 1, saved.data_ptr(),
                   saved.numel() * 4, scratch.data_ptr(), scratch.numel() * 4)
         stream = torch.cuda.current_stream().cuda_stream
-        if ctx.hoisted:
-            status = lib.stc_cell_bwd_x(*common, Yx.data_ptr(), dYx.data_ptr(), stream)
+        if ctx.hoisted or ctx.h_given or fold:
+            fx, fh = fold.get("x"), fold.get("h")
+            status = lib.stc_cell_bwd_x(*common, _ptr(Yx), _ptr(dYx), _ptr(fx), _ptr(Yh), _ptr(dYh), _ptr(fh), stream)
         else:
             status = lib.stc_cell_bwd(*common, stream)
         _lib.check(status, "stc_cell_bwd")
         _lib.note_launches()
-        for i in (0, 1, 4, 5, 6, 7, 8, 9):
+        for i in (0, 1, 4, 5, 6, 7, 8, 9, 11):
             if not need[i]:
                 returned[i] = None
-        return tuple(returned)
+        return tuple(returned[:n_in])
 
 
 def stc_cell_forward(Gs, Gc, Xt, Ht_1, Wg, bg, Wc, bc, Ks: int, Kc: int, activation=None) -> torch.Tensor:
@@ -230,6 +264,11 @@
     def init_hidden(self, batch_size: int):
         weight = next(self.parameters()).data
         return weight.new_zeros(batch_size, self.num_nodes, self.num_categories, self.hidden_dim)
+
+    def _shared_step(self, Gs, Gc, Xt, Ht_1, Yx=None, Yh=None, give=(), yx_shared=False):
+        return _CellFunction.apply(Gs, Gc, Xt, Ht_1, self.gates.W, getattr(self.gates, "b", None), self.candi.W,
+                                   getattr(self.candi, "b", None), Yx, _edge_values(Gs), (self.Ks, self.Kc, self._act),
+                                   Yh, (give, yx_shared))
 
     def forward(self, Gs, Gc: torch.Tensor, Xt: torch.Tensor, Ht_1: torch.Tensor, _Yx: torch.Tensor = None):
         assert len(Xt.shape) == len(Ht_1.shape) == 4, 'STC-cell must take in 4D tensor as input [Xt, Ht-1]'
diff --git a/stc_gnn_b200/csrc/stc_api.cu b/stc_gnn_b200/csrc/stc_api.cu
--- a/stc_gnn_b200/csrc/stc_api.cu
+++ b/stc_gnn_b200/csrc/stc_api.cu
@@ -414,6 +414,7 @@
   cudaStream_t st;
   Lanes* lanes = nullptr;
   const float* yx_pre = nullptr;
+  const float* yh_pre = nullptr;
 };
 
 static int fwd_terms_xh(const FwdCtx& f) {
@@ -424,7 +425,7 @@
   const int CD = d.C * d.Din, CH = d.C * d.h;
   const long long nbs_h = (long long)d.N * CH;
   cudaStream_t sx = f.st;
-  if (f.lanes && f.lanes->active() && d.Ks > 1 && !f.yx_pre) {
+  if (f.lanes && f.lanes->active() && d.Ks > 1 && !f.yx_pre && !f.yh_pre) {
     STC_TRY(f.lanes->fork(0));
     sx = f.lanes->stream(0);
   }
@@ -437,7 +438,7 @@
     STC_TRY(launch_support_apply(*f.gs, d.N, d.B, CD, true, xin, xin_bs, xz, xz_bs, ws + w.Yx + (size_t)(k - 1) * Rx,
                                  alpha, beta, nullptr, 0.f, sx));
   }
-  for (int k = 1; k < d.Ks; ++k) {
+  for (int k = 1; k < d.Ks && !f.yh_pre; ++k) {
     const float alpha = k == 1 ? 1.f : 2.f, beta = k == 1 ? 0.f : -1.f;
     const float* hin = k == 1 ? f.h_prev : ws + w.Yh + (size_t)(k - 2) * Rh;
     const float* hz = k == 1 ? nullptr : (k == 2 ? f.h_prev : ws + w.Yh + (size_t)(k - 3) * Rh);
@@ -456,7 +457,7 @@
   ConvArgs a = base_args(d, f.xt, f.xt_bs, Wg, ws + w.Q, ws, w, 0);
   if (f.yx_pre) a.yx = f.yx_pre;
   a.h0 = f.h_prev;
-  a.yh = ws + w.Yh;
+  a.yh = f.yh_pre ? f.yh_pre : ws + w.Yh;
   a.bias = d.has_bias ? bg : nullptr;
   a.Hprev = f.h_prev;
   a.u = ws + w.u;
@@ -525,8 +526,8 @@
 
 static int cell_fwd_impl(const StcDims* dp, const StcSupport* gs, const float* gc, const float* xt,
                          int64_t xt_batch_stride, const float* h_prev, const float* Wg, const float* bg, const float* Wc,
-                         const float* bc, float* h_out, void* wsv, size_t ws_bytes, const float* yx_terms, void* stream,
-                         const char* who) {
+                         const float* bc, float* h_out, void* wsv, size_t ws_bytes, const float* yx_terms,
+                         const float* yh_terms, void* stream, const char* who) {
   reset_launch_count();
   STC_TRY(check_fwd_args(dp, gc, xt, h_prev, Wg, bg, Wc, bc, h_out, wsv, ws_bytes, who));
   if (!gs) {
@@ -541,6 +542,7 @@
   FwdCtx f{d, w, gs, gc, xt, xt_batch_stride, h_prev, (float*)wsv, (cudaStream_t)stream};
   f.lanes = &lanes;
   f.yx_pre = d.Ks > 1 ? yx_terms : nullptr;
+  f.yh_pre = d.Ks > 1 ? yh_terms : nullptr;
   STC_TRY(fwd_terms_xh(f));
   STC_TRY(fwd_gates(f, Wg, bg));
   STC_TRY(fwd_terms_rh(f));
@@ -551,15 +553,16 @@
 int stc_cell_fwd(const StcDims* dp, const StcSupport* gs, const float* gc, const float* xt,
                  int64_t xt_batch_stride, const float* h_prev, const float* Wg, const float* bg, const float* Wc,
                  const float* bc, float* h_out, void* wsv, size_t ws_bytes, void* stream) {
-  return cell_fwd_impl(dp, gs, gc, xt, xt_batch_stride, h_prev, Wg, bg, Wc, bc, h_out, wsv, ws_bytes, nullptr, stream,
-                       "stc_cell_fwd");
+  return cell_fwd_impl(dp, gs, gc, xt, xt_batch_stride, h_prev, Wg, bg, Wc, bc, h_out, wsv, ws_bytes, nullptr, nullptr,
+                       stream, "stc_cell_fwd");
 }
 
 int stc_cell_fwd_x(const StcDims* dp, const StcSupport* gs, const float* gc, const float* xt,
                    int64_t xt_batch_stride, const float* h_prev, const float* Wg, const float* bg, const float* Wc,
-                   const float* bc, float* h_out, void* wsv, size_t ws_bytes, const float* yx_terms, void* stream) {
-  return cell_fwd_impl(dp, gs, gc, xt, xt_batch_stride, h_prev, Wg, bg, Wc, bc, h_out, wsv, ws_bytes, yx_terms, stream,
-                       "stc_cell_fwd_x");
+                   const float* bc, float* h_out, void* wsv, size_t ws_bytes, const float* yx_terms,
+                   const float* yh_terms, void* stream) {
+  return cell_fwd_impl(dp, gs, gc, xt, xt_batch_stride, h_prev, Wg, bg, Wc, bc, h_out, wsv, ws_bytes, yx_terms, yh_terms,
+                       stream, "stc_cell_fwd_x");
 }
 
 int stc_cell_saved_layout(const StcDims* dp, int64_t* offsets, int32_t n_offsets) {
@@ -642,6 +645,10 @@
   Lanes* lanes = nullptr;
   const float* yx_pre = nullptr;
   float* dyx_out = nullptr;
+  const float* yh_pre = nullptr;
+  float* dyh_out = nullptr;
+  const float* dyx_fold = nullptr;
+  const float* dyh_fold = nullptr;
   bool want_dGc() const { return dGc != nullptr && d.Kc > 1; }
   float* dYx0() const { return d_xt ? d_xt : sc + w.dYx0; }
 };
@@ -712,6 +719,7 @@
   a.dYx0 = b.dYx0();
   a.dYx = b.dyx_out ? b.dyx_out : b.sc + w.dYx;
   a.accum_x = 0;
+  a.dYx_add = b.dyx_fold;
   a.dYh0 = b.sc + w.dYr;
   a.dYh = b.sc + w.dYr + Rh;
   a.dQ = b.want_dGc() ? b.sc + w.dQ : nullptr;
@@ -728,7 +736,7 @@
   ConvArgs a = base_args(d, b.xt, b.xt_bs, Wg, b.sv + w.Q, b.sv, w, 0);
   if (b.yx_pre) a.yx = b.yx_pre;
   a.h0 = b.h_prev;
-  a.yh = b.sv + w.Yh;
+  a.yh = b.yh_pre ? b.yh_pre : b.sv + w.Yh;
   a.Hprev = b.h_prev;
   a.u = b.sv + w.u;
   a.r = b.sv + w.r;
@@ -741,7 +749,8 @@
   a.dYx = b.dyx_out ? b.dyx_out : b.sc + w.dYx;
   a.accum_x = 1;
   a.dYh0 = b.d_h_prev;
-  a.dYh = b.sc + w.dYh;
+  a.dYh = b.dyh_out ? b.dyh_out : b.sc + w.dYh;
+  a.dYh_add = b.dyh_fold;
   a.dQ = b.want_dGc() ? b.sc + w.dQ : nullptr;
   a.dW = dWg;
   a.Psave = b.sv + w.Pg;
@@ -757,8 +766,9 @@
                          int64_t xt_batch_stride, const float* h_prev, const float* Wg, const float* Wc,
                          const float* d_h_out, float* d_xt, float* d_h_prev, float* dWg, float* dbg, float* dWc, float* dbc,
                          float* dGs, float* dGc, int32_t accumulate_params, const void* savedv, size_t saved_bytes,
-                         void* scratchv, size_t scratch_bytes, const float* yx_terms, float* dyx_terms_out, void* stream,
-                         const char* who) {
+                         void* scratchv, size_t scratch_bytes, const float* yx_terms, float* dyx_terms_out,
+                         const float* dyx_fold, const float* yh_terms, float* dyh_terms_out, const float* dyh_fold,
+                         void* stream, const char* who) {
   reset_launch_count();
   STC_TRY(check_bwd_args(dp, gc, xt, h_prev, Wg, Wc, d_h_out, d_h_prev, dWg, dbg, dWc, dbc, savedv, saved_bytes, scratchv,
                          scratch_bytes, who));
@@ -771,8 +781,8 @@
     set_error("%s: the edge-value gradient of a CSR support needs its rowptr/col/vals and nnz", who);
     return STC_ERR_BAD_ARG;
   }
-  if (d.Ks > 1 && ((yx_terms != nullptr) != (dyx_terms_out != nullptr))) {
-    set_error("%s: yx_terms and dyx_terms_out go together (the caller that supplied the Xt-side terms folds their adjoints)", who);
+  if ((yx_terms && dyx_fold) || (yh_terms && dyh_fold)) {
+    set_error("%s: a side either takes supplied terms or folds an adjoint into its own terms, not both", who);
     return STC_ERR_BAD_ARG;
   }
   const WsLayout w = make_layout(d);
@@ -783,9 +793,18 @@
            const_cast<float*>((const float*)savedv), (float*)scratchv, st};
   b.lanes = &lanes;
   const bool hoisted = d.Ks > 1 && yx_terms != nullptr;
+  const bool h_given = d.Ks > 1 && yh_terms != nullptr;
   if (hoisted) {
     b.yx_pre = yx_terms;
     b.dyx_out = dyx_terms_out;
+  }
+  if (h_given) {
+    b.yh_pre = yh_terms;
+    b.dyh_out = dyh_terms_out;
+  }
+  if (d.Ks > 1) {
+    b.dyx_fold = dyx_fold;
+    b.dyh_fold = dyh_fold;
   }
   const size_t dGs_floats = gs->kind == STC_SUPPORT_CSR ? (size_t)gs->nnz : (size_t)d.N * d.N;
   STC_TRY(bwd_begin(b, dWg, dbg, dWc, dbc, dGs, dGs_floats, accumulate_params));
@@ -805,7 +824,8 @@
     }
     STC_TRY(adjoint_chain(d, *gs, CD, xt, xt_batch_stride, b.sv + w.Yx, b.dYx0(), b.sc + w.dYx, dGs, sx, &lanes, 1));
   }
-  STC_TRY(adjoint_chain(d, *gs, CH, h_prev, (int64_t)d.N * CH, b.sv + w.Yh, d_h_prev, b.sc + w.dYh, dGs, st, &lanes, 1));
+  if (!h_given)
+    STC_TRY(adjoint_chain(d, *gs, CH, h_prev, (int64_t)d.N * CH, b.sv + w.Yh, d_h_prev, b.sc + w.dYh, dGs, st, &lanes, 1));
   return lanes.join_all();
 }
 
@@ -815,18 +835,19 @@
                  float* dGs, float* dGc, int32_t accumulate_params, const void* savedv, size_t saved_bytes,
                  void* scratchv, size_t scratch_bytes, void* stream) {
   return cell_bwd_impl(dp, gs, gc, xt, xt_batch_stride, h_prev, Wg, Wc, d_h_out, d_xt, d_h_prev, dWg, dbg, dWc, dbc, dGs, dGc,
-                       accumulate_params, savedv, saved_bytes, scratchv, scratch_bytes, nullptr, nullptr, stream,
-                       "stc_cell_bwd");
+                       accumulate_params, savedv, saved_bytes, scratchv, scratch_bytes, nullptr, nullptr, nullptr, nullptr,
+                       nullptr, nullptr, stream, "stc_cell_bwd");
 }
 
 int stc_cell_bwd_x(const StcDims* dp, const StcSupport* gs, const float* gc, const float* xt,
                    int64_t xt_batch_stride, const float* h_prev, const float* Wg, const float* Wc,
                    const float* d_h_out, float* d_xt, float* d_h_prev, float* dWg, float* dbg, float* dWc, float* dbc,
                    float* dGs, float* dGc, int32_t accumulate_params, const void* savedv, size_t saved_bytes,
-                   void* scratchv, size_t scratch_bytes, const float* yx_terms, float* dyx_terms_out, void* stream) {
+                   void* scratchv, size_t scratch_bytes, const float* yx_terms, float* dyx_terms_out,
+                   const float* dyx_fold, const float* yh_terms, float* dyh_terms_out, const float* dyh_fold, void* stream) {
   return cell_bwd_impl(dp, gs, gc, xt, xt_batch_stride, h_prev, Wg, Wc, d_h_out, d_xt, d_h_prev, dWg, dbg, dWc, dbc, dGs, dGc,
-                       accumulate_params, savedv, saved_bytes, scratchv, scratch_bytes, yx_terms, dyx_terms_out, stream,
-                       "stc_cell_bwd_x");
+                       accumulate_params, savedv, saved_bytes, scratchv, scratch_bytes, yx_terms, dyx_terms_out, dyx_fold,
+                       yh_terms, dyh_terms_out, dyh_fold, stream, "stc_cell_bwd_x");
 }
 
 int stc_support_outer(int32_t N, int32_t B, int32_t width, const float* a, int64_t a_batch_stride, const float* b,
diff --git a/stc_gnn_b200/csrc/stc_common.cuh b/stc_gnn_b200/csrc/stc_common.cuh
--- a/stc_gnn_b200/csrc/stc_common.cuh
+++ b/stc_gnn_b200/csrc/stc_common.cuh
@@ -150,6 +150,8 @@
   int accum_x;
   float* dYh0;
   float* dYh;
+  const float* dYx_add;
+  const float* dYh_add;
   float* dQ;
   float* dW;
   int opt;
diff --git a/stc_gnn_b200/csrc/stc_conv.cu b/stc_gnn_b200/csrc/stc_conv.cu
--- a/stc_gnn_b200/csrc/stc_conv.cu
+++ b/stc_gnn_b200/csrc/stc_conv.cu
@@ -294,19 +294,22 @@
       float* dx = (k == 0) ? a.dYx0 : a.dYx + (size_t)(k - 1) * R * Din;
       if (dx) {
         dx += row0 * Din;
+        const float* xprior = a.accum_x ? dx
+                              : (k >= 1 && a.dYx_add) ? a.dYx_add + (size_t)(k - 1) * R * Din + row0 * Din : nullptr;
         for (int idx = threadIdx.x; idx < rows_valid * Din; idx += blockDim.x) {
           int row = idx / Din, l = idx - row * Din;
           float v = DY[row * LP + l];
-          dx[idx] = a.accum_x ? dx[idx] + v : v;
+          dx[idx] = xprior ? xprior[idx] + v : v;
         }
       }
       float* dh = (k == 0) ? a.dYh0 : a.dYh + (size_t)(k - 1) * R * h;
       dh += row0 * h;
-      const bool add_direct = (k == 0 && a.phase == 0);
+      const float* hprior = (k == 0 && a.phase == 0) ? dh
+                            : (k >= 1 && a.dYh_add) ? a.dYh_add + (size_t)(k - 1) * R * h + row0 * h : nullptr;
       for (int idx = threadIdx.x; idx < rows_valid * h; idx += blockDim.x) {
         int row = idx / h, l = idx - row * h;
         float v = DY[row * LP + Din + l];
-        dh[idx] = add_direct ? dh[idx] + v : v;
+        dh[idx] = hprior ? hprior[idx] + v : v;
       }
     }
   }
diff --git a/stc_gnn_b200/csrc/stc_conv_tc_big.cu b/stc_gnn_b200/csrc/stc_conv_tc_big.cu
--- a/stc_gnn_b200/csrc/stc_conv_tc_big.cu
+++ b/stc_gnn_b200/csrc/stc_conv_tc_big.cu
@@ -731,11 +731,17 @@
               const float4* src = reinterpret_cast<const float4*>(a.dYh0 + gr * h + c0);
               prev[gi][0] = src[0];
               prev[gi][1] = src[1];
+            } else if (k >= 1 && a.dYh_add != nullptr) {
+              const float4* src = reinterpret_cast<const float4*>(a.dYh_add + (size_t)(k - 1) * R * h + gr * h + c0);
+              prev[gi][0] = src[0];
+              prev[gi][1] = src[1];
             }
           } else {
             const int xi = c0 - h;
-            if (xi < Din && xvec && a.accum_x) {
-              const float* src = (k == 0 ? a.dYx0 : a.dYx + (size_t)(k - 1) * R * Din) + gr * Din + xi;
+            const float* xsrc = a.accum_x ? (k == 0 ? a.dYx0 : a.dYx + (size_t)(k - 1) * R * Din)
+                                : (k >= 1 && a.dYx_add != nullptr) ? a.dYx_add + (size_t)(k - 1) * R * Din : nullptr;
+            if (xi < Din && xvec && xsrc != nullptr) {
+              const float* src = xsrc + gr * Din + xi;
               prev[gi][0] = *reinterpret_cast<const float4*>(src);
               if (xi + 4 < Din) prev[gi][1] = *reinterpret_cast<const float4*>(src + 4);
             }
@@ -832,9 +838,12 @@
             reinterpret_cast<float4*>(dst)[0] = make_float4(v[0] + p0.x, v[1] + p0.y, v[2] + p0.z, v[3] + p0.w);
             if (xi + 4 < Din) reinterpret_cast<float4*>(dst)[1] = make_float4(v[4] + p1.x, v[5] + p1.y, v[6] + p1.z, v[7] + p1.w);
           } else {
+            const float* prior = a.accum_x ? dst
+                                 : (k >= 1 && a.dYx_add != nullptr) ? a.dYx_add + (size_t)(k - 1) * R * Din + gr * Din + xi
+                                                                     : nullptr;
 #pragma unroll
             for (int i = 0; i < 8; ++i)
-              if (xi + i < Din) dst[i] = a.accum_x ? dst[i] + v[i] : v[i];
+              if (xi + i < Din) dst[i] = prior ? prior[i] + v[i] : v[i];
           }
         }
       }
@@ -874,7 +883,7 @@
   *handled = false;
   if (a.Wimg == nullptr || !big_dx_shape_ok(a) || (a.opt & OPT_WIDE_DX_FFMA)) return STC_OK;
   if (!aligned16g(a.dHn) || !aligned16g(a.u) || !aligned16g(a.c) || !aligned16g(a.Hprev) || !aligned16g(a.dpre) ||
-      !aligned16g(a.dYh0) || !aligned16g(a.dYh) || !aligned16g(a.Psave) || (a.dpre_ld % 4) != 0 ||
+      !aligned16g(a.dYh0) || !aligned16g(a.dYh) || !aligned16g(a.dYh_add) || !aligned16g(a.Psave) || (a.dpre_ld % 4) != 0 ||
       (a.phase == 0 && (!aligned16g(a.r) || !aligned16g(a.drH))) || ((reinterpret_cast<uintptr_t>(a.Wimg) & 127) != 0)) {
     set_error("tcgen05 wide-state backward needs 16-byte aligned gradient / workspace tensors");
     return STC_ERR_BAD_ARG;
@@ -886,7 +895,7 @@
   p.KBLp = (p.KBL + 15) & ~15;
   p.nkc = 2 * a.Hout / 32;
   p.DP = a.Hout + 4;
-  p.x_vec = (a.Din % 4 == 0) && aligned16g(a.dYx0) && aligned16g(a.dYx);
+  p.x_vec = (a.Din % 4 == 0) && aligned16g(a.dYx0) && aligned16g(a.dYx) && aligned16g(a.dYx_add);
   const long long total_nodes = (long long)a.B * a.N;
   p.ntiles = ceil_div(total_nodes, p.npt);
   p.stage_bytes = (uint32_t)(2 * p.KBLp * ATOM_ROW_BYTES);
diff --git a/stc_gnn_b200/csrc/stc_conv_tc_bwd.cu b/stc_gnn_b200/csrc/stc_conv_tc_bwd.cu
--- a/stc_gnn_b200/csrc/stc_conv_tc_bwd.cu
+++ b/stc_gnn_b200/csrc/stc_conv_tc_bwd.cu
@@ -81,13 +81,18 @@
     l2_prefetch(a.drH + row0 * a.h, hb);
   }
   if (want_dQ) l2_prefetch(a.Psave + row0 * p.PW, (uint32_t)(nv * a.C * p.PW * 4));
+  const long long R = total_nodes * a.C;
   if (a.accum_x && p.x_vec) {
     const uint32_t xb = (uint32_t)(nv * a.C * a.Din * 4);
-    const long long R = total_nodes * a.C;
     if (a.dYx0) l2_prefetch(a.dYx0 + row0 * a.Din, xb);
     if (a.dYx)
       for (int k = 1; k < a.Ks; ++k) l2_prefetch(a.dYx + (size_t)(k - 1) * R * a.Din + row0 * a.Din, xb);
-  }
+  } else if (a.dYx_add && p.x_vec) {
+    const uint32_t xb = (uint32_t)(nv * a.C * a.Din * 4);
+    for (int k = 1; k < a.Ks; ++k) l2_prefetch(a.dYx_add + (size_t)(k - 1) * R * a.Din + row0 * a.Din, xb);
+  }
+  if (a.dYh_add)
+    for (int k = 1; k < a.Ks; ++k) l2_prefetch(a.dYh_add + (size_t)(k - 1) * R * a.h + row0 * a.h, hb);
 }
 
 template <bool FAST, bool AT>
@@ -379,8 +384,8 @@
 #pragma unroll
     for (int i = 0; i < 4; ++i) xprev[i] = make_float4(0.f, 0.f, 0.f, 0.f);
     if constexpr (FAST) {
-      if (a.accum_x && p.x_vec && erow < rows_valid) {
-        const float* dbase_pf = (half == 0 ? a.dYx0 : a.dYx);
+      if (p.x_vec && erow < rows_valid) {
+        const float* dbase_pf = a.accum_x ? (half == 0 ? a.dYx0 : a.dYx) : (half == 0 ? nullptr : a.dYx_add);
         if (dbase_pf != nullptr) {
           const float* src = dbase_pf + (row0 + erow) * Din;
 #pragma unroll
@@ -470,6 +475,14 @@
               v[i] += d.x; v[i + 1] += d.y; v[i + 2] += d.z; v[i + 3] += d.w;
             }
           }
+          if (k == 1 && a.dYh_add != nullptr) {
+            const float4* ap = reinterpret_cast<const float4*>(a.dYh_add + gr * 16);
+#pragma unroll
+            for (int i = 0; i < 4; ++i) {
+              const float4 q = ap[i];
+              v[4 * i] += q.x; v[4 * i + 1] += q.y; v[4 * i + 2] += q.z; v[4 * i + 3] += q.w;
+            }
+          }
           float* dst = (k == 0 ? a.dYh0 : a.dYh) + gr * 16;
 #pragma unroll
           for (int i = 0; i < 16; i += 4) *reinterpret_cast<float4*>(dst + i) = make_float4(v[i], v[i + 1], v[i + 2], v[i + 3]);
@@ -502,7 +515,7 @@
                                  __uint_as_float(sm[4 * i + 1]) + __uint_as_float(mn[4 * i + 1]),
                                  __uint_as_float(sm[4 * i + 2]) + __uint_as_float(mn[4 * i + 2]),
                                  __uint_as_float(sm[4 * i + 3]) + __uint_as_float(mn[4 * i + 3]));
-            if (a.accum_x) {
+            if (a.accum_x || (k == 1 && a.dYx_add != nullptr)) {
 #pragma unroll
               for (int i = 0; i < 4; ++i)
                 if (4 * i < Din) { o[i].x += xprev[i].x; o[i].y += xprev[i].y; o[i].z += xprev[i].z; o[i].w += xprev[i].w; }
@@ -511,11 +524,12 @@
             for (int i = 0; i < 4; ++i)
               if (4 * i < Din) *reinterpret_cast<float4*>(dst + 4 * i) = o[i];
           } else {
+            const float* prior = a.accum_x ? dst : (k == 1 && a.dYx_add != nullptr) ? a.dYx_add + gr * Din : nullptr;
 #pragma unroll
             for (int i = 0; i < 16; ++i)
               if (i < Din) {
                 const float vi = __uint_as_float(sm[i]) + __uint_as_float(mn[i]);
-                dst[i] = a.accum_x ? dst[i] + vi : vi;
+                dst[i] = prior ? prior[i] + vi : vi;
               }
           }
         }
@@ -550,6 +564,12 @@
 #pragma unroll
             for (int i = 0; i < 8; ++i) v[i] += dp[i];
           }
+          if (k >= 1 && a.dYh_add != nullptr) {
+            const float4* ap = reinterpret_cast<const float4*>(a.dYh_add + (size_t)(k - 1) * R * h + gr * h + kb);
+            const float4 p0 = ap[0], p1 = ap[1];
+            v[0] += p0.x; v[1] += p0.y; v[2] += p0.z; v[3] += p0.w;
+            v[4] += p1.x; v[5] += p1.y; v[6] += p1.z; v[7] += p1.w;
+          }
           reinterpret_cast<float4*>(dst)[0] = make_float4(v[0], v[1], v[2], v[3]);
           reinterpret_cast<float4*>(dst)[1] = make_float4(v[4], v[5], v[6], v[7]);
         } else {
@@ -557,10 +577,13 @@
           float* dbase = (k == 0 ? a.dYx0 : a.dYx + (size_t)(k - 1) * R * Din);
           if (dbase == nullptr) continue;
           float* dst = dbase + gr * Din + xi;
+          const float* prior = a.accum_x ? dst
+                               : (k >= 1 && a.dYx_add != nullptr) ? a.dYx_add + (size_t)(k - 1) * R * Din + gr * Din + xi
+                                                                   : nullptr;
           if (p.x_vec && xi + 8 <= Din) {
             float4 o0 = make_float4(v[0], v[1], v[2], v[3]), o1 = make_float4(v[4], v[5], v[6], v[7]);
-            if (a.accum_x) {
-              const float4 p0 = reinterpret_cast<const float4*>(dst)[0], p1 = reinterpret_cast<const float4*>(dst)[1];
+            if (prior != nullptr) {
+              const float4 p0 = reinterpret_cast<const float4*>(prior)[0], p1 = reinterpret_cast<const float4*>(prior)[1];
               o0.x += p0.x; o0.y += p0.y; o0.z += p0.z; o0.w += p0.w;
               o1.x += p1.x; o1.y += p1.y; o1.z += p1.z; o1.w += p1.w;
             }
@@ -569,7 +592,7 @@
           } else {
 #pragma unroll
             for (int i = 0; i < 8; ++i)
-              if (xi + i < Din) dst[i] = a.accum_x ? dst[i] + v[i] : v[i];
+              if (xi + i < Din) dst[i] = prior ? prior[i] + v[i] : v[i];
           }
         }
       }
@@ -626,7 +649,8 @@
   *handled = false;
   if (!conv_tc_eligible(a)) return STC_OK;
   if (!aligned16b(a.dHn) || !aligned16b(a.u) || !aligned16b(a.c) || !aligned16b(a.Hprev) || !aligned16b(a.dpre) ||
-      !aligned16b(a.dYh0) || !aligned16b(a.dYh) || !aligned16b(a.Psave) || (a.phase == 0 && (!aligned16b(a.r) || !aligned16b(a.drH)))) {
+      !aligned16b(a.dYh0) || !aligned16b(a.dYh) || !aligned16b(a.dYh_add) || !aligned16b(a.Psave) ||
+      (a.phase == 0 && (!aligned16b(a.r) || !aligned16b(a.drH)))) {
     set_error("tcgen05 backward needs 16-byte aligned gradient / workspace tensors");
     return STC_ERR_BAD_ARG;
   }
@@ -644,7 +668,7 @@
   while (p.tmem_cols < (p.nmain + 1) * p.Npad) p.tmem_cols *= 2;
   p.DP = a.Hout + 4;
   p.PW = (a.Kc - 1) * a.Hout;
-  p.x_vec = (a.Din % 4 == 0) && aligned16b(a.dYx0) && aligned16b(a.dYx);
+  p.x_vec = (a.Din % 4 == 0) && aligned16b(a.dYx0) && aligned16b(a.dYx) && aligned16b(a.dYx_add);
   const long long total_nodes = (long long)a.B * a.N;
   p.ntiles = ceil_div(total_nodes, p.npt);
   const size_t atomB = (size_t)p.Npad * ATOM_ROW_BYTES;
diff --git a/stc_gnn_b200/stack.py b/stc_gnn_b200/stack.py
--- a/stc_gnn_b200/stack.py
+++ b/stc_gnn_b200/stack.py
@@ -4,8 +4,8 @@
 from torch import nn
 
 from . import _lib
-from .cell import STC_Cell
-from .support import dense_struct, support_apply
+from .cell import STC_Cell, _csr_cache
+from .support import CsrSupport, dense_struct, support_apply
 
 
 class _XSideTerms(torch.autograd.Function):
@@ -55,6 +55,45 @@
             and X_seq.dtype == torch.float32)
 
 
+def share_plan(layers: int, T: int, horizon: int) -> dict:
+    order, readers = [], {}
+
+    def read(cell, side, state):
+        if state is not None:
+            readers.setdefault(state, []).append((cell, side))
+
+    for l in range(layers):
+        for t in range(T):
+            cell = ("enc", l, t)
+            order.append(cell)
+            read(cell, "x", None if l == 0 else ("enc", l - 1, t))
+            read(cell, "h", None if t == 0 else ("enc", l, t - 1))
+    for s in range(horizon):
+        x = ("enc", layers - 1, T - 1) if s == 0 else ("dec", layers - 1, s - 1)
+        for l in range(layers):
+            cell = ("dec", l, s)
+            order.append(cell)
+            read(cell, "x", x if l == 0 else ("dec", l - 1, s))
+            read(cell, "h", ("enc", l, T - 1) if s == 0 else ("dec", l, s - 1))
+    rank = {c: i for i, c in enumerate(order)}
+    pairs = []
+    for rs in readers.values():
+        if len(rs) == 2 and rs[0][0] != rs[1][0]:
+            first, second = sorted(rs, key=lambda r: rank[r[0]])
+            pairs.append((first, second))
+    pairs.sort(key=lambda pr: rank[pr[0][0]])
+    zero = [(("enc", l, 0), "h") for l in range(layers)] if T > 0 else []
+    return {"pairs": pairs, "zero": zero}
+
+
+def _shares_terms(Gs, cell: STC_Cell) -> bool:
+    if cell.Ks < 2:
+        return False
+    if isinstance(Gs, CsrSupport):
+        return True
+    return isinstance(Gs, torch.Tensor) and Gs.layout == torch.strided and Gs.is_cuda and Gs.dtype == torch.float32
+
+
 class RecurrentStack(nn.Module):
     def __init__(self, num_nodes: int, num_categories: int, Ks: int, Kc: int, input_dim: int, hidden_dim: int,
                  num_layers: int, out_horizon: int, use_bias=True, activation=None):
@@ -70,6 +109,9 @@
     def forward(self, Gs, Gc: torch.Tensor, X_seq: torch.Tensor) -> torch.Tensor:
         assert X_seq.dim() == 5, "X_seq must be [B,T,N,C,Din]"
         B, T = X_seq.shape[0], X_seq.shape[1]
+        if isinstance(Gs, torch.Tensor) and Gs.layout != torch.strided:
+            Gs = _csr_cache(Gs)
+        step = self._shared_steps(Gs, Gc, T)
         seq = [X_seq[:, t] for t in range(T)]
         last = []
         for li, cell in enumerate(self.encoder):
@@ -77,7 +119,11 @@
             outs = []
             yx = _XSideTerms.apply(Gs, X_seq) if (li == 0 and _hoistable(Gs, X_seq, cell)) else None
             for t in range(T):
-                Ht = cell(Gs=Gs, Gc=Gc, Xt=seq[t], Ht_1=Ht, _Yx=None if yx is None else yx[t])
+                yx_t = None if yx is None else yx[t]
+                if step is None:
+                    Ht = cell(Gs=Gs, Gc=Gc, Xt=seq[t], Ht_1=Ht, _Yx=yx_t)
+                else:
+                    Ht = step(cell, ("enc", li, t), seq[t], Ht, yx_t)
                 outs.append(Ht)
             seq = outs
             last.append(Ht)
@@ -87,8 +133,44 @@
         for _ in range(self.out_horizon):
             new_states, inp = [], x
             for l, cell in enumerate(self.decoder):
-                inp = cell(Gs=Gs, Gc=Gc, Xt=inp, Ht_1=states[l])
+                if step is None:
+                    inp = cell(Gs=Gs, Gc=Gc, Xt=inp, Ht_1=states[l])
+                else:
+                    inp = step(cell, ("dec", l, len(outs)), inp, states[l], None)
                 new_states.append(inp)
             states, x = new_states, new_states[-1]
             outs.append(x)
         return torch.stack(outs, dim=1)
+
+    def _shared_steps(self, Gs, Gc, T: int):
+        cells = list(self.encoder) + list(self.decoder)
+        if not cells or not all(_shares_terms(Gs, c) for c in cells) or len({c.Ks for c in cells}) != 1:
+            return None
+        plan = share_plan(self.num_layers, T, self.out_horizon)
+        give = {}
+        for pc, pside in sorted((p for p, _ in plan["pairs"]), key=lambda p: p[1]):
+            give[pc] = give.get(pc, ()) + (pside,)
+        take = {}
+        for producer, (cc, cside) in plan["pairs"]:
+            take.setdefault(cc, {})[cside] = producer
+        zero = {c for c, _ in plan["zero"]}
+        given = {}
+        Ks = cells[0].Ks
+
+        def step(cell, key, Xt, H, yx):
+            src = take.get(key, {})
+            yx_shared = "x" in src
+            if yx_shared:
+                yx = given.pop(src["x"])
+            yh = given.pop(src["h"]) if "h" in src else None
+            if key in zero:
+                yh = H.unsqueeze(0) if Ks == 2 else H.new_zeros((Ks - 1,) + tuple(H.shape))
+            g = give.get(key, ())
+            out = cell._shared_step(Gs, Gc, Xt, H, yx, yh, g, yx_shared)
+            if not g:
+                return out
+            for side, terms in zip(g, out[1:]):
+                given[(key, side)] = terms
+            return out[0]
+
+        return step
```
